# Pose-Group/FAMI-Pose

Hardware: AMD Instinct MI355X
Metric: train clips/sec (5-frame 384x288 HRNet-W48) (higher is better)
Workload: dtype f32

## Files before the change

fami-pose_amd/csrc/elementwise.hip:

```cpp
#include "common.h"

template <typename T>
__global__ void nchw_to_nhwc_kernel(const float* __restrict__ src, T* __restrict__ dst, int N, int C, int H, int W) {
  const long total = (long)N * C * H * W;
  const long HW = (long)H * W;
  for (long i = blockIdx.x * (long)blockDim.x + threadIdx.x; i < total; i += (long)gridDim.x * blockDim.x) {
    const int c = (int)(i % C);
    const long p = i / C;
    const long n = p / HW, hw = p - n * HW;
    st1(dst + i, src[(n * C + c) * HW + hw]);
  }
}
template <typename T>
__global__ void nhwc_to_nchw_kernel(const T* __restrict__ src, float* __restrict__ dst, int N, int C, int H, int W,
                                    int accumulate) {
  const long total = (long)N * C * H * W;
  const long HW = (long)H * W;
  for (long i = blockIdx.x * (long)blockDim.x + threadIdx.x; i < total; i += (long)gridDim.x * blockDim.x) {
    const long hw = i % HW;
    const long nc = i / HW;
    const long n = nc / C;
    const int c = (int)(nc - n * C);
    const float v = ld1(src + (n * HW + hw) * C + c);
    dst[i] = accumulate ? dst[i] + v : v;
  }
}

template <typename T>
__global__ void pack_frames_kernel(const float* __restrict__ kf, const float* __restrict__ sup, T* __restrict__ out,
                                   int B, int S, int H, int W) {
  const long HW = (long)H * W;
  const long total = (long)(1 + S) * B * HW * 3;
  for (long i = blockIdx.x * (long)blockDim.x + threadIdx.x; i < total; i += (long)gridDim.x * blockDim.x) {
    const int c = (int)(i % 3);
    const long p = i / 3;
    const long n = p / HW, hw = p - n * HW;
    const int f = (int)(n / B), b = (int)(n - (long)f * B);
    float v;
    if (f == 0)
      v = kf[((long)b * 3 + c) * HW + hw];
    else
      v = sup[((long)b * 3 * S + 3 * (f - 1) + c) * HW + hw];
    st1(out + i, v);
  }
}

template <typename T, int V>
__global__ void copy_channels_kernel(const T* __restrict__ src, T* __restrict__ dst, long P, int Cs, int src_off,
                                     int Cd, int dst_off, int Cc, int accumulate) {
  const int CcV = Cc / V;
  const long total = P * CcV;
  for (long i = blockIdx.x * (long)blockDim.x + threadIdx.x; i < total; i += (long)gridDim.x * blockDim.x) {
    const int c = (int)(i % CcV) * V;
    const long p = i / CcV;
    const T* sp = src + p * Cs + src_off + c;
    T* d = dst + p * Cd + dst_off + c;
    if (V == 4) {
      f32x4 v = ld4(sp);
      if (accumulate) v += ld4(d);
      st4(d, v);
    } else {
      const float v = ld1(sp);
      st1(d, accumulate ? ld1(d) + v : v);
    }
  }
}

struct Cat4 { const void* src[4]; void* dst[4]; int c[4], acc[4]; int n; };
template <typename T, bool SPLIT>
__global__ void cat4_kernel(Cat4 a, const T* __restrict__ whole_src, T* __restrict__ whole_dst, long P, int Ct) {
  const int CtV = Ct >> 2;
  const long total = P * CtV;
  for (long i = blockIdx.x * (long)blockDim.x + threadIdx.x; i < total; i += (long)gridDim.x * blockDim.x) {
    const int c = (int)(i % CtV) * 4;
    const long p = i / CtV;
    int k = 0, base = 0;
#pragma unroll
    for (int j = 0; j < 3; ++j)
      if (j + 1 < a.n && c >= base + a.c[k]) {
        base += a.c[k];
        ++k;
      }
    if (SPLIT) {
      T* d = reinterpret_cast<T*>(a.dst[k]);
      if (!d) continue;
      d += p * a.c[k] + (c - base);
      f32x4 v = ld4(whole_src + p * Ct + c);
      if (a.acc[k]) v += ld4(d);
      st4(d, v);
    } else {
      st4(whole_dst + p * Ct + c, ld4(reinterpret_cast<const T*>(a.src[k]) + p * a.c[k] + (c - base)));
    }
  }
}
template <typename T>
static int cat4_impl(bool split, const void* const* ptrs, const int* cs, const int* accs, int n, const T* whole_src, T* whole_dst, long P,
                     hipStream_t s, const char* nm) {
  FAMI_REQUIRE(ptrs && cs && n >= 1 && n <= 4 && P > 0 && (split ? (const void*)whole_src : (const void*)whole_dst), nm, "bad argument");
  Cat4 a;
  int Ct = 0;
  for (int k = 0; k < 4; ++k) {
    a.src[k] = nullptr; a.dst[k] = nullptr; a.c[k] = 0; a.acc[k] = 0;
    if (k < n) {
      FAMI_REQUIRE(cs[k] > 0 && (cs[k] & 3) == 0 && (split || ptrs[k]) && (reinterpret_cast<uintptr_t>(ptrs[k]) & 7) == 0, nm,
                   "channel counts must be multiples of 4, pointers 8-byte aligned");
      if (split) { a.dst[k] = const_cast<void*>(ptrs[k]); a.acc[k] = accs ? accs[k] : 0; }
      else a.src[k] = ptrs[k];
      a.c[k] = cs[k];
      Ct += cs[k];
    }
  }
  a.n = n;
  if (split) hipLaunchKernelGGL((cat4_kernel<T, true>), dim3(fami_ew_grid(P * Ct / 4)), dim3(256), 0, s, a, whole_src, (T*)nullptr, P, Ct);
  else hipLaunchKernelGGL((cat4_kernel<T, false>), dim3(fami_ew_grid(P * Ct / 4)), dim3(256), 0, s, a, (const T*)nullptr, whole_dst, P, Ct);
  FAMI_CHECK_LAUNCH(nm);
  return FAMI_OK;
}

__global__ void scale_pairs_kernel(const float* __restrict__ in, float* __restrict__ out, long n, float sx, float sy, int acc) {
  const long i = blockIdx.x * (long)blockDim.x + threadIdx.x;
  if (i >= 2 * n) return;
  const float v = in[i] * ((i & 1) ? sy : sx);
  out[i] = acc ? out[i] + v : v;
}

__global__ __launch_bounds__(256) void unscale_check_kernel(float* __restrict__ g, long n, float f, unsigned* __restrict__ flag) {
  bool bad = false;
  const long n4 = n >> 2;
  for (long i = blockIdx.x * (long)blockDim.x + threadIdx.x; i < n4; i += (long)gridDim.x * blockDim.x) {
    f32x4 v = ld4(g + i * 4) * f;
#pragma unroll
    for (int t = 0; t < 4; ++t) bad |= !(fabsf(v[t]) <= 3.4028235e38f);
    st4(g + i * 4, v);
  }
  for (long i = n4 * 4 + blockIdx.x * (long)blockDim.x + threadIdx.x; i < n; i += (long)gridDim.x * blockDim.x) {
    const float v = g[i] * f;
    bad |= !(fabsf(v) <= 3.4028235e38f);
    g[i] = v;
  }
  if (__any(bad) && (threadIdx.x & 63) == 0) atomicOr(flag, 1u);
}

template <typename T>
__global__ void axpby_kernel(const T* a, const T* b, T* out, long n, float alpha, float beta, int vec) {
  const long n4 = vec ? n >> 2 : 0;
  for (long i = blockIdx.x * (long)blockDim.x + threadIdx.x; i < n4; i += (long)gridDim.x * blockDim.x) {
    f32x4 v = ld4(a + i * 4) * alpha;
    if (b) v += ld4(b + i * 4) * beta;
    st4(out + i * 4, v);
  }
  for (long i = (n4 << 2) + blockIdx.x * (long)blockDim.x + threadIdx.x; i < n; i += (long)gridDim.x * blockDim.x) {
    float v = alpha * ld1(a + i);
    if (b) v += beta * ld1(b + i);
    st1(out + i, v);
  }
}

template <typename T>
__global__ void cast_add_kernel(const float* __restrict__ src, T* dst, long n, int accumulate) {
  for (long i = blockIdx.x * (long)blockDim.x + threadIdx.x; i < n; i += (long)gridDim.x * blockDim.x) {
    const float v = src[i];
    st1(dst + i, accumulate ? ld1(dst + i) + v : v);
  }
}

template <typename T>
__global__ void fill_kernel(T* out, long n, float v) {
  for (long i = blockIdx.x * (long)blockDim.x + threadIdx.x; i < n; i += (long)gridDim.x * blockDim.x) st1(out + i, v);
}

__global__ void incr_i64_kernel(long long* v, long n) {
  for (long i = blockIdx.x * (long)blockDim.x + threadIdx.x; i < n; i += (long)gridDim.x * blockDim.x) v[i] += 1;
}
__global__ void add_i64_kernel(long long* v, const long long* inc, long n) {
  for (long i = blockIdx.x * (long)blockDim.x + threadIdx.x; i < n; i += (long)gridDim.x * blockDim.x) v[i] += inc[i];
}

template <typename T>
struct FuseArgs {
  const T* x[4];
  const float* mean[4];
  const float* invstd[4];
  const float* gamma[4];
  const float* beta[4];
  int shift[4];
  int nterms;
};

template <typename T>
__global__ __launch_bounds__(256) void fuse_sum_kernel(FuseArgs<T> a, T* __restrict__ y, int N, int H, int W, int C,
                                                       int relu) {
  const int CV = C >> 2;
  const long total = (long)N * H * W * CV;
  for (long i = blockIdx.x * (long)blockDim.x + threadIdx.x; i < total; i += (long)gridDim.x * blockDim.x) {
    const int cv = (int)(i % CV);
    long p = i / CV;
    const int w = (int)(p % W);
    p /= W;
    const int h = (int)(p % H);
    const long n = p / H;
    f32x4 acc = {0.f, 0.f, 0.f, 0.f};
    for (int k = 0; k < a.nterms; ++k) {
      const int s = a.shift[k];
      const int Hk = H >> s, Wk = W >> s;
      const long o = ((n * Hk + (h >> s)) * Wk + (w >> s)) * C + cv * 4;
      f32x4 v = ld4(a.x[k] + o);
      if (a.mean[k]) {
#pragma unroll
        for (int t = 0; t < 4; ++t) {
          const int c = cv * 4 + t;
          const float sc = a.invstd[k][c] * a.gamma[k][c];
          v[t] = v[t] * sc + (a.beta[k][c] - a.mean[k][c] * sc);
        }
      }
      acc += v;
    }
    if (relu) {
#pragma unroll
      for (int t = 0; t < 4; ++t) acc[t] = fmaxf(acc[t], 0.f);
    }
    st4(y + i * 4, acc);
  }
}

template <typename T>
__global__ void relu_bwd_kernel(const T* __restrict__ dy, const T* __restrict__ y, T* dx, long n4, int accumulate) {
  for (long i = blockIdx.x * (long)blockDim.x + threadIdx.x; i < n4; i += (long)gridDim.x * blockDim.x) {
    f32x4 g = ld4(dy + i * 4);
    const f32x4 yy = ld4(y + i * 4);
#pragma unroll
    for (int t = 0; t < 4; ++t) g[t] = yy[t] > 0.f ? g[t] : 0.f;
    if (accumulate) g += ld4(dx + i * 4);
    st4(dx + i * 4, g);
  }
}

template <typename T>
__global__ void pool_relu_bwd_kernel(const T* __restrict__ dy, const T* __restrict__ y, T* __restrict__ out, int N,
                                     int Hl, int Wl, int C, int s, int relu) {
  const int CV = C >> 2;
  const int f = 1 << s;
  const int H = Hl << s, W = Wl << s;
  const long total = (long)N * Hl * Wl * CV;
  for (long i = blockIdx.x * (long)blockDim.x + threadIdx.x; i < total; i += (long)gridDim.x * blockDim.x) {
    const int cv = (int)(i % CV);
    long p = i / CV;
    const int wl = (int)(p % Wl);
    p /= Wl;
    const int hl = (int)(p % Hl);
    const long n = p / Hl;
    f32x4 acc = {0.f, 0.f, 0.f, 0.f};
    for (int dh = 0; dh < f; ++dh)
      for (int dw = 0; dw < f; ++dw) {
        const long o = ((n * H + (hl * f + dh)) * W + (wl * f + dw)) * C + cv * 4;
        f32x4 g = ld4(dy + o);
        if (relu) {
          const f32x4 yy = ld4(y + o);
#pragma unroll
          for (int t = 0; t < 4; ++t) g[t] = yy[t] > 0.f ? g[t] : 0.f;
        }
        acc += g;
      }
    st4(out + i * 4, acc);
  }
}

__global__ void adam_prep_kernel(float* state, float beta1, float beta2, unsigned* flag) {
  if (threadIdx.x == 0 && blockIdx.x == 0) {
    if (flag && *flag) {
      *flag = 0u;
      flag[1] += 1u;
      state[2] = 0.f;
      return;
    }
    const float t = state[0] + 1.f;
    state[0] = t;
    state[2] = 1.f - powf(beta1, t);
    state[3] = 1.f - powf(beta2, t);
  }
}
__device__ __forceinline__ void adam_elem(float& p, float gi, float& m, float& v, float beta1, float beta2, float eps,
                                          float wd, float step_size, float bc2s) {
#pragma clang fp contract(off)
  const float pi = p;
  if (wd != 0.f) gi = fmaf(wd, pi, gi);
  const float mi = beta1 * m + (1.f - beta1) * gi;
  const float vi = beta2 * v + (1.f - beta2) * gi * gi;
  m = mi;
  v = vi;
  p = fmaf(-step_size, mi / (sqrtf(vi) / bc2s + eps), pi);
}
template <bool SCALED>
__device__ __forceinline__ void adam_body(float* __restrict__ p, const float* __restrict__ g, float* __restrict__ m,
                                          float* __restrict__ v, long n, const float* __restrict__ state, float beta1,
                                          float beta2, float eps, float wd, const float* __restrict__ gmul) {
  const float lr = state[1], bc1 = state[2], bc2s = sqrtf(state[3]);
  if (bc1 == 0.f) return;
  const float step_size = lr / bc1;
  const float gm = SCALED ? gmul[0] : 1.f;
  for (long i = blockIdx.x * (long)blockDim.x + threadIdx.x; i < n; i += (long)gridDim.x * blockDim.x) {
    const float gi = SCALED ? mul_rn(gm, g[i]) : g[i];
    float pe = p[i], me = m[i], ve = v[i];
    adam_elem(pe, gi, me, ve, beta1, beta2, eps, wd, step_size, bc2s);
    m[i] = me;
    v[i] = ve;
    p[i] = pe;
  }
}
__global__ void adam_kernel(float* __restrict__ p, const float* __restrict__ g, float* __restrict__ m,
                            float* __restrict__ v, long n, const float* __restrict__ state, float beta1,
                            float beta2, float eps, float wd) {
  adam_body<false>(p, g, m, v, n, state, beta1, beta2, eps, wd, nullptr);
}
__global__ void adam_scaled_kernel(float* __restrict__ p, const float* __restrict__ g, float* __restrict__ m,
                                   float* __restrict__ v, long n, const float* __restrict__ state, float beta1,
                                   float beta2, float eps, float wd, const float* __restrict__ gmul) {
  adam_body<true>(p, g, m, v, n, state, beta1, beta2, eps, wd, gmul);
}


template <typename T>
static int nchw_to_nhwc_impl(const float* src, T* dst, int N, int C, int H, int W, hipStream_t s, const char* nm) {
  FAMI_REQUIRE(src && dst && N > 0 && C > 0 && H > 0 && W > 0, nm, "bad argument");
  hipLaunchKernelGGL(nchw_to_nhwc_kernel<T>, dim3(fami_ew_grid((long)N * C * H * W)), dim3(256), 0, s, src, dst, N, C, H, W);
  FAMI_CHECK_LAUNCH(nm);
  return FAMI_OK;
}
template <typename T>
static int nhwc_to_nchw_impl(const T* src, float* dst, int N, int C, int H, int W, int accumulate, hipStream_t s,
                             const char* nm) {
  FAMI_REQUIRE(src && dst && N > 0 && C > 0 && H > 0 && W > 0, nm, "bad argument");
  hipLaunchKernelGGL(nhwc_to_nchw_kernel<T>, dim3(fami_ew_grid((long)N * C * H * W)), dim3(256), 0, s, src, dst, N, C, H, W, accumulate);
  FAMI_CHECK_LAUNCH(nm);
  return FAMI_OK;
}
template <typename T>
static int pack_frames_impl(const float* kf, const float* sup, T* out, int B, int S, int H, int W, hipStream_t s,
                            const char* nm) {
  FAMI_REQUIRE(kf && out && B > 0 && S >= 0 && (S == 0 || sup), nm, "bad argument");
  hipLaunchKernelGGL(pack_frames_kernel<T>, dim3(fami_ew_grid((long)(1 + S) * B * H * W * 3)), dim3(256), 0, s, kf, sup, out, B, S, H, W);
  FAMI_CHECK_LAUNCH(nm);
  return FAMI_OK;
}
template <typename T>
static int copy_channels_impl(const T* src, T* dst, long P, int Cs, int src_off, int Cd, int dst_off, int Cc,
                              int accumulate, hipStream_t s, const char* nm) {
  FAMI_REQUIRE(src && dst && P > 0 && Cc > 0 && src_off >= 0 && dst_off >= 0 && src_off + Cc <= Cs && dst_off + Cc <= Cd, nm, "bad argument");
  const bool v4 = ((Cs | src_off | Cd | dst_off | Cc) & 3) == 0 && ((reinterpret_cast<uintptr_t>(src) | reinterpret_cast<uintptr_t>(dst)) & 15) == 0;
  if (v4)
    hipLaunchKernelGGL((copy_channels_kernel<T, 4>), dim3(fami_ew_grid(P * Cc / 4)), dim3(256), 0, s, src, dst, P, Cs, src_off, Cd, dst_off, Cc, accumulate);
  else
    hipLaunchKernelGGL((copy_channels_kernel<T, 1>), dim3(fami_ew_grid(P * Cc)), dim3(256), 0, s, src, dst, P, Cs, src_off, Cd, dst_off, Cc, accumulate);
  FAMI_CHECK_LAUNCH(nm);
  return FAMI_OK;
}
template <typename T>
static int axpby_impl(const T* a, const T* b, T* out, long n, float alpha, float beta, hipStream_t s, const char* nm) {
  FAMI_REQUIRE(a && out && n > 0, nm, "bad argument");
  const int vec = ((reinterpret_cast<uintptr_t>(a) | reinterpret_cast<uintptr_t>(b) | reinterpret_cast<uintptr_t>(out)) & (4 * sizeof(T) - 1)) == 0;
  hipLaunchKernelGGL(axpby_kernel<T>, dim3(fami_ew_grid(vec ? (n + 3) / 4 : n)), dim3(256), 0, s, a, b, out, n, alpha, beta, vec);
  FAMI_CHECK_LAUNCH(nm);
  return FAMI_OK;
}
template <typename T>
__global__ void widen_kernel(const T* __restrict__ src, float* __restrict__ dst, long n) {
  for (long i = blockIdx.x * (long)blockDim.x + threadIdx.x; i < n; i += (long)gridDim.x * blockDim.x) dst[i] = ld1(src + i);
}
template <typename T>
static int widen_impl(const T* src, float* dst, long n, hipStream_t s, const char* nm) {
  FAMI_REQUIRE(src && dst && n > 0, nm, "bad argument");
  hipLaunchKernelGGL(widen_kernel<T>, dim3(fami_ew_grid(n)), dim3(256), 0, s, src, dst, n);
  FAMI_CHECK_LAUNCH(nm);
  return FAMI_OK;
}

template <typename T>
static int cast_add_impl(const float* src, T* dst, long n, int accumulate, hipStream_t s, const char* nm) {
  FAMI_REQUIRE(src && dst && n > 0, nm, "bad argument");
  hipLaunchKernelGGL(cast_add_kernel<T>, dim3(fami_ew_grid(n)), dim3(256), 0, s, src, dst, n, accumulate);
  FAMI_CHECK_LAUNCH(nm);
  return FAMI_OK;
}
template <typename T>
static int fill_impl(T* out, long n, float v, hipStream_t s, const char* nm) {
  FAMI_REQUIRE(out && n > 0, nm, "bad argument");
  hipLaunchKernelGGL(fill_kernel<T>, dim3(fami_ew_grid(n)), dim3(256), 0, s, out, n, v);
  FAMI_CHECK_LAUNCH(nm);
  return FAMI_OK;
}
template <typename T>
static int fuse_sum_impl(int nterms, const T* const* x, const float* const* mean, const float* const* invstd,
                         const float* const* gamma, const float* const* beta, const int* shift, T* y, int N, int H,
                         int W, int C, int relu, hipStream_t s, const char* nm) {
  FAMI_REQUIRE(nterms >= 1 && nterms <= 4 && x && shift && y && (C % 4) == 0, nm, "bad argument");
  FuseArgs<T> a;
  a.nterms = nterms;
  for (int k = 0; k < 4; ++k) {
    const bool on = k < nterms;
    a.x[k] = on ? x[k] : nullptr;
    a.mean[k] = on && mean ? mean[k] : nullptr;
    a.invstd[k] = on && invstd ? invstd[k] : nullptr;
    a.gamma[k] = on && gamma ? gamma[k] : nullptr;
    a.beta[k] = on && beta ? beta[k] : nullptr;
    a.shift[k] = on ? shift[k] : 0;
    if (on) {
      FAMI_REQUIRE(a.x[k] && a.shift[k] >= 0 && (H % (1 << a.shift[k])) == 0 && (W % (1 << a.shift[k])) == 0, nm, "bad term");
    }
  }
  hipLaunchKernelGGL(fuse_sum_kernel<T>, dim3(fami_ew_grid((long)N * H * W * (C / 4))), dim3(256), 0, s, a, y, N, H, W, C, relu);
  FAMI_CHECK_LAUNCH(nm);
  return FAMI_OK;
}
template <typename T>
static int relu_bwd_impl(const T* dy, const T* y, T* dx, long n, int accumulate, hipStream_t s, const char* nm) {
  FAMI_REQUIRE(dy && y && dx && n > 0 && (n % 4) == 0, nm, "bad argument");
  hipLaunchKernelGGL(relu_bwd_kernel<T>, dim3(fami_ew_grid(n / 4)), dim3(256), 0, s, dy, y, dx, n / 4, accumulate);
  FAMI_CHECK_LAUNCH(nm);
  return FAMI_OK;
}
template <typename T>
static int pool_relu_bwd_impl(const T* dy, const T* y, T* out, int N, int Hl, int Wl, int C, int shift, int relu,
                              hipStream_t s, const char* nm) {
  FAMI_REQUIRE(dy && out && (!relu || y) && (C % 4) == 0 && shift >= 0 && shift <= 4, nm, "bad argument");
  hipLaunchKernelGGL(pool_relu_bwd_kernel<T>, dim3(fami_ew_grid((long)N * Hl * Wl * (C / 4))), dim3(256), 0, s, dy, y, out, N, Hl, Wl, C, shift, relu);
  FAMI_CHECK_LAUNCH(nm);
  return FAMI_OK;
}


#define FAMI_AXPBY_BATCH 32
struct AxpbyBatch { const float* a[FAMI_AXPBY_BATCH]; float* out[FAMI_AXPBY_BATCH]; int n[FAMI_AXPBY_BATCH]; };
__global__ __launch_bounds__(256) void add_batch_kernel(AxpbyBatch b) {
  const float* __restrict__ a = b.a[blockIdx.y];
  float* __restrict__ o = b.out[blockIdx.y];
  const int n = b.n[blockIdx.y];
  for (int i = blockIdx.x * 256 + threadIdx.x; i < n; i += gridDim.x * 256) o[i] += a[i];
}

extern "C" {

#define FAMI_EW_ABI(sfx, T)                                                                                            \
  int fami_nchw_to_nhwc_##sfx(const float* src, T* dst, int N, int C, int H, int W, hipStream_t s) {                   \
    return nchw_to_nhwc_impl<T>(src, dst, N, C, H, W, s, "fami_nchw_to_nhwc_" #sfx);                                   \
  }                                                                                                                    \
  int fami_nhwc_to_nchw_##sfx(const T* src, float* dst, int N, int C, int H, int W, int accumulate, hipStream_t s) {   \
    return nhwc_to_nchw_impl<T>(src, dst, N, C, H, W, accumulate, s, "fami_nhwc_to_nchw_" #sfx);                       \
  }                                                                                                                    \
                        \
  int fami_pack_frames_##sfx(const float* kf, const float* sup, T* out, int B, int S, int H, int W, hipStream_t s) {   \
    return pack_frames_impl<T>(kf, sup, out, B, S, H, W, s, "fami_pack_frames_" #sfx);                                 \
  }                                                                                                                    \
  int fami_copy_channels_##sfx(const T* src, T* dst, long P, int Cs, int src_off, int Cd, int dst_off, int Cc,         \
                               int accumulate, hipStream_t s) {                                                        \
    return copy_channels_impl<T>(src, dst, P, Cs, src_off, Cd, dst_off, Cc, accumulate, s, "fami_copy_channels_" #sfx);\
  }                                                                                                                    \
                                         \
  int fami_concat_channels_##sfx(const T* const* src, const int* c, int n, T* dst, long P, hipStream_t s) {            \
    return cat4_impl<T>(false, reinterpret_cast<const void* const*>(src), c, nullptr, n, (const T*)nullptr, dst, P, s, \
                        "fami_concat_channels_" #sfx);                                                                \
  }                                                                                                                    \
   \
  int fami_split_channels_##sfx(const T* src, T* const* dst, const int* c, const int* accumulate, int n, long P,       \
                                hipStream_t s) {                                                                       \
    return cat4_impl<T>(true, reinterpret_cast<const void* const*>(dst), c, accumulate, n, src, (T*)nullptr, P, s,     \
                        "fami_split_channels_" #sfx);                                                                 \
  }                                                                                                                    \
  int fami_axpby_##sfx(const T* a, const T* b, T* out, long n, float alpha, float beta, hipStream_t s) {               \
    return axpby_impl<T>(a, b, out, n, alpha, beta, s, "fami_axpby_" #sfx);                                            \
  }                                                                                                                    \
  int fami_cast_add_##sfx(const float* src, T* dst, long n, int accumulate, hipStream_t s) {                           \
    return cast_add_impl<T>(src, dst, n, accumulate, s, "fami_cast_add_" #sfx);                                        \
  }                                                                                                                    \
  int fami_widen_##sfx(const T* src, float* dst, long n, hipStream_t s) {                                              \
    return widen_impl<T>(src, dst, n, s, "fami_widen_" #sfx);                                                          \
  }                                                                                                                    \
  int fami_fill_##sfx(T* out, long n, float v, hipStream_t s) { return fill_impl<T>(out, n, v, s, "fami_fill_" #sfx); }\
   \
  int fami_fuse_sum_##sfx(int nterms, const T* const* x, const float* const* mean, const float* const* invstd,         \
                          const float* const* gamma, const float* const* beta, const int* shift, T* y, int N, int H,   \
                          int W, int C, int relu, hipStream_t s) {                                                     \
    return fuse_sum_impl<T>(nterms, x, mean, invstd, gamma, beta, shift, y, N, H, W, C, relu, s, "fami_fuse_sum_" #sfx);\
  }                                                                                                                    \
  int fami_relu_bwd_##sfx(const T* dy, const T* y, T* dx, long n, int accumulate, hipStream_t s) {                     \
    return relu_bwd_impl<T>(dy, y, dx, n, accumulate, s, "fami_relu_bwd_" #sfx);                                       \
  }                                                                                                                    \
                                                                     \
  int fami_pool_relu_bwd_##sfx(const T* dy, const T* y, T* out, int N, int Hl, int Wl, int C, int shift, int relu,     \
                               hipStream_t s) {                                                                        \
    return pool_relu_bwd_impl<T>(dy, y, out, N, Hl, Wl, C, shift, relu, s, "fami_pool_relu_bwd_" #sfx);                \
  }
FAMI_EW_ABI(f32, float)
FAMI_EW_ABI(bf16, bf16_t)
FAMI_EW_ABI(f16, f16_t)
#undef FAMI_EW_ABI

int fami_scale_pairs_f32(const float* in, float* out, long n, float sx, float sy, int accumulate, hipStream_t s) {
  FAMI_REQUIRE(in && out && n > 0, "fami_scale_pairs_f32", "bad argument");
  hipLaunchKernelGGL(scale_pairs_kernel, dim3(fami_cdiv(2 * n, 256)), dim3(256), 0, s, in, out, n, sx, sy, accumulate);
  FAMI_CHECK_LAUNCH("fami_scale_pairs_f32");
  return FAMI_OK;
}

int fami_incr_i64(long long* v, long n, hipStream_t s) {
  FAMI_REQUIRE(v && n > 0, "fami_incr_i64", "bad argument");
  hipLaunchKernelGGL(incr_i64_kernel, dim3(fami_ew_grid(n)), dim3(256), 0, s, v, n);
  FAMI_CHECK_LAUNCH("fami_incr_i64");
  return FAMI_OK;
}

int fami_add_i64(long long* v, const long long* inc, long n, hipStream_t s) {
  FAMI_REQUIRE(v && inc && n > 0, "fami_add_i64", "bad argument");
  hipLaunchKernelGGL(add_i64_kernel, dim3(fami_ew_grid(n)), dim3(256), 0, s, v, inc, n);
  FAMI_CHECK_LAUNCH("fami_add_i64");
  return FAMI_OK;
}

int fami_adam_prep_f32(float* state, float beta1, float beta2, hipStream_t s) {
  FAMI_REQUIRE(state, "fami_adam_prep_f32", "bad argument");
  hipLaunchKernelGGL(adam_prep_kernel, dim3(1), dim3(64), 0, s, state, beta1, beta2, (unsigned*)nullptr);
  FAMI_CHECK_LAUNCH("fami_adam_prep_f32");
  return FAMI_OK;
}
int fami_adam_prep_checked_f32(float* state, float beta1, float beta2, unsigned* flag, hipStream_t s) {
  FAMI_REQUIRE(state && flag, "fami_adam_prep_checked_f32", "bad argument");
  hipLaunchKernelGGL(adam_prep_kernel, dim3(1), dim3(64), 0, s, state, beta1, beta2, flag);
  FAMI_CHECK_LAUNCH("fami_adam_prep_checked_f32");
  return FAMI_OK;
}
int fami_unscale_check_f32(float* g, long n, float f, unsigned* flag, hipStream_t s) {
  FAMI_REQUIRE(g && flag && n > 0, "fami_unscale_check_f32", "bad argument");
  hipLaunchKernelGGL(unscale_check_kernel, dim3(fami_ew_grid((n + 3) / 4)), dim3(256), 0, s, g, n, f, flag);
  FAMI_CHECK_LAUNCH("fami_unscale_check_f32");
  return FAMI_OK;
}
int fami_adam_f32(float* p, const float* g, float* m, float* v, long n, const float* state, float beta1, float beta2,
                  float eps, float weight_decay, hipStream_t s) {
  FAMI_REQUIRE(p && g && m && v && state && n > 0, "fami_adam_f32", "bad argument");
  hipLaunchKernelGGL(adam_kernel, dim3(fami_ew_grid(n)), dim3(256), 0, s, p, g, m, v, n, state, beta1, beta2, eps, weight_decay);
  FAMI_CHECK_LAUNCH("fami_adam_f32");
  return FAMI_OK;
}
int fami_adam_scaled_f32(float* p, const float* g, float* m, float* v, long n, const float* state, float beta1, float beta2,
                         float eps, float weight_decay, const float* gmul, hipStream_t s) {
  FAMI_REQUIRE(p && g && m && v && state && gmul && n > 0, "fami_adam_scaled_f32", "bad argument");
  hipLaunchKernelGGL(adam_scaled_kernel, dim3(fami_ew_grid(n)), dim3(256), 0, s, p, g, m, v, n, state, beta1, beta2, eps,
                     weight_decay, gmul);
  FAMI_CHECK_LAUNCH("fami_adam_scaled_f32");
  return FAMI_OK;
}


int fami_add_batch_f32(const long* ptrs, const int* counts, int n, hipStream_t s) {
  FAMI_REQUIRE(ptrs && counts && n > 0, "fami_add_batch_f32", "bad argument");
  int i0 = 0;
  while (i0 < n) {
    AxpbyBatch b;
    int m = 0, maxn = 1;
    for (; m < FAMI_AXPBY_BATCH && i0 + m < n; ++m) {
      float* o = reinterpret_cast<float*>(ptrs[2 * (i0 + m) + 1]);
      bool repeated = false;
      for (int k = 0; k < m; ++k) repeated |= (b.out[k] == o);
      if (repeated) break;
      b.a[m] = reinterpret_cast<const float*>(ptrs[2 * (i0 + m)]);
      b.out[m] = o;
      b.n[m] = counts[i0 + m];
      if (b.n[m] > maxn) maxn = b.n[m];
    }
    for (int i = m; i < FAMI_AXPBY_BATCH; ++i) { b.a[i] = b.a[0]; b.out[i] = b.out[0]; b.n[i] = 0; }
    int gx = (maxn + 255) / 256;
    if (gx > 64) gx = 64;
    hipLaunchKernelGGL(add_batch_kernel, dim3(gx, m), dim3(256), 0, s, b);
    FAMI_CHECK_LAUNCH("fami_add_batch_f32");
    i0 += m;
  }
  return FAMI_OK;
}

}
```

fami-pose_amd/csrc/norm.hip:

```cpp
#include "common.h"

#define BN_MAXG 512
#ifndef BN_U
#define BN_U 4
#endif

struct ColMap {
  int cv, prow, rows, CV;
  bool active;
};
__device__ __forceinline__ ColMap col_map(int C) {
  ColMap m;
  m.CV = C >> 2;
  m.rows = 256 / m.CV;
  m.cv = threadIdx.x % m.CV;
  m.prow = threadIdx.x / m.CV;
  m.active = m.prow < m.rows;
  return m;
}

__device__ __forceinline__ double block_sum_d(double v, double* sm4) {
  v = wave_sum_d(v);
  const int lane = threadIdx.x & 63, wave = threadIdx.x >> 6;
  __syncthreads();
  if (lane == 0) sm4[wave] = v;
  __syncthreads();
  return (sm4[0] + sm4[1]) + (sm4[2] + sm4[3]);
}

template <typename T>
__global__ __launch_bounds__(256) void bn_partial_kernel(const T* __restrict__ x, float* __restrict__ partial,
                                                         long P, int C) {
  extern __shared__ float sm[];
  const ColMap m = col_map(C);
  f32x4 s = {0.f, 0.f, 0.f, 0.f}, q = {0.f, 0.f, 0.f, 0.f};
  if (m.active) {
    const f32x4 piv = ld4(x + m.cv * 4);
    const long step = (long)gridDim.x * m.rows;
    long p = (long)blockIdx.x * m.rows + m.prow;
    for (; p + (BN_U - 1) * step < P; p += BN_U * step) {
      f32x4 v[BN_U];
#pragma unroll
      for (int u = 0; u < BN_U; ++u) v[u] = ld4(x + (p + u * step) * C + m.cv * 4);
#pragma unroll
      for (int u = 0; u < BN_U; ++u) {
        const f32x4 d = v[u] - piv;
        s += d;
        q += d * d;
      }
    }
    for (; p < P; p += step) {
      const f32x4 v = ld4(x + p * C + m.cv * 4) - piv;
      s += v;
      q += v * v;
    }
    float* d = sm + (long)m.prow * 2 * C;
#pragma unroll
    for (int t = 0; t < 4; ++t) {
      d[m.cv * 4 + t] = s[t];
      d[C + m.cv * 4 + t] = q[t];
    }
  }
  __syncthreads();
  for (int e = threadIdx.x; e < 2 * C; e += 256) {
    float tot = 0.f;
    for (int r = 0; r < m.rows; ++r) tot += sm[(long)r * 2 * C + e];
    partial[(long)blockIdx.x * 2 * C + e] = tot;
  }
}

template <typename T>
__global__ void bn_finalize_kernel(const float* __restrict__ partial, const T* __restrict__ x, int G, long P,
                                   int C, float* mean, float* invstd, float* running_mean, float* running_var,
                                   float momentum, float eps) {
  __shared__ double sm4[4];
  const int c = blockIdx.x;
  double s = 0.0, q = 0.0;
  for (int g = threadIdx.x; g < G; g += 256) {
    s += (double)partial[(long)g * 2 * C + c];
    q += (double)partial[(long)g * 2 * C + C + c];
  }
  s = block_sum_d(s, sm4);
  q = block_sum_d(q, sm4);
  if (threadIdx.x != 0) return;
  const double dm = s / (double)P;
  double var = q / (double)P - dm * dm;
  if (var < 0.0) var = 0.0;
  const double mu = (double)ld1(x + c) + dm;
  mean[c] = (float)mu;
  invstd[c] = (float)(1.0 / sqrt(var + (double)eps));
  if (running_mean) {
    const double unb = P > 1 ? var * (double)P / (double)(P - 1) : var;
    running_mean[c] = (float)((1.0 - momentum) * running_mean[c] + momentum * mu);
    running_var[c] = (float)((1.0 - momentum) * running_var[c] + momentum * unb);
  }
}

__global__ void bn_finalize_slots_kernel(const double* __restrict__ slots, int NS, const float* __restrict__ pivot, long P,
                                         int C, float* mean, float* invstd, float* running_mean, float* running_var,
                                         float momentum, float eps) {
  const int c = blockIdx.x * blockDim.x + threadIdx.x;
  if (c >= C) return;
  double s = 0.0, q = 0.0;
  for (int k = 0; k < NS; ++k) {
    s += slots[(long)k * 2 * C + c];
    q += slots[(long)k * 2 * C + C + c];
  }
  const double invP = 1.0 / (double)P;
  const double dm = s * invP;
  double var = q * invP - dm * dm;
  if (var < 0.0) var = 0.0;
  const double mu = (double)pivot[c] + dm;
  mean[c] = (float)mu;
  invstd[c] = (float)(1.0 / sqrt(var + (double)eps));
  if (running_mean) {
    const double unb = P > 1 ? var * (double)P / (double)(P - 1) : var;
    running_mean[c] = (float)((1.0 - momentum) * running_mean[c] + momentum * mu);
    running_var[c] = (float)((1.0 - momentum) * running_var[c] + momentum * unb);
  }
}

__global__ void bn_running_update_kernel(float* running_mean, float* running_var, const float* __restrict__ mean,
                                         const float* __restrict__ invstd, int C, long P, float momentum, float eps) {
  const int c = blockIdx.x * blockDim.x + threadIdx.x;
  if (c >= C) return;
  const double mu = (double)mean[c], is = (double)invstd[c];
  double var = 1.0 / (is * is) - (double)eps;
  if (var < 0.0) var = 0.0;
  const double unb = P > 1 ? var * (double)P / (double)(P - 1) : var;
  running_mean[c] = (float)((1.0 - momentum) * running_mean[c] + momentum * mu);
  running_var[c] = (float)((1.0 - momentum) * running_var[c] + momentum * unb);
}


#define FAMI_BNRU_BATCH 32
struct BnRunBatch { float* rm[FAMI_BNRU_BATCH]; float* rv[FAMI_BNRU_BATCH]; const float* mean[FAMI_BNRU_BATCH]; const float* invstd[FAMI_BNRU_BATCH];
                    int C[FAMI_BNRU_BATCH]; float P[FAMI_BNRU_BATCH], mom[FAMI_BNRU_BATCH], eps[FAMI_BNRU_BATCH]; int n; };
__global__ __launch_bounds__(256) void bn_running_update_batch_kernel(BnRunBatch b) {
  const int c = blockIdx.x * blockDim.x + threadIdx.x;
  for (int k = 0; k < b.n; ++k) {
    if (c >= b.C[k]) continue;
    const double mu = (double)b.mean[k][c], is = (double)b.invstd[k][c];
    double var = 1.0 / (is * is) - (double)b.eps[k];
    if (var < 0.0) var = 0.0;
    const double P = (double)b.P[k];
    const double unb = P > 1.0 ? var * P / (P - 1.0) : var;
    const float momentum = b.mom[k];
    b.rm[k][c] = (float)((1.0 - momentum) * b.rm[k][c] + momentum * mu);
    b.rv[k][c] = (float)((1.0 - momentum) * b.rv[k][c] + momentum * unb);
  }
}

__global__ void bn_eval_stats_kernel(const float* running_mean, const float* running_var, float* mean, float* invstd,
                                     int C, float eps) {
  const int c = blockIdx.x * blockDim.x + threadIdx.x;
  if (c >= C) return;
  mean[c] = running_mean[c];
  invstd[c] = 1.0f / sqrtf(running_var[c] + eps);
}

template <typename T>
__global__ __launch_bounds__(256) void bn_apply_kernel(const T* __restrict__ x, const float* __restrict__ mean,
                                                       const float* __restrict__ invstd,
                                                       const float* __restrict__ gamma,
                                                       const float* __restrict__ beta,
                                                       const T* __restrict__ residual, T* __restrict__ y,
                                                       long P, int C, int relu) {
  const ColMap m = col_map(C);
  if (!m.active) return;
  f32x4 sc, sf;
#pragma unroll
  for (int t = 0; t < 4; ++t) {
    const int c = m.cv * 4 + t;
    sc[t] = invstd[c] * gamma[c];
    sf[t] = beta[c] - mean[c] * sc[t];
  }
  for (long p = (long)blockIdx.x * m.rows + m.prow; p < P; p += (long)gridDim.x * m.rows) {
    const long o = p * C + m.cv * 4;
    f32x4 v = ld4(x + o) * sc + sf;
    if (residual) v += ld4(residual + o);
    if (relu) {
#pragma unroll
      for (int t = 0; t < 4; ++t) v[t] = fmaxf(v[t], 0.f);
    }
    st4(y + o, v);
  }
}

template <typename T>
__global__ __launch_bounds__(256) void bn_bwd_partial_kernel(const T* __restrict__ dy,
                                                             const T* __restrict__ x,
                                                             const T* __restrict__ y,
                                                             const float* __restrict__ mean,
                                                             const float* __restrict__ invstd,
                                                             float* __restrict__ partial, long P, int C, int relu) {
  extern __shared__ float sm[];
  const ColMap m = col_map(C);
  f32x4 s = {0.f, 0.f, 0.f, 0.f}, q = {0.f, 0.f, 0.f, 0.f};
  if (m.active) {
    f32x4 mu, is;
#pragma unroll
    for (int t = 0; t < 4; ++t) {
      mu[t] = mean[m.cv * 4 + t];
      is[t] = invstd[m.cv * 4 + t];
    }
    const long step = (long)gridDim.x * m.rows;
    for (long p = (long)blockIdx.x * m.rows + m.prow; p < P; p += BN_U * step) {
      f32x4 g[BN_U], yy[BN_U], xx[BN_U];
      long o[BN_U];
#pragma unroll
      for (int u = 0; u < BN_U; ++u) {
        const long pu = p + u * step;
        o[u] = (pu < P ? pu : p) * C + m.cv * 4;
        g[u] = ld4(dy + o[u]);
      }
      if (relu) {
#pragma unroll
        for (int u = 0; u < BN_U; ++u) yy[u] = ld4(y + o[u]);
      }
#pragma unroll
      for (int u = 0; u < BN_U; ++u) xx[u] = ld4(x + o[u]);
#pragma unroll
      for (int u = 0; u < BN_U; ++u) {
        if (relu) {
#pragma unroll
          for (int t = 0; t < 4; ++t) g[u][t] = yy[u][t] > 0.f ? g[u][t] : 0.f;
        }
        if (p + u * step >= P) g[u] = f32x4{0.f, 0.f, 0.f, 0.f};
        const f32x4 xh = (xx[u] - mu) * is;
        s += g[u];
        q += g[u] * xh;
      }
    }
    float* d = sm + (long)m.prow * 2 * C;
#pragma unroll
    for (int t = 0; t < 4; ++t) {
      d[m.cv * 4 + t] = s[t];
      d[C + m.cv * 4 + t] = q[t];
    }
  }
  __syncthreads();
  for (int e = threadIdx.x; e < 2 * C; e += 256) {
    float tot = 0.f;
    for (int r = 0; r < m.rows; ++r) tot += sm[(long)r * 2 * C + e];
    partial[(long)blockIdx.x * 2 * C + e] = tot;
  }
}

__global__ void bn_bwd_finalize_kernel(const float* __restrict__ partial, int G, long P, int C, float* coef,
                                       float* dgamma, float* dbeta, int accumulate) {
  __shared__ double sm4[4];
  const int c = blockIdx.x;
  double s = 0.0, q = 0.0;
  for (int g = threadIdx.x; g < G; g += 256) {
    s += (double)partial[(long)g * 2 * C + c];
    q += (double)partial[(long)g * 2 * C + C + c];
  }
  s = block_sum_d(s, sm4);
  q = block_sum_d(q, sm4);
  if (threadIdx.x != 0) return;
  if (coef) {
    coef[c] = (float)(s / (double)P);
    coef[C + c] = (float)(q / (double)P);
  }
  if (dgamma) dgamma[c] = accumulate ? dgamma[c] + (float)q : (float)q;
  if (dbeta) dbeta[c] = accumulate ? dbeta[c] + (float)s : (float)s;
}

template <typename T>
__global__ __launch_bounds__(256) void bn_bwd_apply_kernel(const T* __restrict__ dy, const T* __restrict__ x,
                                                           const T* __restrict__ y,
                                                           const float* __restrict__ mean,
                                                           const float* __restrict__ invstd,
                                                           const float* __restrict__ gamma,
                                                           const float* __restrict__ coef, T* __restrict__ dx,
                                                           T* __restrict__ dres, long P, int C, int relu,
                                                           int acc_dx, int acc_dres) {
  const ColMap m = col_map(C);
  if (!m.active) return;
  f32x4 mu, is, gi, c1, c2;
#pragma unroll
  for (int t = 0; t < 4; ++t) {
    const int c = m.cv * 4 + t;
    mu[t] = mean[c];
    is[t] = invstd[c];
    gi[t] = gamma[c] * invstd[c];
    c1[t] = coef[c];
    c2[t] = coef[C + c];
  }
  for (long p = (long)blockIdx.x * m.rows + m.prow; p < P; p += (long)gridDim.x * m.rows) {
    const long o = p * C + m.cv * 4;
    f32x4 g = ld4(dy + o);
    if (relu) {
      const f32x4 yy = ld4(y + o);
#pragma unroll
      for (int t = 0; t < 4; ++t) g[t] = yy[t] > 0.f ? g[t] : 0.f;
    }
    const f32x4 xh = (ld4(x + o) - mu) * is;
    f32x4 d = gi * (g - c1 - xh * c2);
    if (acc_dx) d += ld4(dx + o);
    st4(dx + o, d);
    if (dres) {
      f32x4 r = g;
      if (acc_dres) r += ld4(dres + o);
      st4(dres + o, r);
    }
  }
}

template <typename T, bool SUMS>
__global__ __launch_bounds__(256) void bn_eval_bwd_kernel(const T* __restrict__ dy, const T* __restrict__ x,
                                                          const T* __restrict__ y, const float* __restrict__ mean,
                                                          const float* __restrict__ invstd,
                                                          const float* __restrict__ gamma, float* __restrict__ partial,
                                                          T* dx, T* dres, long P, int C, int relu, int acc_dx,
                                                          int acc_dres) {
  extern __shared__ float sm[];
  const ColMap m = col_map(C);
  f32x4 s = {0.f, 0.f, 0.f, 0.f}, q = {0.f, 0.f, 0.f, 0.f};
  if (m.active) {
    f32x4 mu = {0.f, 0.f, 0.f, 0.f}, is, gi;
#pragma unroll
    for (int t = 0; t < 4; ++t) {
      const int c = m.cv * 4 + t;
      is[t] = invstd[c];
      gi[t] = gamma[c] * is[t];
      if (SUMS) mu[t] = mean[c];
    }
    const long step = (long)gridDim.x * m.rows;
    for (long p = (long)blockIdx.x * m.rows + m.prow; p < P; p += BN_U * step) {
      f32x4 g[BN_U], yy[BN_U], xx[BN_U], dd[BN_U], rr[BN_U];
      long o[BN_U];
#pragma unroll
      for (int u = 0; u < BN_U; ++u) {
        const long pu = p + u * step;
        o[u] = (pu < P ? pu : p) * C + m.cv * 4;
        g[u] = ld4(dy + o[u]);
      }
      if (relu) {
#pragma unroll
        for (int u = 0; u < BN_U; ++u) yy[u] = ld4(y + o[u]);
      }
      if (SUMS) {
#pragma unroll
        for (int u = 0; u < BN_U; ++u) xx[u] = ld4(x + o[u]);
      }
      if (acc_dx) {
#pragma unroll
        for (int u = 0; u < BN_U; ++u) dd[u] = ld4(dx + o[u]);
      }
      if (dres && acc_dres) {
#pragma unroll
        for (int u = 0; u < BN_U; ++u) rr[u] = ld4(dres + o[u]);
      }
#pragma unroll
      for (int u = 0; u < BN_U; ++u) {
        if (relu) {
#pragma unroll
          for (int t = 0; t < 4; ++t) g[u][t] = yy[u][t] > 0.f ? g[u][t] : 0.f;
        }
        const bool in = p + u * step < P;
        if (SUMS) {
          const f32x4 gz = in ? g[u] : f32x4{0.f, 0.f, 0.f, 0.f};
          s += gz;
          q += gz * ((xx[u] - mu) * is);
        }
        if (in) {
          f32x4 d = g[u] * gi;
          if (acc_dx) d += dd[u];
          st4(dx + o[u], d);
          if (dres) {
            f32x4 r = g[u];
            if (acc_dres) r += rr[u];
            st4(dres + o[u], r);
          }
        }
      }
    }
    if (SUMS) {
      float* d = sm + (long)m.prow * 2 * C;
#pragma unroll
      for (int t = 0; t < 4; ++t) {
        d[m.cv * 4 + t] = s[t];
        d[C + m.cv * 4 + t] = q[t];
      }
    }
  }
  if (!SUMS) return;
  __syncthreads();
  for (int e = threadIdx.x; e < 2 * C; e += 256) {
    float tot = 0.f;
    for (int r = 0; r < m.rows; ++r) tot += sm[(long)r * 2 * C + e];
    partial[(long)blockIdx.x * 2 * C + e] = tot;
  }
}


template <typename T>
__global__ __launch_bounds__(256) void bn_partial2_kernel(const T* __restrict__ x, double* __restrict__ slots, int NS,
                                                          long P, int C) {
  extern __shared__ float sm[];
  const ColMap m = col_map(C);
  f32x4 s = {0.f, 0.f, 0.f, 0.f}, q = {0.f, 0.f, 0.f, 0.f};
  if (m.active) {
    const f32x4 piv = ld4(x + m.cv * 4);
    const long step = (long)gridDim.x * m.rows;
    long p = (long)blockIdx.x * m.rows + m.prow;
    for (; p + (BN_U - 1) * step < P; p += BN_U * step) {
      f32x4 v[BN_U];
#pragma unroll
      for (int u = 0; u < BN_U; ++u) v[u] = ld4(x + (p + u * step) * C + m.cv * 4);
#pragma unroll
      for (int u = 0; u < BN_U; ++u) {
        const f32x4 d = v[u] - piv;
        s += d;
        q += d * d;
      }
    }
    for (; p < P; p += step) {
      const f32x4 v = ld4(x + p * C + m.cv * 4) - piv;
      s += v;
      q += v * v;
    }
    float* d = sm + (long)m.prow * 2 * C;
#pragma unroll
    for (int t = 0; t < 4; ++t) {
      d[m.cv * 4 + t] = s[t];
      d[C + m.cv * 4 + t] = q[t];
    }
  }
  __syncthreads();
  double* row = slots + (long)(blockIdx.x % NS) * 2 * C;
  for (int e = threadIdx.x; e < 2 * C; e += 256) {
    float tot = 0.f;
    for (int r = 0; r < m.rows; ++r) tot += sm[(long)r * 2 * C + e];
    unsafeAtomicAdd(row + e, (double)tot);
  }
}

__device__ __forceinline__ void bn_scale_shift(float mean, float invstd, float gamma, float beta, float& sc, float& sf) {
  sc = invstd * gamma;
  sf = __builtin_fmaf(-mean, sc, beta);
}

template <typename T>
__global__ __launch_bounds__(256) void bn_apply2_kernel(const T* __restrict__ x, const double* __restrict__ slots, int NS,
                                                        const float* __restrict__ gamma, const float* __restrict__ beta,
                                                        const T* __restrict__ residual, T* __restrict__ y,
                                                        float* __restrict__ mean, float* __restrict__ invstd,
                                                        float* running_mean, float* running_var, long P, int C,
                                                        int relu, float momentum, float eps, const float* pivot) {
  extern __shared__ float sm[];
  for (int c = threadIdx.x; c < C; c += 256) {
    double s = 0.0, q = 0.0;
    for (int k = 0; k < NS; ++k) {
      s += slots[(long)k * 2 * C + c];
      q += slots[(long)k * 2 * C + C + c];
    }
    const double invP = 1.0 / (double)P;
    const double dm = s * invP;
    double var = q * invP - dm * dm;
    if (var < 0.0) var = 0.0;
    const double mu = (double)(pivot ? pivot[c] : ld1(x + c)) + dm;
    const float muf = (float)mu;
    const float isf = (float)(1.0 / sqrt(var + (double)eps));
    if (blockIdx.x == 0) {
      mean[c] = muf;
      invstd[c] = isf;
      if (running_mean) {
        const double unb = P > 1 ? var * (double)P / (double)(P - 1) : var;
        running_mean[c] = (float)((1.0 - momentum) * running_mean[c] + momentum * mu);
        running_var[c] = (float)((1.0 - momentum) * running_var[c] + momentum * unb);
      }
    }
    float sc, sf;
    bn_scale_shift(muf, isf, gamma[c], beta[c], sc, sf);
    sm[c] = sc;
    sm[C + c] = sf;
  }
  __syncthreads();
  const ColMap m = col_map(C);
  if (!m.active) return;
  const f32x4 sc = *reinterpret_cast<const f32x4*>(sm + m.cv * 4), sf = *reinterpret_cast<const f32x4*>(sm + C + m.cv * 4);
  for (long p = (long)blockIdx.x * m.rows + m.prow; p < P; p += (long)gridDim.x * m.rows) {
    const long o = p * C + m.cv * 4;
    const f32x4 xv = ld4(x + o);
    f32x4 v;
#pragma unroll
    for (int t = 0; t < 4; ++t) v[t] = __builtin_fmaf(xv[t], sc[t], sf[t]);
    if (residual) v += ld4(residual + o);
    if (relu) {
#pragma unroll
      for (int t = 0; t < 4; ++t) v[t] = fmaxf(v[t], 0.f);
    }
    st4(y + o, v);
  }
}

__device__ __forceinline__ f32x4 bn_relu_mask(f32x4 g, int relu, f32x4 yy, f32x4 xv, f32x4 sc, f32x4 sf) {
  if (relu == 1) {
#pragma unroll
    for (int t = 0; t < 4; ++t) g[t] = yy[t] > 0.f ? g[t] : 0.f;
  } else if (relu == 2) {
#pragma unroll
    for (int t = 0; t < 4; ++t) g[t] = __builtin_fmaf(xv[t], sc[t], sf[t]) > 0.f ? g[t] : 0.f;
  }
  return g;
}

template <typename T>
__global__ __launch_bounds__(256) void bn_bwd_partial2_kernel(const T* __restrict__ dy, const T* __restrict__ x,
                                                              const T* __restrict__ y, const float* __restrict__ mean,
                                                              const float* __restrict__ invstd,
                                                              const float* __restrict__ gamma,
                                                              const float* __restrict__ beta,
                                                              double* __restrict__ slots, int NS, long P, int C, int relu) {
  extern __shared__ float sm[];
  const ColMap m = col_map(C);
  f32x4 s = {0.f, 0.f, 0.f, 0.f}, q = {0.f, 0.f, 0.f, 0.f};
  if (m.active) {
    f32x4 mu, is, sc, sf;
#pragma unroll
    for (int t = 0; t < 4; ++t) {
      const int c = m.cv * 4 + t;
      mu[t] = mean[c];
      is[t] = invstd[c];
      float a, b;
      bn_scale_shift(mu[t], is[t], gamma[c], beta[c], a, b);
      sc[t] = a;
      sf[t] = b;
    }
    const long step = (long)gridDim.x * m.rows;
    for (long p = (long)blockIdx.x * m.rows + m.prow; p < P; p += BN_U * step) {
      f32x4 g[BN_U], yy[BN_U], xx[BN_U];
      long o[BN_U];
#pragma unroll
      for (int u = 0; u < BN_U; ++u) {
        const long pu = p + u * step;
        o[u] = (pu < P ? pu : p) * C + m.cv * 4;
        g[u] = ld4(dy + o[u]);
      }
      if (relu == 1) {
#pragma unroll
        for (int u = 0; u < BN_U; ++u) yy[u] = ld4(y + o[u]);
      }
#pragma unroll
      for (int u = 0; u < BN_U; ++u) xx[u] = ld4(x + o[u]);
#pragma unroll
      for (int u = 0; u < BN_U; ++u) {
        g[u] = bn_relu_mask(g[u], relu, yy[u], xx[u], sc, sf);
        if (p + u * step >= P) g[u] = f32x4{0.f, 0.f, 0.f, 0.f};
        const f32x4 xh = (xx[u] - mu) * is;
        s += g[u];
        q += g[u] * xh;
      }
    }
    float* d = sm + (long)m.prow * 2 * C;
#pragma unroll
    for (int t = 0; t < 4; ++t) {
      d[m.cv * 4 + t] = s[t];
      d[C + m.cv * 4 + t] = q[t];
    }
  }
  __syncthreads();
  double* row = slots + (long)(blockIdx.x % NS) * 2 * C;
  for (int e = threadIdx.x; e < 2 * C; e += 256) {
    float tot = 0.f;
    for (int r = 0; r < m.rows; ++r) tot += sm[(long)r * 2 * C + e];
    unsafeAtomicAdd(row + e, (double)tot);
  }
}

template <typename T>
__global__ __launch_bounds__(256) void bn_bwd_apply2_kernel(const T* __restrict__ dy, const T* __restrict__ x,
                                                            const T* __restrict__ y, const float* __restrict__ mean,
                                                            const float* __restrict__ invstd,
                                                            const float* __restrict__ gamma,
                                                            const float* __restrict__ beta,
                                                            const double* __restrict__ slots, int NS, T* __restrict__ dx,
                                                            float* dgamma, float* dbeta, T* __restrict__ dres, long P,
                                                            int C, int relu, int acc_dx, int acc_param, int acc_dres) {
  extern __shared__ float sm[];
  for (int c = threadIdx.x; c < C; c += 256) {
    double s = 0.0, q = 0.0;
    for (int k = 0; k < NS; ++k) {
      s += slots[(long)k * 2 * C + c];
      q += slots[(long)k * 2 * C + C + c];
    }
    sm[c] = (float)(s / (double)P);
    sm[C + c] = (float)(q / (double)P);
    if (blockIdx.x == 0) {
      if (dgamma) dgamma[c] = acc_param ? dgamma[c] + (float)q : (float)q;
      if (dbeta) dbeta[c] = acc_param ? dbeta[c] + (float)s : (float)s;
    }
  }
  __syncthreads();
  const ColMap m = col_map(C);
  if (!m.active) return;
  f32x4 mu, is, gi, sc, sf;
  const f32x4 c1 = *reinterpret_cast<const f32x4*>(sm + m.cv * 4), c2 = *reinterpret_cast<const f32x4*>(sm + C + m.cv * 4);
#pragma unroll
  for (int t = 0; t < 4; ++t) {
    const int c = m.cv * 4 + t;
    mu[t] = mean[c];
    is[t] = invstd[c];
    gi[t] = gamma[c] * invstd[c];
    float a, b;
    bn_scale_shift(mu[t], is[t], gamma[c], beta[c], a, b);
    sc[t] = a;
    sf[t] = b;
  }
  for (long p = (long)blockIdx.x * m.rows + m.prow; p < P; p += (long)gridDim.x * m.rows) {
    const long o = p * C + m.cv * 4;
    f32x4 g = ld4(dy + o);
    const f32x4 xv = ld4(x + o);
    f32x4 yy = {0.f, 0.f, 0.f, 0.f};
    if (relu == 1) yy = ld4(y + o);
    g = bn_relu_mask(g, relu, yy, xv, sc, sf);
    const f32x4 xh = (xv - mu) * is;
    f32x4 d = gi * (g - c1 - xh * c2);
    if (acc_dx) d += ld4(dx + o);
    st4(dx + o, d);
    if (dres) {
      f32x4 r = g;
      if (acc_dres) r += ld4(dres + o);
      st4(dres + o, r);
    }
  }
}

#define BN_SMALL_P 16384
static inline bool bn_small_ok(long P, int C) { return P * C <= g_bn_small_elems; }

__device__ __forceinline__ f32x4 block_sum4(f32x4 v, float* sm) {
  const int lane = threadIdx.x & 63, wave = threadIdx.x >> 6;
#pragma unroll
  for (int t = 0; t < 4; ++t) v[t] = wave_sum(v[t]);
  __syncthreads();
  if (lane == 0) {
#pragma unroll
    for (int t = 0; t < 4; ++t) sm[wave * 4 + t] = v[t];
  }
  __syncthreads();
  f32x4 r;
#pragma unroll
  for (int t = 0; t < 4; ++t) r[t] = (sm[t] + sm[4 + t]) + (sm[8 + t] + sm[12 + t]);
  return r;
}

template <typename T>
__global__ __launch_bounds__(256) void bn_small_fwd_kernel(const T* __restrict__ x, const T* __restrict__ residual,
                                                           T* __restrict__ y, const float* __restrict__ gamma,
                                                           const float* __restrict__ beta, float* __restrict__ mean,
                                                           float* __restrict__ invstd, float* running_mean,
                                                           float* running_var, long P, int C, int relu,
                                                           float momentum, float eps) {
  __shared__ float sm[16];
  const int c0 = blockIdx.x * 4;
  const f32x4 piv = ld4(x + c0);
  f32x4 s = {0.f, 0.f, 0.f, 0.f}, q = {0.f, 0.f, 0.f, 0.f};
  for (long p = threadIdx.x; p < P; p += 256) {
    const f32x4 v = ld4(x + p * C + c0) - piv;
    s += v;
    q += v * v;
  }
  s = block_sum4(s, sm);
  q = block_sum4(q, sm);
  f32x4 mu, is, sc, sf;
#pragma unroll
  for (int t = 0; t < 4; ++t) {
    const double dm = (double)s[t] / (double)P;
    double var = (double)q[t] / (double)P - dm * dm;
    if (var < 0.0) var = 0.0;
    const double m = (double)piv[t] + dm;
    mu[t] = (float)m;
    is[t] = (float)(1.0 / sqrt(var + (double)eps));
    if (threadIdx.x == 0) {
      mean[c0 + t] = mu[t];
      invstd[c0 + t] = is[t];
      if (running_mean) {
        const double unb = P > 1 ? var * (double)P / (double)(P - 1) : var;
        running_mean[c0 + t] = (float)((1.0 - momentum) * running_mean[c0 + t] + momentum * m);
        running_var[c0 + t] = (float)((1.0 - momentum) * running_var[c0 + t] + momentum * unb);
      }
    }
    sc[t] = is[t] * gamma[c0 + t];
    sf[t] = beta[c0 + t] - mu[t] * sc[t];
  }
  for (long p = threadIdx.x; p < P; p += 256) {
    const long o = p * C + c0;
    f32x4 v = ld4(x + o) * sc + sf;
    if (residual) v += ld4(residual + o);
    if (relu) {
#pragma unroll
      for (int t = 0; t < 4; ++t) v[t] = fmaxf(v[t], 0.f);
    }
    st4(y + o, v);
  }
}

template <typename T>
__global__ __launch_bounds__(256) void bn_small_bwd_kernel(const T* __restrict__ dy, const T* __restrict__ x,
                                                           const T* __restrict__ y, const float* __restrict__ mean,
                                                           const float* __restrict__ invstd,
                                                           const float* __restrict__ gamma, T* __restrict__ dx,
                                                           float* dgamma, float* dbeta, T* __restrict__ dres, long P,
                                                           int C, int relu, int acc_dx, int acc_param, int acc_dres) {
  __shared__ float sm[16];
  const int c0 = blockIdx.x * 4;
  f32x4 mu, is, gi;
#pragma unroll
  for (int t = 0; t < 4; ++t) {
    mu[t] = mean[c0 + t];
    is[t] = invstd[c0 + t];
    gi[t] = gamma[c0 + t] * is[t];
  }
  f32x4 s = {0.f, 0.f, 0.f, 0.f}, q = {0.f, 0.f, 0.f, 0.f};
  for (long p = threadIdx.x; p < P; p += 256) {
    const long o = p * C + c0;
    f32x4 g = ld4(dy + o);
    if (relu) {
      const f32x4 yy = ld4(y + o);
#pragma unroll
      for (int t = 0; t < 4; ++t) g[t] = yy[t] > 0.f ? g[t] : 0.f;
    }
    s += g;
    q += g * ((ld4(x + o) - mu) * is);
  }
  s = block_sum4(s, sm);
  q = block_sum4(q, sm);
  f32x4 c1, c2;
#pragma unroll
  for (int t = 0; t < 4; ++t) {
    c1[t] = (float)((double)s[t] / (double)P);
    c2[t] = (float)((double)q[t] / (double)P);
    if (threadIdx.x == 0) {
      if (dgamma) dgamma[c0 + t] = acc_param ? dgamma[c0 + t] + q[t] : q[t];
      if (dbeta) dbeta[c0 + t] = acc_param ? dbeta[c0 + t] + s[t] : s[t];
    }
  }
  for (long p = threadIdx.x; p < P; p += 256) {
    const long o = p * C + c0;
    f32x4 g = ld4(dy + o);
    if (relu) {
      const f32x4 yy = ld4(y + o);
#pragma unroll
      for (int t = 0; t < 4; ++t) g[t] = yy[t] > 0.f ? g[t] : 0.f;
    }
    const f32x4 xh = (ld4(x + o) - mu) * is;
    f32x4 d = gi * (g - c1 - xh * c2);
    if (acc_dx) d += ld4(dx + o);
    st4(dx + o, d);
    if (dres) {
      f32x4 r = g;
      if (acc_dres) r += ld4(dres + o);
      st4(dres + o, r);
    }
  }
}

template <typename T>
__global__ __launch_bounds__(256) void chan_sum_partial_kernel(const T* __restrict__ x,
                                                               float* __restrict__ partial, long P, int C) {
  extern __shared__ float sm[];
  if (C > 256) {
    for (int c = threadIdx.x; c < C; c += 256) {
      float s = 0.f;
      for (long p = blockIdx.x; p < P; p += gridDim.x) s += ld1(x + p * C + c);
      partial[(long)blockIdx.x * C + c] = s;
    }
    return;
  }
  const int rows = max(1, 256 / C);
  const int c = threadIdx.x % C, prow = threadIdx.x / C;
  const bool active = prow < rows;
  float s = 0.f;
  if (active) {
    for (long p = (long)blockIdx.x * rows + prow; p < P; p += (long)gridDim.x * rows) s += ld1(x + p * C + c);
    sm[prow * C + c] = s;
  }
  __syncthreads();
  for (int e = threadIdx.x; e < C; e += 256) {
    float tot = 0.f;
    for (int r = 0; r < rows; ++r) tot += sm[r * C + e];
    partial[(long)blockIdx.x * C + e] = tot;
  }
}
template <typename T>
__global__ __launch_bounds__(256) void chan_sum_partial4_kernel(const T* __restrict__ x, float* __restrict__ partial, long P,
                                                                int C) {
  extern __shared__ float sm[];
  const ColMap m = col_map(C);
  f32x4 s = {0.f, 0.f, 0.f, 0.f};
  if (m.active) {
    const long step = (long)gridDim.x * m.rows;
    long p = (long)blockIdx.x * m.rows + m.prow;
    for (; p + (BN_U - 1) * step < P; p += BN_U * step) {
      f32x4 v[BN_U];
#pragma unroll
      for (int u = 0; u < BN_U; ++u) v[u] = ld4(x + (p + u * step) * C + m.cv * 4);
#pragma unroll
      for (int u = 0; u < BN_U; ++u) s += v[u];
    }
    for (; p < P; p += step) s += ld4(x + p * C + m.cv * 4);
    *reinterpret_cast<f32x4*>(sm + (long)m.prow * C + m.cv * 4) = s;
  }
  __syncthreads();
  for (int e = threadIdx.x; e < C; e += 256) {
    float tot = 0.f;
    for (int r = 0; r < m.rows; ++r) tot += sm[r * C + e];
    partial[(long)blockIdx.x * C + e] = tot;
  }
}
__global__ void chan_sum_finalize_kernel(const float* __restrict__ partial, int G, int C, float* out,
                                         int accumulate) {
  __shared__ double sm4[4];
  const int c = blockIdx.x;
  double s = 0.0;
  for (int g = threadIdx.x; g < G; g += 256) s += (double)partial[(long)g * C + c];
  s = block_sum_d(s, sm4);
  if (threadIdx.x != 0) return;
  out[c] = accumulate ? out[c] + (float)s : (float)s;
}

static inline int bn_grid(long P, int C) {
  const int rows = 256 / (C >> 2);
  long g = (P + (long)rows * 2 * BN_U - 1) / ((long)rows * 2 * BN_U);
  if (g > BN_MAXG) g = BN_MAXG;
  if (g < 1) g = 1;
  return (int)g;
}
static inline int bn_grid2(long P, int C, int esz) {
  const int rows = 256 / (C >> 2);
  long g = (P + (long)rows * 2 * BN_U - 1) / ((long)rows * 2 * BN_U);
  const long cap = (long)g_bn2_maxg * (esz == 4 ? 4 : 1);
  if (g > cap) g = cap;
  if (g < 1) g = 1;
  return (int)g;
}
static inline bool bn_shape_ok(long P, int C) { return P > 0 && C >= 4 && (C % 4) == 0 && C <= 1024; }

template <typename T>
static int bn_stats_impl(const T* x, long P, int C, float* mean, float* invstd, float* running_mean,
                         float* running_var, float momentum, float eps, float* ws, hipStream_t s, const char* nm) {
  FAMI_REQUIRE(x && mean && invstd && ws, nm, "null pointer");
  if (!bn_shape_ok(P, C)) {
    fami_set_error(nm, "C must be a multiple of 4, <= 1024");
    return FAMI_ESHAPE;
  }
  const int G = bn_grid(P, C);
  const int rows = 256 / (C >> 2);
  hipLaunchKernelGGL(bn_partial_kernel<T>, dim3(G), dim3(256), (size_t)rows * 2 * C * sizeof(float), s, x, ws, P, C);
  FAMI_CHECK_LAUNCH(nm);
  hipLaunchKernelGGL(bn_finalize_kernel<T>, dim3(C), dim3(256), 0, s, ws, x, G, P, C, mean, invstd, running_mean,
                     running_var, momentum, eps);
  FAMI_CHECK_LAUNCH(nm);
  return FAMI_OK;
}

template <typename T>
static int bn_apply_impl(const T* x, const float* mean, const float* invstd, const float* gamma, const float* beta,
                         const T* residual, T* y, long P, int C, int relu, hipStream_t s, const char* nm) {
  FAMI_REQUIRE(x && mean && invstd && gamma && beta && y, nm, "null pointer");
  if (!bn_shape_ok(P, C)) {
    fami_set_error(nm, "C must be a multiple of 4, <= 1024");
    return FAMI_ESHAPE;
  }
  const int rows = 256 / (C >> 2);
  long g = (P + rows - 1) / rows;
  if (g > 2048) g = 2048;
  hipLaunchKernelGGL(bn_apply_kernel<T>, dim3((int)g), dim3(256), 0, s, x, mean, invstd, gamma, beta, residual, y, P,
                     C, relu);
  FAMI_CHECK_LAUNCH(nm);
  return FAMI_OK;
}

template <typename T>
static int bn_bwd_impl(const T* dy, const T* x, const T* y, const float* mean, const float* invstd,
                       const float* gamma, T* dx, float* dgamma, float* dbeta, T* dres, long P, int C, int relu,
                       int acc_dx, int acc_param, int acc_dres, float* ws, hipStream_t s, const char* nm) {
  FAMI_REQUIRE(dy && x && mean && invstd && gamma && dx && ws, nm, "null pointer");
  FAMI_REQUIRE(!relu || y, nm, "relu needs y");
  if (!bn_shape_ok(P, C)) {
    fami_set_error(nm, "C must be a multiple of 4, <= 1024");
    return FAMI_ESHAPE;
  }
  if (bn_small_ok(P, C)) {
    hipLaunchKernelGGL(bn_small_bwd_kernel<T>, dim3(C / 4), dim3(256), 0, s, dy, x, y, mean, invstd, gamma, dx, dgamma,
                       dbeta, dres, P, C, relu, acc_dx, acc_param, acc_dres);
    FAMI_CHECK_LAUNCH(nm);
    return FAMI_OK;
  }
  const int G = bn_grid(P, C);
  const int rows = 256 / (C >> 2);
  float* coef = ws + (long)BN_MAXG * 2 * C - 2 * C;
  const int Gp = G < BN_MAXG ? G : BN_MAXG - 1;
  hipLaunchKernelGGL(bn_bwd_partial_kernel<T>, dim3(Gp), dim3(256), (size_t)rows * 2 * C * sizeof(float), s, dy, x, y,
                     mean, invstd, ws, P, C, relu);
  FAMI_CHECK_LAUNCH(nm);
  hipLaunchKernelGGL(bn_bwd_finalize_kernel, dim3(C), dim3(256), 0, s, ws, Gp, P, C, coef, dgamma, dbeta, acc_param);
  FAMI_CHECK_LAUNCH(nm);
  long g = (P + rows - 1) / rows;
  if (g > 2048) g = 2048;
  hipLaunchKernelGGL(bn_bwd_apply_kernel<T>, dim3((int)g), dim3(256), 0, s, dy, x, y, mean, invstd, gamma, coef, dx,
                     dres, P, C, relu, acc_dx, acc_dres);
  FAMI_CHECK_LAUNCH(nm);
  return FAMI_OK;
}

template <typename T>
static int bn_eval_bwd_impl(const T* dy, const T* x, const T* y, const float* mean, const float* invstd,
                            const float* gamma, T* dx, float* dgamma, float* dbeta, T* dres, long P, int C, int relu,
                            int acc_dx, int acc_param, int acc_dres, float* ws, hipStream_t s, const char* nm) {
  FAMI_REQUIRE(dy && invstd && gamma && dx, nm, "null pointer");
  FAMI_REQUIRE(!relu || y, nm, "relu needs y");
  if (!bn_shape_ok(P, C)) {
    fami_set_error(nm, "C must be a multiple of 4, <= 1024");
    return FAMI_ESHAPE;
  }
  const int rows = 256 / (C >> 2);
  if (!dgamma && !dbeta) {
    long g = (P + (long)rows * BN_U - 1) / ((long)rows * BN_U);
    if (g > 2048) g = 2048;
    hipLaunchKernelGGL((bn_eval_bwd_kernel<T, false>), dim3((int)g), dim3(256), 0, s, dy, x, y, mean, invstd, gamma,
                       (float*)nullptr, dx, dres, P, C, relu, acc_dx, acc_dres);
    FAMI_CHECK_LAUNCH(nm);
    return FAMI_OK;
  }
  FAMI_REQUIRE(x && mean && ws, nm, "parameter sums need x, mean and ws");
  const int G = bn_grid(P, C);
  hipLaunchKernelGGL((bn_eval_bwd_kernel<T, true>), dim3(G), dim3(256), (size_t)rows * 2 * C * sizeof(float), s, dy, x, y,
                     mean, invstd, gamma, ws, dx, dres, P, C, relu, acc_dx, acc_dres);
  FAMI_CHECK_LAUNCH(nm);
  hipLaunchKernelGGL(bn_bwd_finalize_kernel, dim3(C), dim3(256), 0, s, ws, G, P, C, (float*)nullptr, dgamma, dbeta,
                     acc_param);
  FAMI_CHECK_LAUNCH(nm);
  return FAMI_OK;
}

template <typename T>
static int bn_train_fwd_impl(const T* x, const T* residual, T* y, const float* gamma, const float* beta, float* mean,
                             float* invstd, float* running_mean, float* running_var, long P, int C, int relu,
                             float momentum, float eps, float* ws, hipStream_t s, const char* nm) {
  FAMI_REQUIRE(x && y && gamma && beta && mean && invstd && ws, nm, "null pointer");
  if (!bn_shape_ok(P, C)) {
    fami_set_error(nm, "C must be a multiple of 4, <= 1024");
    return FAMI_ESHAPE;
  }
  if (bn_small_ok(P, C)) {
    hipLaunchKernelGGL(bn_small_fwd_kernel<T>, dim3(C / 4), dim3(256), 0, s, x, residual, y, gamma, beta, mean, invstd,
                       running_mean, running_var, P, C, relu, momentum, eps);
    FAMI_CHECK_LAUNCH(nm);
    return FAMI_OK;
  }
  int rc = bn_stats_impl<T>(x, P, C, mean, invstd, running_mean, running_var, momentum, eps, ws, s, nm);
  if (rc != FAMI_OK) return rc;
  return bn_apply_impl<T>(x, mean, invstd, gamma, beta, residual, y, P, C, relu, s, nm);
}

static inline int bn_apply_grid(long P, int C) {
  const int rows = 256 / (C >> 2);
  long g = (P + rows - 1) / rows;
  if (g > 1024) g = 1024;
  return (int)g;
}

template <typename T>
static int bn_train_fwd2_impl(const T* x, const T* residual, T* y, const float* gamma, const float* beta, float* mean,
                              float* invstd, float* running_mean, float* running_var, long P, int C, int relu,
                              float momentum, float eps, void* slots, int pre, hipStream_t s, const char* nm) {
  FAMI_REQUIRE(x && y && gamma && beta && mean && invstd && slots, nm, "null pointer");
  if (!bn_shape_ok(P, C)) {
    fami_set_error(nm, "C must be a multiple of 4, <= 1024");
    return FAMI_ESHAPE;
  }
  if (bn_small_ok(P, C) && !pre) {
    hipLaunchKernelGGL(bn_small_fwd_kernel<T>, dim3(C / 4), dim3(256), 0, s, x, residual, y, gamma, beta, mean, invstd,
                       running_mean, running_var, P, C, relu, momentum, eps);
    FAMI_CHECK_LAUNCH(nm);
    return FAMI_OK;
  }
  const int G = bn_grid2(P, C, (int)sizeof(T)), NS = bn_slots(C);
  const int rows = 256 / (C >> 2);
  if (!pre) {
    hipLaunchKernelGGL(bn_partial2_kernel<T>, dim3(G), dim3(256), (size_t)rows * 2 * C * sizeof(float), s, x,
                       reinterpret_cast<double*>(slots), NS, P, C);
    FAMI_CHECK_LAUNCH(nm);
  }
  hipLaunchKernelGGL(bn_apply2_kernel<T>, dim3(bn_apply_grid(P, C)), dim3(256), (size_t)2 * C * sizeof(float), s, x,
                     reinterpret_cast<const double*>(slots), NS, gamma, beta, residual, y, mean, invstd, running_mean,
                     running_var, P, C, relu, momentum, eps, pre ? bn_slots_pivot(slots, C) : (const float*)nullptr);
  FAMI_CHECK_LAUNCH(nm);
  return FAMI_OK;
}

template <typename T>
static int bn_bwd2_impl(const T* dy, const T* x, const T* y, const float* mean, const float* invstd, const float* gamma,
                        const float* beta, T* dx, float* dgamma, float* dbeta, T* dres, long P, int C, int relu,
                        int acc_dx, int acc_param, int acc_dres, void* slots, int pre, hipStream_t s, const char* nm) {
  FAMI_REQUIRE(dy && x && mean && invstd && gamma && beta && dx && slots, nm, "null pointer");
  FAMI_REQUIRE(relu != 1 || y, nm, "relu = 1 needs y");
  FAMI_REQUIRE(relu >= 0 && relu <= 2, nm, "relu must be 0, 1 (mask from y) or 2 (mask recomputed from x)");
  if (!bn_shape_ok(P, C)) {
    fami_set_error(nm, "C must be a multiple of 4, <= 1024");
    return FAMI_ESHAPE;
  }
  if (bn_small_ok(P, C) && !pre) {
    FAMI_REQUIRE(relu != 2 || y, nm, "small tensors take the ReLU mask from y");
    hipLaunchKernelGGL(bn_small_bwd_kernel<T>, dim3(C / 4), dim3(256), 0, s, dy, x, y, mean, invstd, gamma, dx, dgamma,
                       dbeta, dres, P, C, relu ? 1 : 0, acc_dx, acc_param, acc_dres);
    FAMI_CHECK_LAUNCH(nm);
    return FAMI_OK;
  }
  const int G = bn_grid2(P, C, (int)sizeof(T)), NS = bn_slots(C);
  const int rows = 256 / (C >> 2);
  if (!pre) {
    hipLaunchKernelGGL(bn_bwd_partial2_kernel<T>, dim3(G), dim3(256), (size_t)rows * 2 * C * sizeof(float), s, dy, x, y, mean,
                       invstd, gamma, beta, reinterpret_cast<double*>(slots), NS, P, C, relu);
    FAMI_CHECK_LAUNCH(nm);
  }
  hipLaunchKernelGGL(bn_bwd_apply2_kernel<T>, dim3(bn_apply_grid(P, C)), dim3(256), (size_t)2 * C * sizeof(float), s, dy, x,
                     y, mean, invstd, gamma, beta, reinterpret_cast<const double*>(slots), NS, dx, dgamma, dbeta, dres, P,
                     C, relu, acc_dx, acc_param, acc_dres);
  FAMI_CHECK_LAUNCH(nm);
  return FAMI_OK;
}

template <typename T>
static int channel_sum_impl(const T* x, long P, int C, float* out, int accumulate, float* ws, hipStream_t s,
                            const char* nm) {
  FAMI_REQUIRE(x && out && ws && P > 0 && C > 0, nm, "bad argument");
  FAMI_REQUIRE(C <= 4096, nm, "C > 4096 unsupported");
  int rows = C > 256 ? 1 : 256 / C;
  const bool vec4 = C % 4 == 0 && C <= 1024 && P >= 4096;
  if (vec4) rows = 256 / (C >> 2);
  long g = (P + rows - 1) / rows;
  if (vec4) g = (g + 2 * BN_U - 1) / (2 * BN_U);
  if (g > BN_MAXG) g = BN_MAXG;
  if (g < 1) g = 1;
  if (vec4) hipLaunchKernelGGL(chan_sum_partial4_kernel<T>, dim3((int)g), dim3(256), (size_t)rows * C * sizeof(float), s, x, ws, P, C);
  else hipLaunchKernelGGL(chan_sum_partial_kernel<T>, dim3((int)g), dim3(256), C > 256 ? 0 : (size_t)rows * C * sizeof(float), s, x, ws, P, C);
  FAMI_CHECK_LAUNCH(nm);
  hipLaunchKernelGGL(chan_sum_finalize_kernel, dim3(C), dim3(256), 0, s, ws, (int)g, C, out, accumulate);
  FAMI_CHECK_LAUNCH(nm);
  return FAMI_OK;
}

extern "C" {

long fami_bn_workspace(int C) { return (long)BN_MAXG * 2 * C * (long)sizeof(float); }
long fami_bn_slots_bytes(int C) { return bn_slots_bytes(C); }
int fami_bn_tune_small(long elems) {
  if (elems <= -1000) { g_bn2_maxg = (int)(-elems - 1000); return FAMI_OK; }
  if (elems < 0) { g_bn_small_elems = 32768; g_bn2_maxg = 512; return FAMI_OK; }
  g_bn_small_elems = elems;
  return FAMI_OK;
}
int fami_bn_is_small(long P, int C) { return bn_small_ok(P, C) ? 1 : 0; }
long fami_channel_sum_workspace(int C) { return (long)BN_MAXG * C * (long)sizeof(float); }

int fami_bn_eval_stats_f32(const float* running_mean, const float* running_var, float* mean, float* invstd, int C,
                           float eps, hipStream_t s) {
  FAMI_REQUIRE(running_mean && running_var && mean && invstd && C > 0, "fami_bn_eval_stats_f32", "bad argument");
  hipLaunchKernelGGL(bn_eval_stats_kernel, dim3(fami_cdiv(C, 64)), dim3(64), 0, s, running_mean, running_var, mean,
                     invstd, C, eps);
  FAMI_CHECK_LAUNCH("fami_bn_eval_stats_f32");
  return FAMI_OK;
}

int fami_bn_finalize_slots_f32(void* slots, long P, int C, float* mean, float* invstd, float* running_mean,
                               float* running_var, float momentum, float eps, hipStream_t s) {
  FAMI_REQUIRE(slots && mean && invstd && C > 0 && P > 0, "fami_bn_finalize_slots_f32", "bad argument");
  hipLaunchKernelGGL(bn_finalize_slots_kernel, dim3(fami_cdiv(C, 64)), dim3(64), 0, s, reinterpret_cast<const double*>(slots),
                     bn_slots(C), bn_slots_pivot(slots, C), P, C, mean, invstd, running_mean, running_var, momentum, eps);
  FAMI_CHECK_LAUNCH("fami_bn_finalize_slots_f32");
  return FAMI_OK;
}

int fami_bn_running_update_f32(float* running_mean, float* running_var, const float* mean, const float* invstd, int C,
                               long P, float momentum, float eps, hipStream_t s) {
  FAMI_REQUIRE(running_mean && running_var && mean && invstd && C > 0 && P > 0, "fami_bn_running_update_f32", "bad argument");
  hipLaunchKernelGGL(bn_running_update_kernel, dim3(fami_cdiv(C, 64)), dim3(64), 0, s, running_mean, running_var, mean,
                     invstd, C, P, momentum, eps);
  FAMI_CHECK_LAUNCH("fami_bn_running_update_f32");
  return FAMI_OK;
}


int fami_bn_running_update_batch_f32(const long* ptrs, const float* meta, int n, hipStream_t s) {
  FAMI_REQUIRE(ptrs && meta && n > 0, "fami_bn_running_update_batch_f32", "bad argument");
  for (int i0 = 0; i0 < n; i0 += FAMI_BNRU_BATCH) {
    BnRunBatch b;
    b.n = n - i0 < FAMI_BNRU_BATCH ? n - i0 : FAMI_BNRU_BATCH;
    int maxc = 1;
    for (int i = 0; i < FAMI_BNRU_BATCH; ++i) {
      const int j = i < b.n ? i0 + i : i0;
      b.rm[i] = reinterpret_cast<float*>(ptrs[4 * j]);
      b.rv[i] = reinterpret_cast<float*>(ptrs[4 * j + 1]);
      b.mean[i] = reinterpret_cast<const float*>(ptrs[4 * j + 2]);
      b.invstd[i] = reinterpret_cast<const float*>(ptrs[4 * j + 3]);
      b.C[i] = (int)meta[4 * j];
      b.P[i] = meta[4 * j + 1];
      b.mom[i] = meta[4 * j + 2];
      b.eps[i] = meta[4 * j + 3];
      if (i < b.n && b.C[i] > maxc) maxc = b.C[i];
    }
    hipLaunchKernelGGL(bn_running_update_batch_kernel, dim3(fami_cdiv(maxc, 256)), dim3(256), 0, s, b);
    FAMI_CHECK_LAUNCH("fami_bn_running_update_batch_f32");
  }
  return FAMI_OK;
}

#define FAMI_BN_ABI(sfx, T)                                                                                            \
                            \
  int fami_bn_stats_##sfx(const T* x, long P, int C, float* mean, float* invstd, float* running_mean,                  \
                          float* running_var, float momentum, float eps, float* ws, hipStream_t s) {                   \
    return bn_stats_impl<T>(x, P, C, mean, invstd, running_mean, running_var, momentum, eps, ws, s, "fami_bn_stats_" #sfx); \
  }                                                                                                                    \
  int fami_bn_apply_##sfx(const T* x, const float* mean, const float* invstd, const float* gamma, const float* beta,   \
                          const T* residual, T* y, long P, int C, int relu, hipStream_t s) {                           \
    return bn_apply_impl<T>(x, mean, invstd, gamma, beta, residual, y, P, C, relu, s, "fami_bn_apply_" #sfx);          \
  }                                                                                                                    \
                     \
  int fami_bn_bwd_##sfx(const T* dy, const T* x, const T* y, const float* mean, const float* invstd,                   \
                        const float* gamma, T* dx, float* dgamma, float* dbeta, T* dres, long P, int C, int relu,      \
                        int acc_dx, int acc_param, int acc_dres, float* ws, hipStream_t s) {                           \
    return bn_bwd_impl<T>(dy, x, y, mean, invstd, gamma, dx, dgamma, dbeta, dres, P, C, relu, acc_dx, acc_param,       \
                          acc_dres, ws, s, "fami_bn_bwd_" #sfx);                                                       \
  }                                                                                                                    \
   \
   \
  int fami_bn_eval_bwd_##sfx(const T* dy, const T* x, const T* y, const float* mean, const float* invstd,              \
                             const float* gamma, T* dx, float* dgamma, float* dbeta, T* dres, long P, int C, int relu, \
                             int acc_dx, int acc_param, int acc_dres, float* ws, hipStream_t s) {                      \
    return bn_eval_bwd_impl<T>(dy, x, y, mean, invstd, gamma, dx, dgamma, dbeta, dres, P, C, relu, acc_dx, acc_param,  \
                               acc_dres, ws, s, "fami_bn_eval_bwd_" #sfx);                                             \
  }                                                                                                                    \
                           \
  int fami_bn_train_fwd_##sfx(const T* x, const T* residual, T* y, const float* gamma, const float* beta,              \
                              float* mean, float* invstd, float* running_mean, float* running_var, long P, int C,      \
                              int relu, float momentum, float eps, float* ws, hipStream_t s) {                         \
    return bn_train_fwd_impl<T>(x, residual, y, gamma, beta, mean, invstd, running_mean, running_var, P, C, relu,      \
                                momentum, eps, ws, s, "fami_bn_train_fwd_" #sfx);                                      \
  }                                                                                                                    \
   \
   \
   \
  int fami_bn_train_fwd2_##sfx(const T* x, const T* residual, T* y, const float* gamma, const float* beta,             \
                               float* mean, float* invstd, float* running_mean, float* running_var, long P, int C,     \
                               int relu, float momentum, float eps, void* slots, hipStream_t s) {                      \
    return bn_train_fwd2_impl<T>(x, residual, y, gamma, beta, mean, invstd, running_mean, running_var, P, C, relu,     \
                                 momentum, eps, slots, 0, s, "fami_bn_train_fwd2_" #sfx);                              \
  }                                                                                                                    \
    \
  int fami_bn_apply_slots_##sfx(const T* x, const T* residual, T* y, const float* gamma, const float* beta,            \
                                float* mean, float* invstd, float* running_mean, float* running_var, long P, int C,    \
                                int relu, float momentum, float eps, void* slots, hipStream_t s) {                     \
    return bn_train_fwd2_impl<T>(x, residual, y, gamma, beta, mean, invstd, running_mean, running_var, P, C, relu,     \
                                 momentum, eps, slots, 1, s, "fami_bn_apply_slots_" #sfx);                             \
  }                                                                                                                    \
  \
  \
  int fami_bn_bwd_apply_slots_##sfx(const T* dz, const T* x, const float* mean, const float* invstd,                   \
                                    const float* gamma, const float* beta, T* dx, float* dgamma, float* dbeta,         \
                                    T* dres, long P, int C, int acc_dx, int acc_param, int acc_dres, void* slots,      \
                                    hipStream_t s) {                                                                   \
    return bn_bwd2_impl<T>(dz, x, (const T*)nullptr, mean, invstd, gamma, beta, dx, dgamma, dbeta, dres, P, C, 0,      \
                           acc_dx, acc_param, acc_dres, slots, 1, s, "fami_bn_bwd_apply_slots_" #sfx);                 \
  }                                                                                                                    \
  int fami_bn_bwd2_##sfx(const T* dy, const T* x, const T* y, const float* mean, const float* invstd,                  \
                         const float* gamma, const float* beta, T* dx, float* dgamma, float* dbeta, T* dres, long P,   \
                         int C, int relu, int acc_dx, int acc_param, int acc_dres, void* slots, hipStream_t s) {       \
    return bn_bwd2_impl<T>(dy, x, y, mean, invstd, gamma, beta, dx, dgamma, dbeta, dres, P, C, relu, acc_dx,           \
                           acc_param, acc_dres, slots, 0, s, "fami_bn_bwd2_" #sfx);                                    \
  }                                                                                                                    \
                                                                        \
  int fami_channel_sum_##sfx(const T* x, long P, int C, float* out, int accumulate, float* ws, hipStream_t s) {        \
    return channel_sum_impl<T>(x, P, C, out, accumulate, ws, s, "fami_channel_sum_" #sfx);                             \
  }
FAMI_BN_ABI(f32, float)
FAMI_BN_ABI(bf16, bf16_t)
FAMI_BN_ABI(f16, f16_t)
#undef FAMI_BN_ABI

}
```

fami-pose_amd/engine.py:

```python
import ctypes
import weakref

import torch

from . import options
from ._lib import lib

BN_EPS = 1e-5


def _p(t):
    return None if t is None else t.data_ptr()


_ABL_WGRAD = options.flag('FAMI_ABL_WGRAD', '0')
_SFX = {torch.float32: '_f32', torch.bfloat16: '_bf16', torch.float16: '_f16'}


def _sfx(t):
    return _SFX[t.dtype]


class T:
    __slots__ = ('data', 'grad', 'requires_grad', 'parent', 'n0', 'n1', 'f32grad', 'uses', 'lanes', 'bnrec', 'nofuse', 'xbn', 'pending')

    def __init__(self, data, requires_grad=False, parent=None, n0=0, n1=0, f32grad=False):
        self.data = data
        self.grad = None
        self.requires_grad = requires_grad
        self.parent, self.n0, self.n1 = parent, n0, n1
        self.f32grad = f32grad
        self.uses = 0
        self.lanes = None
        self.bnrec = None
        self.nofuse = parent is not None
        self.xbn = None
        self.pending = None

    @property
    def shape(self):
        return tuple(self.data.shape)


class CatParam:

    def __init__(self, parts):
        self.parts = list(parts)
        self.shape = (sum(p.shape[0] for p in self.parts),) + tuple(self.parts[0].shape[1:])

    @property
    def requires_grad(self):
        return all(p.requires_grad for p in self.parts)

    def adjacent(self):
        ps = self.parts
        if any(not p.data.is_contiguous() or p.dtype != torch.float32 or p.shape[1:] != ps[0].shape[1:] for p in ps):
            return False
        if len({p.requires_grad for p in ps}) != 1:
            return False
        return all(b.data_ptr() == a.data_ptr() + a.numel() * 4 for a, b in zip(ps, ps[1:]))

    @property
    def data(self):
        a = self.parts[0].data
        return torch.as_strided(a, self.shape, a.stride())

    def numel(self):
        return sum(p.numel() for p in self.parts)


def _real_params(ps):
    out = []
    for p in ps:
        if isinstance(p, CatParam):
            out.extend(p.parts)
        else:
            out.append(p)
    return out


class _RoutedQueries:

    def __init__(self, L, eng):
        self._L, self._eng = L, weakref.ref(eng)

    def __getattr__(self, name):
        fn, L, eng = getattr(self._L.cdll, name), self._L, self._eng()

        def query(*args):
            L.bind(eng.route)
            return fn(*args)
        return query


class Engine:
    def __init__(self, device, grad_views=None, record=True, dtype=torch.float32, deterministic=None, route=None):
        assert dtype in _SFX
        self.route = route
        self.dt = dtype
        self.sfx = _SFX[dtype]
        self.half = dtype != torch.float32
        self.deterministic = (options.flag('FAMI_DETERMINISTIC', '0')) if deterministic is None else bool(deterministic)
        self.L = lib()
        self.Q = _RoutedQueries(self.L, self)
        self.record = record
        self.dev = device
        self.tape = []
        self.param_grads = {}
        self.grad_views = grad_views
        self.stream = None
        self.aux = {}
        self.bn_trained = []
        self.prepacked = None
        self.use_lanes = options.flag('FAMI_LANES', '1')
        self.lane = 0
        self._main = None
        self._side = []
        self._forked = 0
        self._epoch = 0
        self._lane_owner = {}
        self._lane_priv = {}
        self._merge = []
        self.defer_bn = None
        self._side_events = []
        self.persist_lanes = True
        self.head_wlane = self.use_lanes
        self.wlane_scope = False
        self.wlane_pair = False
        self.stem_wlanes = 4
        self.head_wlanes = 4
        self._wstreams = []
        self._wowner = {}
        self._wflip = 0
        self._wdirty = False
        self._sliced = []
        self._keep = []
        self.bn2 = not self.deterministic
        fz = options.get('FAMI_FUSE_BN', 'auto')
        self.fuse_bn_fwd = self.bn2 and fz in ('1', 'fwd', 'auto', 'autoall', 'fwd3')
        self.fuse_bn_fwd3 = fz == 'fwd3' or (fz == 'auto' and self.half)
        self.fuse_bn_bwd = self.bn2 and fz in ('1', 'bwd')
        self.fuse_bn_bwd_auto = self.bn2 and self.half and fz in ('auto', 'autoall', 'bwdauto')
        self.fuse_bn_c64 = 2
        self.merge_predictors = options.flag('FAMI_MERGE_PREDICTORS', '1')
        self.use_xbn = options.flag('FAMI_XBN', '0' if self.half else '1')
        self.serial_scope = False
        self.serial_fuse = False
        self.nfused = {'fwd': 0, 'bwd': 0, 'xbn': 0}
        self.conv_flops = 0
        self.defer_reduce = True
        self.npair = 0
        self._red = {}
        self._red_dw = {}
        self._red_longs = self.Q.fami_wgrad_reduce_desc_longs()
        self.abl_lanes = options.number('FAMI_ABL_LANES', '0')
        self.nbnin = 0
        self._pending = []
        self.bn_in = self.half and options.flag('FAMI_BN_IN', '1')
        self.abl_bn1 = options.number('FAMI_ABL_BN1', '0')
        self.sync_stream()
        self._zero_begin()

    def rq(self, p):
        return self.record and p is not None and p.requires_grad

    def sync_stream(self):
        self._main = torch.cuda.current_stream(self.dev)
        self.stream = self._main.cuda_stream
        self.lane = 0

    _side_pool = {}

    def _lanes(self, n):
        pool = Engine._side_pool.setdefault(self.dev, [])
        main = self._main.cuda_stream
        side = [s for s in pool if s.cuda_stream != main]
        tries = 0
        while len(side) < n - 1 and tries < 64:
            tries += 1
            s = torch.cuda.Stream(self.dev)
            if s.cuda_stream != main and all(s.cuda_stream != t.cuda_stream for t in pool):
                pool.append(s)
                side.append(s)
        if len(side) < n - 1:
            raise RuntimeError('could not obtain %d distinct side streams' % (n - 1))
        self._side = side
        if options.flag('FAMI_DEBUG_STREAMS'):
            print('[fami] lanes: main %#x side %s capturing %s' % (main, [hex(t.cuda_stream) for t in side[:n - 1]],
                                                                  torch.cuda.is_current_stream_capturing()), flush=True)
        return side

    def set_lane(self, i):
        self.lane = i
        self.stream = self._main.cuda_stream if i == 0 else self._side[i - 1].cuda_stream

    _wgrad_pool = {}

    def _lane_stream(self):
        return self._main if self.lane == 0 else self._side[self.lane - 1]

    def _new_wstream(self, extra=()):
        taken = {self._main.cuda_stream} | {t.cuda_stream for t in Engine._side_pool.get(self.dev, [])} | set(extra)
        ws, tries = None, 0
        while (ws is None or ws.cuda_stream in taken) and tries < 64:
            ws = torch.cuda.Stream(self.dev)
            tries += 1
        if ws.cuda_stream in taken:
            raise RuntimeError('could not obtain a distinct weight-gradient stream')
        return ws

    def _enter_wlane(self, pair=False, key=None):
        n = max(1, self.stem_wlanes if pair else self.head_wlanes)
        while len(self._wstreams) < n:
            k = len(self._wstreams)
            taken = {self._main.cuda_stream} | {t.cuda_stream for t in Engine._side_pool.get(self.dev, [])} | {t.cuda_stream for t in self._wstreams}
            ws = Engine._wgrad_pool.get((self.dev, k))
            if ws is None or ws.cuda_stream in taken:
                ws = self._new_wstream(tuple(t.cuda_stream for t in self._wstreams))
            Engine._wgrad_pool[(self.dev, k)] = ws
            self._wstreams.append(ws)
        own = self._wowner.get(key) if key is not None else None
        if own is not None and own < n:
            target = self._wstreams[own]
        else:
            self._wflip = (self._wflip + 1) % n
            target = self._wstreams[self._wflip]
            if key is not None:
                self._wowner[key] = self._wflip
        ev = torch.cuda.Event()
        ev.record(self._lane_stream())
        target.wait_event(ev)
        saved = self.stream
        self.stream = target.cuda_stream
        self._wdirty = True
        return saved

    def sync_wgrad_lane(self):
        if self._wdirty:
            for ws in self._wstreams:
                self.flush_reduces(ws.cuda_stream)
                ev = torch.cuda.Event()
                ev.record(ws)
                self._main.wait_event(ev)
            self._wdirty = False

    def side_launch(self, fn):
        side = self._lanes(2)[0]
        ev = torch.cuda.Event()
        ev.record(self._main)
        side.wait_event(ev)
        fn(side.cuda_stream)
        done = torch.cuda.Event()
        done.record(side)
        return done

    late_weights_ready = None

    def join_late_weights(self):
        if self.late_weights_ready is not None:
            self._main.wait_event(self.late_weights_ready)
            self.late_weights_ready = None

    def join_side(self):
        for ev in self._side_events:
            self._main.wait_event(ev)
        self._side_events = []

    def wait_main(self, ev):
        self._main.wait_event(ev)

    def _do_fork(self, n):
        side = self._lanes(n)
        self.flush_reduces()
        ev = torch.cuda.Event()
        ev.record(self._main)
        for i in range(n - 1):
            side[i].wait_event(ev)
        self._forked = n
        self._epoch += 1

    def _do_join(self, n):
        side = self._lanes(n)
        self.flush_reduces()
        for i in range(n - 1):
            ev = torch.cuda.Event()
            ev.record(side[i])
            self._main.wait_event(ev)
        self.set_lane(0)
        self._forked = 0
        if self._merge:
# ... 420 lines not shown
                if xfirst:
                    do_x()
                saved = self._enter_wlane(wpair, id(weight)) if on_wl else None
                if self.rq(weight):
                    g, acc = self.pgrad(weight)
                    self.wgrad(x.data, dy, g, geo, acc,
                               None if xb is None else (xb['mean'], xb['invstd'], xb['bn'].weight.data, xb['bn'].bias.data))
                    self.conv_flops += flops
                if self.rq(bias):
                    do_bias()
                if saved is not None:
                    self.stream = saved
                if not xfirst:
                    do_x()

            def do_bias():
                g, acc = self.pgrad(bias)
                ws = self.ws(self.Q.fami_channel_sum_workspace(Co))
                self.acall('fami_channel_sum', _p(out.grad), N * Ho * Wo, Co, _p(g), acc, _p(ws))

            def do_x(pair=False):
                dy = out.grad
                if x.requires_grad:
                    self.conv_flops += flops
                    gx, acc = self.gbuf(x)
                    wpd = self.packed(weight, 1)
                    rec = x.bnrec
                    pays = False
                    if self.fuse_bn_bwd_auto and rec is not None and (kh, stride, pad, dil) == (3, 1, 1, 1):
                        kind = self.Q.fami_conv_t6_eligible(N, Ho, Wo, Co, Ci)
                        pays = kind in (1, 2) or (kind == 3 and bool(self.fuse_bn_c64 & 2))
                    stats = None
                    if (rec is not None and (self.fuse_bn_bwd or fuse_here or pays) and x.uses == 0 and not x.nofuse and x.lanes is not None
                            and len(x.lanes) == 1 and not x.f32grad):
                        slots = self.zeros_bytes(self.Q.fami_bn_slots_bytes(Ci))
                        stats = (_p(rec['z']), _p(rec['y'] if rec['rmode'] == 1 else None), _p(rec['mean']), _p(rec['invstd']),
                                 _p(rec['gamma']), _p(rec['beta']), rec['rmode'], _p(slots))
                        rec['pre_bwd'] = slots
                        self.nfused['bwd'] += 1
                    xbn_args = None if xb is None else (xb['mean'], xb['invstd'], xb['bn'].weight.data, xb['bn'].bias.data)
                    if pair and (self.half or stats is None):
                        gw, accw = self.pgrad(weight)
                        self.conv_flops += flops
                        self.wgrad_pair(x.data, dy, wpd, gx, acc, gw, accw, geo, stats, xbn_args)
                        return
                    if pair:
                        gw, accw = self.pgrad(weight)
                        self.wgrad(x.data, dy, gw, geo, accw, xbn_args)
                        self.conv_flops += flops
                    if stats is not None:
                        self.acall('fami_conv2d_dgrad_bnstats', _p(dy), _p(wpd), _p(gx), *geo, acc, *stats)
                    elif self.half:
                        self.acall('fami_conv2d_dgrad', _p(dy), _p(wpd), _p(gx), *geo, acc)
                    else:
                        self.call('fami_conv2d_dgrad_f32', _p(dy), _p(wpd), None, _p(gx), *geo, acc)
            self.record_bwd(bwd, [weight, bias], (x,))
        return out

    @staticmethod
    def bn_batch_stats(bn):
        return bn.training and not getattr(bn, 'frozen_stats', False)

    def bn_fusable(self, P, C):
        return C % 4 == 0 and 4 <= C <= 1024 and not self.Q.fami_bn_is_small(P, C)

    def conv_fuses_stats(self, N, Ho, Wo, Ci, Co, kh, st, pd, dl):
        if self.fuse_bn_fwd3:
            kinds = (1, 2, 3) if (self.fuse_bn_c64 & 1) else (1, 2)
            return self.half and (kh, st, pd, dl) == (3, 1, 1, 1) and self.Q.fami_conv_t6_eligible(N, Ho, Wo, Ci, Co) in kinds
        if self.half and not (self.fuse_bn_c64 & 1) and (kh, st, pd, dl) == (3, 1, 1, 1):
            return self.Q.fami_conv_t6_eligible(N, Ho, Wo, Ci, Co) != 3
        return True

    def conv_bn(self, x, conv, bn, relu=False, residual=None):
        N, H, W, _ = x.shape
        Co, _, kh, kw = conv.weight.shape
        st, pd, dl = conv.stride[0], conv.padding[0], conv.dilation[0]
        Ho = (H + 2 * pd - dl * (kh - 1) - 1) // st + 1
        Wo = (W + 2 * pd - dl * (kw - 1) - 1) // st + 1
        if (self.bn_batch_stats(bn) and self.fuse_bn_fwd and self.bn_fusable(N * Ho * Wo, Co)
                and self.conv_fuses_stats(N, Ho, Wo, conv.weight.shape[1], Co, kh, st, pd, dl)):
            slots = self.zeros_bytes(self.Q.fami_bn_slots_bytes(Co))
            z = self.conv(x, conv.weight, conv.bias, st, pd, dl, stats=(slots, bn.running_mean))
            return self.bn(z, bn, relu=relu, residual=residual, pre=slots)
        return self.bn(self.conv(x, conv.weight, conv.bias, st, pd, dl), bn, relu=relu, residual=residual)

    def conv_bn_relu_into(self, x, conv, bn, nxt):
        N, H, W, _ = x.shape
        Co, _, kh, kw = conv.weight.shape
        st, pd, dl = conv.stride[0], conv.padding[0], conv.dilation[0]
        Ho = (H + 2 * pd - dl * (kh - 1) - 1) // st + 1
        Wo = (W + 2 * pd - dl * (kw - 1) - 1) // st + 1
        P = N * Ho * Wo
        okq = self.Q.fami_conv2d_xbn_ok if self.half else self.Q.fami_conv2d_xbn_ok_f32
        ok = (self.use_xbn and self.bn2 and self.defer_reduce and self.bn_batch_stats(bn) and self.fuse_bn_fwd
              and self.defer_bn is None and bn.running_mean is not None and self.bn_fusable(P, Co)
              and tuple(nxt.weight.shape[1:]) == (Co, 3, 3) and nxt.stride[0] == 1 and nxt.padding[0] == 1
              and nxt.dilation[0] == 1 and okq(N, Ho, Wo, Co, nxt.weight.shape[0]))
        if not ok:
            if self.abl_bn1 and self.bn_batch_stats(bn) and self.fuse_bn_fwd and self.bn_fusable(P, Co):
                return self._abl_bn1(x, conv, bn, st, pd, dl, Co)
            if (self.bn_in and self.bn_batch_stats(bn) and self.fuse_bn_fwd and self.bn_fusable(P, Co)
                    and self.conv_fuses_stats(N, Ho, Wo, conv.weight.shape[1], Co, kh, st, pd, dl)
                    and tuple(nxt.weight.shape[1:]) == (Co, 3, 3) and nxt.stride[0] == 1 and nxt.padding[0] == 1
                    and nxt.dilation[0] == 1 and self.Q.fami_conv2d_fwd_bnin_ok(N, Ho, Wo, Co, nxt.weight.shape[0])):
                slots = self.zeros_bytes(self.Q.fami_bn_slots_bytes(Co))
                z = self.conv(x, conv.weight, conv.bias, st, pd, dl, stats=(slots, bn.running_mean))
                return self.bn(z, bn, relu=True, pre=slots, defer=True)
            return self.conv_bn(x, conv, bn, relu=True)
        slots = self.zeros_bytes(self.Q.fami_bn_slots_bytes(Co))
        z = self.conv(x, conv.weight, conv.bias, st, pd, dl, stats=(slots, bn.running_mean))
        self._lane_guard(('running statistics', id(bn)))
        mean, invstd = self.empty(Co), self.empty(Co)
        self.bn_trained.append(bn)
        need_p = self.rq(bn.weight)
        out = T(z.data, z.requires_grad or need_p)
        out.xbn = {'bn': bn, 'slots': slots, 'mean': mean, 'invstd': invstd, 'P': P,
                   'mom': 0.1 if bn.momentum is None else bn.momentum, 'used': False}
        if out.requires_grad:
            def bwd():
                if out.grad is None:
                    return
                gx, accx = self.gbuf(z) if z.requires_grad else (self.act(N, Ho, Wo, Co), 0)
                gg = gb = None
                accp = 0
                if need_p:
                    gg, accp = self.pgrad(bn.weight)
                    gb, _ = self.pgrad(bn.bias)
                self.acall('fami_bn_bwd2', _p(out.grad), _p(z.data), None, _p(mean), _p(invstd), _p(bn.weight.data),
                           _p(bn.bias.data), _p(gx), _p(gg), _p(gb), None, P, Co, 2, accx, accp, 0,
                           _p(self.zeros_bytes(self.Q.fami_bn_slots_bytes(Co))))
            self.record_bwd(bwd, [bn.weight, bn.bias], (z,))
        return out

    _abl_skip = 0

    def _abl_bn1(self, x, conv, bn, st, pd, dl, Co):
        slots = self.zeros_bytes(self.Q.fami_bn_slots_bytes(Co))
        z = self.conv(x, conv.weight, conv.bias, st, pd, dl, stats=(slots, bn.running_mean))
        self._abl_skip = self.abl_bn1
        try:
            y = self.bn(z, bn, relu=True, pre=slots)
        finally:
            self._abl_skip = 0
        return y

    def bn(self, x, bn, relu=False, residual=None, pre=None, defer=False):
        shp = x.shape
        C = shp[-1]
        P = x.data.numel() // C
        mean, invstd = self.empty(C), self.empty(C)
        y = self.like(x.data)
        pending = None
        training = self.bn_batch_stats(bn)
        if training:
            deferred = self.defer_bn is not None and bn.running_mean is not None
            if not deferred:
                self._lane_guard(('running statistics', id(bn)))
            mom = 0.1 if bn.momentum is None else bn.momentum
            bn2 = self.bn2
            if pre is not None and (self._abl_skip & 1):
                y = x.data
                self.call('fami_bn_finalize_slots_f32', _p(pre), P, C, _p(mean), _p(invstd), _p(None if deferred else bn.running_mean),
                          _p(None if deferred else bn.running_var), float(mom), float(bn.eps))
            elif pre is not None and defer and residual is None and relu:
                pending = {'z': x.data, 'y': y, 'slots': pre, 'P': P, 'C': C, 'bn': bn, 'mean': mean, 'invstd': invstd,
                           'rm': None if deferred else bn.running_mean, 'rv': None if deferred else bn.running_var,
                           'mom': float(mom), 'eps': float(bn.eps), 'done': False}
                self._pending.append(pending)
            elif pre is not None:
                self.acall('fami_bn_apply_slots', _p(x.data), _p(None if residual is None else residual.data), _p(y),
                           _p(bn.weight.data), _p(bn.bias.data), _p(mean), _p(invstd),
                           _p(None if deferred else bn.running_mean), _p(None if deferred else bn.running_var), P, C,
                           int(relu), float(mom), float(bn.eps), _p(pre))
            else:
                ws = self.zeros_bytes(self.Q.fami_bn_slots_bytes(C)) if bn2 else self.ws(self.Q.fami_bn_workspace(C))
                self.acall('fami_bn_train_fwd2' if bn2 else 'fami_bn_train_fwd', _p(x.data),
                           _p(None if residual is None else residual.data), _p(y),
                           _p(bn.weight.data), _p(bn.bias.data), _p(mean), _p(invstd),
                           _p(None if deferred else bn.running_mean), _p(None if deferred else bn.running_var), P, C,
                           int(relu), float(mom), float(bn.eps), _p(ws))
            if deferred:
                self.defer_bn.append((bn, mean, invstd, P, float(mom)))
            self.bn_trained.append(bn)
        else:
            assert pre is None
            self.call('fami_bn_eval_stats_f32', _p(bn.running_mean), _p(bn.running_var), _p(mean), _p(invstd), C,
                      float(bn.eps))
            self.acall('fami_bn_apply', _p(x.data), _p(mean), _p(invstd), _p(bn.weight.data), _p(bn.bias.data),
                       _p(None if residual is None else residual.data), _p(y), P, C, int(relu))
        need_p = self.rq(bn.weight)
        rg = x.requires_grad or need_p or (residual is not None and residual.requires_grad)
        out = T(y, rg)
        out.pending = pending
        if rg:
            rmode = (1 if residual is not None else 2) if relu else 0
            rec = None
            if training and self.bn2 and self.bn_fusable(P, C):
                rec = out.bnrec = {'z': x.data, 'y': y, 'mean': mean, 'invstd': invstd, 'gamma': bn.weight.data,
                                   'beta': bn.bias.data, 'rmode': rmode, 'pre_bwd': None}

            abl_bwd = bool(self._abl_skip & 2)
            if abl_bwd:
                rec = out.bnrec = None

            def bwd():
                if out.grad is None:
                    return
                if abl_bwd:
                    if x.requires_grad:
                        x.grad = out.grad
                    return
                gx, accx = self.gbuf(x) if x.requires_grad else (self.act(*shp), 0)
                gg = gb = None
                accp = 0
                if need_p:
                    gg, accp = self.pgrad(bn.weight)
                    gb, _ = self.pgrad(bn.bias)
                gr, accr = (None, 0)
                if residual is not None and residual.requires_grad:
                    gr, accr = self.gbuf(residual)
                if not training:
                    self.acall('fami_bn_eval_bwd', _p(out.grad), _p(x.data), _p(y), _p(mean), _p(invstd),
                               _p(bn.weight.data), _p(gx), _p(gg), _p(gb), _p(gr), P, C, int(relu), accx, accp, accr,
                               _p(self.ws(self.Q.fami_bn_workspace(C)) if need_p else None))
                elif rec is not None and rec['pre_bwd'] is not None:
                    self.acall('fami_bn_bwd_apply_slots', _p(out.grad), _p(x.data), _p(mean), _p(invstd),
                               _p(bn.weight.data), _p(bn.bias.data), _p(gx), _p(gg), _p(gb), _p(gr), P, C, accx, accp,
                               accr, _p(rec['pre_bwd']))
                elif self.bn2:
                    self.acall('fami_bn_bwd2', _p(out.grad), _p(x.data), _p(y), _p(mean), _p(invstd),
                               _p(bn.weight.data), _p(bn.bias.data), _p(gx), _p(gg), _p(gb), _p(gr), P, C, rmode, accx,
                               accp, accr, _p(self.zeros_bytes(self.Q.fami_bn_slots_bytes(C))))
                else:
                    ws = self.ws(self.Q.fami_bn_workspace(C))
                    self.acall('fami_bn_bwd', _p(out.grad), _p(x.data), _p(y), _p(mean), _p(invstd),
                               _p(bn.weight.data), _p(gx), _p(gg), _p(gb), _p(gr), P, C, int(relu), accx, accp, accr,
                               _p(ws))
            self.record_bwd(bwd, [bn.weight, bn.bias], (x, residual))
        return out

    def conv_fuse_term(self, x, conv, bn, shift):
        N, H, W, _ = x.shape
        Co, _, kh, kw = conv.weight.shape
        st, pd, dl = conv.stride[0], conv.padding[0], conv.dilation[0]
        Ho = (H + 2 * pd - dl * (kh - 1) - 1) // st + 1
        Wo = (W + 2 * pd - dl * (kw - 1) - 1) // st + 1
        if (self.bn_batch_stats(bn) and self.fuse_bn_fwd and self.bn_fusable(N * Ho * Wo, Co)
                and self.conv_fuses_stats(N, Ho, Wo, conv.weight.shape[1], Co, kh, st, pd, dl)):
            slots = self.zeros_bytes(self.Q.fami_bn_slots_bytes(Co))
            z = self.conv(x, conv.weight, conv.bias, st, pd, dl, stats=(slots, bn.running_mean))
            return self.fuse_term(z, bn, shift, pre=slots)
        return self.fuse_term(self.conv(x, conv.weight, conv.bias, st, pd, dl), bn, shift)

    def fuse_term(self, x, bn, shift, pre=None):
        C = x.shape[-1]
        h = {'x': x, 'bn': bn, 'shift': shift, 'stats': None, 'out': None}
        if bn is not None:
            Pk = x.data.numel() // C
            mean, invstd = self.empty(C), self.empty(C)
            if self.bn_batch_stats(bn):
                self._lane_guard(('running statistics', id(bn)))
                mom = 0.1 if bn.momentum is None else bn.momentum
                if pre is not None:
                    self.call('fami_bn_finalize_slots_f32', _p(pre), Pk, C, _p(mean), _p(invstd), _p(bn.running_mean),
                              _p(bn.running_var), float(mom), float(bn.eps))
                else:
                    ws = self.ws(self.Q.fami_bn_workspace(C))
                    self.acall('fami_bn_stats', _p(x.data), Pk, C, _p(mean), _p(invstd), _p(bn.running_mean),
                               _p(bn.running_var), float(mom), float(bn.eps), _p(ws))
                self.bn_trained.append(bn)
            else:
                assert pre is None
                self.call('fami_bn_eval_stats_f32', _p(bn.running_mean), _p(bn.running_var), _p(mean), _p(invstd),
                          C, float(bn.eps))
            h['stats'] = (mean, invstd)
        need_p = bn is not None and self.rq(bn.weight)
        training = bn is not None and self.bn_batch_stats(bn)
        if self.record and (x.requires_grad or need_p):
            def bwd():
                out = h['out']
                if out is None or out.grad is None:
                    return
                dy, y = out.grad, out.data
                N, H, W, _ = out.shape
                if bn is None:
                    if x.requires_grad:
                        g, acc = self.gbuf(x)
                        self.acall('fami_relu_bwd', _p(dy), _p(y), _p(g), y.numel(), acc)
                    return
                Pk = x.data.numel() // C
                gx, accx = self.gbuf(x) if x.requires_grad else (self.like(x.data), 0)
                gg = gb = None
                accp = 0
                if need_p:
                    gg, accp = self.pgrad(bn.weight)
                    gb, _ = self.pgrad(bn.bias)
                st = h['stats']
                if not training:
                    ws = self.ws(self.Q.fami_bn_workspace(C)) if need_p else None
                    if shift == 0:
                        self.acall('fami_bn_eval_bwd', _p(dy), _p(x.data), _p(y), _p(st[0]), _p(st[1]),
                                   _p(bn.weight.data), _p(gx), _p(gg), _p(gb), None, Pk, C, 1, accx, accp, 0, _p(ws))
                    else:
                        low = self.like(x.data)
                        self.acall('fami_pool_relu_bwd', _p(dy), _p(y), _p(low), N, H >> shift, W >> shift, C, shift, 1)
                        self.acall('fami_bn_eval_bwd', _p(low), _p(x.data), None, _p(st[0]), _p(st[1]),
                                   _p(bn.weight.data), _p(gx), _p(gg), _p(gb), None, Pk, C, 0, accx, accp, 0, _p(ws))
                    return
                two = self.bn2 and self.bn_fusable(Pk, C)
                ws = self.zeros_bytes(self.Q.fami_bn_slots_bytes(C)) if two else self.ws(self.Q.fami_bn_workspace(C))
                if shift == 0:
                    if two:
                        self.acall('fami_bn_bwd2', _p(dy), _p(x.data), _p(y), _p(st[0]), _p(st[1]), _p(bn.weight.data),
                                   _p(bn.bias.data), _p(gx), _p(gg), _p(gb), None, Pk, C, 1, accx, accp, 0, _p(ws))
                    else:
                        self.acall('fami_bn_bwd', _p(dy), _p(x.data), _p(y), _p(st[0]), _p(st[1]),
                                   _p(bn.weight.data), _p(gx), _p(gg), _p(gb), None, Pk, C, 1, accx, accp, 0, _p(ws))
                else:
                    low = self.like(x.data)
                    self.acall('fami_pool_relu_bwd', _p(dy), _p(y), _p(low), N, H >> shift, W >> shift, C, shift, 1)
                    if two:
                        self.acall('fami_bn_bwd2', _p(low), _p(x.data), None, _p(st[0]), _p(st[1]), _p(bn.weight.data),
                                   _p(bn.bias.data), _p(gx), _p(gg), _p(gb), None, Pk, C, 0, accx, accp, 0, _p(ws))
                    else:
                        self.acall('fami_bn_bwd', _p(low), _p(x.data), None, _p(st[0]), _p(st[1]),
                                   _p(bn.weight.data), _p(gx), _p(gg), _p(gb), None, Pk, C, 0, accx, accp, 0, _p(ws))
            self.record_bwd(bwd, [bn.weight, bn.bias] if bn is not None else [], (x,))
        return h

    def fuse(self, handles):
        k = len(handles)
        assert 1 <= k <= 4
        big = [h for h in handles if h['shift'] == 0][0]['x']
        N, H, W, C = big.shape
        PA = ctypes.c_void_p * k
        xs = PA(*[_p(h['x'].data) for h in handles])
        mean_a = PA(*[None if h['stats'] is None else _p(h['stats'][0]) for h in handles])
        inv_a = PA(*[None if h['stats'] is None else _p(h['stats'][1]) for h in handles])
        gam_a = PA(*[None if h['bn'] is None else _p(h['bn'].weight.data) for h in handles])
        bet_a = PA(*[None if h['bn'] is None else _p(h['bn'].bias.data) for h in handles])
        sh_a = (ctypes.c_int * k)(*[h['shift'] for h in handles])
        y = self.act(N, H, W, C)
        self.acall('fami_fuse_sum', k, xs, mean_a, inv_a, gam_a, bet_a, sh_a, _p(y), N, H, W, C, 1)
        rg = self.record and any(h['x'].requires_grad or (h['bn'] is not None and self.rq(h['bn'].weight)) for h in handles)
        out = T(y, rg)
        for h in handles:
            h['out'] = out
        return out

    def batch_slice(self, x, n0, n1, terminal=False):
        x.nofuse = True
        if x.requires_grad and not terminal and all(x is not p for p in self._sliced):
            self._sliced.append(x)
        return T(x.data[n0:n1], x.requires_grad, parent=x, n0=n0, n1=n1)

    def sub(self, a, b):
        y = self.like(a.data)
        self.acall('fami_axpby', _p(a.data), _p(b.data), _p(y), y.numel(), 1.0, -1.0)
        out = T(y, a.requires_grad or b.requires_grad)
        if out.requires_grad:
            def bwd():
                if out.grad is None:
                    return
                for t, sgn in ((a, 1.0), (b, -1.0)):
                    if t.requires_grad:
                        g, acc = self.gbuf(t)
                        self.acall('fami_axpby', _p(out.grad), _p(g) if acc else None, _p(g), g.numel(), sgn, 1.0)
            self.record_bwd(bwd, (), (a, b))
        return out

    def concat(self, xs):
        N, H, W, _ = xs[0].shape
        Ct = sum(x.shape[3] for x in xs)
        P = N * H * W
        y = self.act(N, H, W, Ct)
        n = len(xs)
        one = 2 <= n <= 4 and all(x.shape[3] % 4 == 0 for x in xs) and len({id(x) for x in xs}) == n
        cs = (ctypes.c_int * 4)(*[x.shape[3] for x in xs]) if one else None
        if one:
            self.acall('fami_concat_channels', (ctypes.c_void_p * 4)(*[x.data.data_ptr() for x in xs]), cs, n, _p(y), P)
        else:
            off = 0
            for x in xs:
                c = x.shape[3]
                self.acall('fami_copy_channels', _p(x.data), _p(y), P, c, 0, Ct, off, c, 0)
                off += c
        out = T(y, any(x.requires_grad for x in xs))
        if out.requires_grad:
            def bwd():
                if out.grad is None:
                    return
                if one:
                    dst, accs = (ctypes.c_void_p * 4)(), (ctypes.c_int * 4)()
                    for k, x in enumerate(xs):
                        if x.requires_grad:
                            g, acc = self.gbuf(x)
                            dst[k], accs[k] = g.data_ptr(), acc
                    self.acall('fami_split_channels', _p(out.grad), dst, cs, accs, n, P)
                    return
                o = 0
                for x in xs:
                    c = x.shape[3]
                    if x.requires_grad:
                        g, acc = self.gbuf(x)
                        self.acall('fami_copy_channels', _p(out.grad), _p(g), P, Ct, o, c, 0, c, acc)
                    o += c
            self.record_bwd(bwd, (), tuple(xs))
        return out

    def flatten_chw(self, x):
        N, H, W, C = x.shape
        y = self.empty(N, C * H * W)
        self.acall('fami_nhwc_to_nchw', _p(x.data), _p(y), N, C, H, W, 0)
        out = T(y, x.requires_grad, f32grad=True)
        if out.requires_grad:
            def bwd():
                if out.grad is None:
                    return
                g, acc = self.gbuf(x)
                if acc:
                    tmp = self.like(g)
                    self.acall('fami_nchw_to_nhwc', _p(out.grad), _p(tmp), N, C, H, W)
                    self.acall('fami_axpby', _p(tmp), _p(g), _p(g), g.numel(), 1.0, 1.0)
                else:
                    self.acall('fami_nchw_to_nhwc', _p(out.grad), _p(g), N, C, H, W)
            self.record_bwd(bwd, (), (x,))
        return out

    def linear(self, x, lin):
        M, K = x.shape
        Nn = lin.out_features
        y = self.empty(M, Nn)
        self.call('fami_linear_fwd_f32', _p(x.data), _p(lin.weight.data), _p(None if lin.bias is None else lin.bias.data),
                  _p(y), M, K, Nn)
        need_p = self.rq(lin.weight)
        out = T(y, x.requires_grad or need_p, f32grad=True)
        if out.requires_grad:
            def bwd():
                if out.grad is None:
                    return
                gx = gw = gb = None
                accx = accp = 0
                if x.requires_grad:
                    gx, accx = self.gbuf(x)
                if need_p:
                    gw, accp = self.pgrad(lin.weight)
                    if lin.bias is not None:
                        gb, _ = self.pgrad(lin.bias)
                self.call('fami_linear_bwd_f32', _p(out.grad), _p(x.data), _p(lin.weight.data), _p(gx), _p(gw),
                          _p(gb), M, K, Nn, accx, accp)
            self.record_bwd(bwd, [lin.weight, lin.bias], (x,))
        return out

    def scale_pairs(self, t, sx, sy):
        B = t.shape[0]
        y = self.empty(B, 2)
        self.call('fami_scale_pairs_f32', _p(t.data), _p(y), B, float(sx), float(sy), 0)
        out = T(y, t.requires_grad, f32grad=True)
        if out.requires_grad:
            def bwd():
                if out.grad is None:
                    return
                g, acc = self.gbuf(t)
                self.call('fami_scale_pairs_f32', _p(out.grad), _p(g), B, float(sx), float(sy), acc)
            self.record_bwd(bwd, (), (t,))
        return out

    def shift(self, x, t, align_corners=True):
        B, H, W, C = x.shape
        if not align_corners:
            t = self.scale_pairs(t, W / max(W - 1, 1), H / max(H - 1, 1))
        y = self.like(x.data)
        self.acall('fami_shift_bilinear_fwd', _p(x.data), _p(t.data), _p(y), B, H, W, C)
        out = T(y, x.requires_grad or t.requires_grad)
        if out.requires_grad:
            def bwd():
                if out.grad is None:
                    return
                gs = gt = None
                accs = acct = 0
                if x.requires_grad:
                    gs, accs = self.gbuf(x)
                if t.requires_grad:
                    gt, acct = self.gbuf(t)
                ws = self.ws(self.Q.fami_shift_workspace(B))
                self.acall('fami_shift_bilinear_bwd', _p(out.grad), _p(x.data), _p(t.data), _p(gs), _p(gt), B, H,
                           W, C, accs, acct, _p(ws))
            self.record_bwd(bwd, (), (x, t))
        return out

    def dcn(self, x, off, msk, weight, bias, G, pad=3, dil=3):
        om = msk is None
        B, H, W, C = x.shape
        Co, _, kh, kw = weight.shape
        K = kh * kw
        wp = (getattr(self, 'prepacked_dcn_fwd', None) or {}).get(id(weight))
        if wp is not None:
            ev = getattr(self, 'dcn_fwd_ready', None)
            if ev is not None:
                self.wait_main(ev)
# ... 141 lines not shown
```

fami-pose_amd/options.py:

```python
import os

SWITCHES = {
    'FAMI_LANES': ('1', 'independent sub-graphs (the parallel HRNet branches) on side streams between fork / join; 0: everything on one stream (debug)'),
    'FAMI_DEBUG_STREAMS': ('', 'print the stream handles of every lane set-up'),
    'FAMI_FUSE_BN': ('auto', "BatchNorm statistics in the neighbouring convolutions' epilogues: auto (f32: forward everywhere; 16-bit: forward in the DMA-staged 3x3 kernels only + backward where the input gradient runs on one) | autoall (16-bit: forward everywhere) | 0 | fwd | fwd3 | bwd | bwdauto | 1"),
    'FAMI_BN_IN': ('1', 'conv1 -> bn1 -> ReLU -> conv2 (16-bit storage): bn1\'s apply pass inside conv2\'s launch where the weight-resident 48-channel kernel takes conv2 (fami_conv2d_fwd_bnin_*)'),
    'FAMI_XBN': (None, 'BatchNorm + ReLU applied by the consumer convolution; default on in f32 storage, off in the 16-bit modes'),
    'FAMI_MERGE_PREDICTORS': ('1', 'offset + mask predictor of a DCN layer as one 48 -> 324 convolution (needs the Trainer arena)'),
    'FAMI_DETERMINISTIC': ('0', 'run-to-run reproducible kernels (fixed-point DCN input gradient, three-launch BatchNorm)'),
    'FAMI_DDP_PLAN': ('overlap', 'data-parallel launch plan: overlap (graph segments + all-reduce between them) | serial'),
    'FAMI_DDP_GRAPH': ('1', '0: eager launches with the all-reduce fired from the backward hooks'),
    'FAMI_DDP_ALGO': ('ring', 'ring (one all_reduce per slice) | mesh (reduce_scatter_tensor -> all_gather_into_tensor)'),
    'FAMI_DDP_PAYLOAD': ('f32', 'gradient bytes on the wire: f32 | bf16 | f16 (the arena, the 1/world scale and Adam stay fp32)'),
    'FAMI_F32_SPLIT': ('1', 'f32 3x3 convolutions as exact three-term bf16 splits on the matrix pipe; 0 = exact-f32 MFMA'),
    'FAMI_T5': ('1', 'A/B: 0 = the band kernel instead of the persistent split-product kernel'),
    'FAMI_T5_WG': ('', 'A/B: workgroups of the persistent grid / 8'),
    'FAMI_WG16_TARGET': ('', 'A/B: workgroup target of the pipelined 16-bit weight-gradient kernel'),
    'FAMI_WGS3_TARGET': ('', 'A/B: workgroup target of the split-product weight-gradient kernel'),
    'FAMI_ALLOW_WRONG': ('', '1: allow the ablation switches below'),
    'FAMI_T5_ABL': ('', 'upper bound: n channel chunks per split-product convolution'),
    'FAMI_ABL_WGRAD': ('0', 'upper bound: no weight-gradient kernels at all'),
    'FAMI_ABL_LANES': ('0', 'critical-path probe: bit i = every launch enqueued on stream lane i is skipped (what the step costs without that branch)'),
    'FAMI_ABL_BN1': ('0', 'upper bound: bit 1 no apply pass / bit 2 no backward of every conv1 -> bn1 -> ReLU -> conv2 BatchNorm'),
}
WRONG = ('FAMI_T5_ABL', 'FAMI_ABL_WGRAD', 'FAMI_ABL_LANES', 'FAMI_ABL_BN1')


def get(name, default=None):
    if name not in SWITCHES:
        raise KeyError('%s is not a registered switch (fami_pose_amd/options.py)' % name)
    v = os.environ.get(name)
    if v is None or v == '':
        reg = SWITCHES[name][0]
        return default if (default is not None or reg is None) else reg
    if name in WRONG and v != '0' and os.environ.get('FAMI_ALLOW_WRONG') != '1':
        raise RuntimeError('%s set: this switch skips work and produces WRONG results (measurement ablation only); '
                           'set FAMI_ALLOW_WRONG=1 to run it on purpose' % name)
    return v


def flag(name, default=None):
    v = get(name, default)
    return v not in (None, '', '0')


def number(name, default=None):
    v = get(name, default)
    return int(v) if v not in (None, '') else None


def describe():
    return '\n'.join('%-24s %-8s %s' % (k, 'mode' if d is None else (d or '-'), m) for k, (d, m) in SWITCHES.items())
```

include/fami.h:

```cpp
#ifndef FAMI_H
#define FAMI_H
#ifdef __cplusplus
extern "C" {
#endif

typedef void* fami_stream_t;

#include "fami_route.h"
long fami_route_size(void);
int fami_route_init(fami_route_t* route);
int fami_route_bind(fami_route_t* route);

const char* fami_version(void);
const char* fami_last_error(void);
int fami_device_info(int device, int* info, char* name, int name_len);

int fami_conv_tune(int mt, int nt, int ks);
int fami_conv_tune_lds(int on);
int fami_conv_tune_wgrad_lds(int on);
int fami_conv_tune_xcd(int mode);
int fami_conv_tune_stages(int stages);
int fami_tune_reset(void);
int fami_tune_defaults(int f32_split);
int fami_conv_t5_eligible(int N, int H, int W, int Ci, int Co);
// ... 332 lines not shown
int fami_relu_bwd_bf16(const fami_bf16_t* dy, const fami_bf16_t* y, fami_bf16_t* dx, long n, int accumulate,
                       fami_stream_t stream);
int fami_pool_relu_bwd_bf16(const fami_bf16_t* dy, const fami_bf16_t* y, fami_bf16_t* out, int N, int Hl, int Wl,
                            int C, int shift, int relu, fami_stream_t stream);

int fami_shift_bilinear_fwd_bf16(const fami_bf16_t* src, const float* t, fami_bf16_t* out, int B, int H, int W, int C,
                                 fami_stream_t stream);
int fami_shift_bilinear_bwd_bf16(const fami_bf16_t* gout, const fami_bf16_t* src, const float* t, fami_bf16_t* gsrc,
                                 float* gt, int B, int H, int W, int C, int acc_src, int acc_t, float* ws,
                                 fami_stream_t stream);
int fami_dcn_fwd_bf16(const fami_bf16_t* x, const fami_bf16_t* off, const fami_bf16_t* msk, const float* wp,
                      const float* bias, fami_bf16_t* y, int B, int H, int W, int C, int Co, int G, int kh, int kw,
                      int stride, int pad, int dil, fami_stream_t stream);
int fami_dcn_bwd_bf16(const fami_bf16_t* x, const fami_bf16_t* off, const fami_bf16_t* msk, const fami_bf16_t* dy,
                      const float* wpb, fami_bf16_t* col, float* gx, fami_bf16_t* goff, fami_bf16_t* gmsk, int B,
                      int H, int W, int C, int Co, int G, int kh, int kw, int stride, int pad, int dil, int acc_off,
                      fami_stream_t stream);
int fami_dcn_bwd_det_bf16(const fami_bf16_t* x, const fami_bf16_t* off, const fami_bf16_t* msk, const fami_bf16_t* dy, const float* wpb, fami_bf16_t* col,
                         fami_bf16_t* gx, fami_bf16_t* goff, fami_bf16_t* gmsk, int B, int H, int W, int C, int Co, int G, int kh, int kw,
                         int stride, int pad, int dil, int acc_off, int acc_x, void* ws, fami_stream_t stream);
int fami_dcn_fwd_om_bf16(const fami_bf16_t* x, const fami_bf16_t* om, const float* wp, const float* bias, fami_bf16_t* y, int B, int H, int W,
                       int C, int Co, int G, int kh, int kw, int stride, int pad, int dil, fami_stream_t stream);
int fami_dcn_bwd_om_bf16(const fami_bf16_t* x, const fami_bf16_t* om, const fami_bf16_t* dy, const float* wpb, fami_bf16_t* col, float* gx, fami_bf16_t* gom,
                       int B, int H, int W, int C, int Co, int G, int kh, int kw, int stride, int pad, int dil, int acc_om,
                       fami_stream_t stream);
int fami_dcn_bwd_det_om_bf16(const fami_bf16_t* x, const fami_bf16_t* om, const fami_bf16_t* dy, const float* wpb, fami_bf16_t* col, fami_bf16_t* gx,
                           fami_bf16_t* gom, int B, int H, int W, int C, int Co, int G, int kh, int kw, int stride, int pad,
                           int dil, int acc_om, int acc_x, void* ws, fami_stream_t stream);


typedef unsigned short fami_f16_t;

long fami_packed_weight_elems_f16(int Co, int Ci, int kh, int kw, int mode);
int fami_pack_conv_weight_f16(const float* w_oihw, fami_f16_t* wp, int Co, int Ci, int kh, int kw, int mode,
                               fami_stream_t stream);
int fami_pack_conv_weights_batch_f16(const float* params, fami_f16_t* packed, const void* desc, int n,
                                      fami_stream_t stream);
int fami_conv2d_fwd_f16(const fami_f16_t* x, const fami_f16_t* wp, const float* bias, void* y, int N, int H, int W,
                         int Ci, int Co, int kh, int kw, int stride, int pad, int dil, int relu, int accumulate,
                         int out_f32, fami_stream_t stream);
int fami_conv2d_dgrad_f16(const fami_f16_t* dy, const fami_f16_t* wp, fami_f16_t* dx, int N, int H, int W, int Ci,
                           int Co, int kh, int kw, int stride, int pad, int dil, int accumulate,
                           fami_stream_t stream);
int fami_conv2d_fwd_xbn_f16(const fami_f16_t* z, const fami_f16_t* wp, const float* bias, fami_f16_t* y, int N, int H, int W,
                             int Ci, int Co, void* slots, const float* pivot_src, const void* xslots, long xP,
                             const float* xgamma, const float* xbeta, float* xmean, float* xinvstd,
                             float* xrunning_mean, float* xrunning_var, float xmomentum, float xeps, fami_stream_t stream);
int fami_conv2d_fwd_bnin_f16(const fami_f16_t* z, const fami_f16_t* wp, const float* bias, fami_f16_t* y, fami_f16_t* a_out, int N, int H, int W,
                              int Ci, int Co, void* slots, const float* pivot_src, const void* xslots, long xP,
                              const float* xgamma, const float* xbeta, float* xmean, float* xinvstd,
                              float* xrunning_mean, float* xrunning_var, float xmomentum, float xeps, fami_stream_t stream);
int fami_conv2d_wgrad_defer_xbn_f16(const fami_f16_t* z, const fami_f16_t* dy, float* dw, float* workspace, long ws_bytes,
                                     int N, int H, int W, int Ci, int Co, int accumulate, long* desc_out,
                                     const float* xmean, const float* xinvstd, const float* xgamma, const float* xbeta,
                                     fami_stream_t stream);
int fami_conv2d_fwd_stats_f16(const fami_f16_t* x, const fami_f16_t* wp, const float* bias, fami_f16_t* y, int N, int H, int W,
                               int Ci, int Co, int kh, int kw, int stride, int pad, int dil, void* slots,
                               const float* pivot_src, fami_stream_t stream);
int fami_conv2d_dgrad_bnstats_f16(const fami_f16_t* dy, const fami_f16_t* wp, fami_f16_t* dx, int N, int H, int W, int Ci,
                                   int Co, int kh, int kw, int stride, int pad, int dil, int accumulate,
                                   const fami_f16_t* z, const fami_f16_t* yrelu, const float* mean, const float* invstd,
                                   const float* gamma, const float* beta, int relu, void* slots, fami_stream_t stream);
int fami_conv2d_bwd_pair_f16(const fami_f16_t* x, const fami_f16_t* dy, const fami_f16_t* wpd, fami_f16_t* dx, float* dw, float* workspace,
                              long ws_bytes, int N, int H, int W, int Ci, int Co, int kh, int kw, int stride, int pad,
                              int dil, int acc_dx, int acc_dw, long* desc_out, const fami_f16_t* z, const fami_f16_t* yrelu,
                              const float* mean, const float* invstd, const float* gamma, const float* beta, int relu,
                              void* slots, fami_stream_t stream);
int fami_bn_apply_slots_f16(const fami_f16_t* x, const fami_f16_t* residual, fami_f16_t* y, const float* gamma,
                             const float* beta, float* mean, float* invstd, float* running_mean, float* running_var,
                             long P, int C, int relu, float momentum, float eps, void* slots, fami_stream_t stream);
int fami_bn_bwd_apply_slots_f16(const fami_f16_t* dz, const fami_f16_t* x, const float* mean, const float* invstd,
                                 const float* gamma, const float* beta, fami_f16_t* dx, float* dgamma, float* dbeta,
                                 fami_f16_t* dres, long P, int C, int acc_dx, int acc_param, int acc_dres, void* slots,
                                 fami_stream_t stream);
int fami_conv2d_wgrad_defer_f16(const fami_f16_t* x, const fami_f16_t* dy, float* dw, float* workspace, long ws_bytes,
                                 int N, int H, int W, int Ci, int Co, int kh, int kw, int stride, int pad, int dil,
                                 int accumulate, long* desc_out, fami_stream_t stream);
int fami_conv2d_wgrad_f16(const fami_f16_t* x, const fami_f16_t* dy, float* dw, float* workspace, long ws_bytes,
                           int N, int H, int W, int Ci, int Co, int kh, int kw, int stride, int pad, int dil,
                           int accumulate, fami_stream_t stream);

int fami_bn_stats_f16(const fami_f16_t* x, long P, int C, float* mean, float* invstd, float* running_mean,
                       float* running_var, float momentum, float eps, float* ws, fami_stream_t stream);
int fami_bn_train_fwd_f16(const fami_f16_t* x, const fami_f16_t* residual, fami_f16_t* y, const float* gamma,
                           const float* beta, float* mean, float* invstd, float* running_mean, float* running_var,
                           long P, int C, int relu, float momentum, float eps, float* ws, fami_stream_t stream);
int fami_bn_apply_f16(const fami_f16_t* x, const float* mean, const float* invstd, const float* gamma,
                       const float* beta, const fami_f16_t* residual, fami_f16_t* y, long P, int C, int relu,
                       fami_stream_t stream);
int fami_bn_train_fwd2_f16(const fami_f16_t* x, const fami_f16_t* residual, fami_f16_t* y, const float* gamma, const float* beta,
                           float* mean, float* invstd, float* running_mean, float* running_var, long P, int C,
                           int relu, float momentum, float eps, void* slots, fami_stream_t stream);
int fami_bn_bwd2_f16(const fami_f16_t* dy, const fami_f16_t* x, const fami_f16_t* y, const float* mean, const float* invstd,
                     const float* gamma, const float* beta, fami_f16_t* dx, float* dgamma, float* dbeta, fami_f16_t* dres, long P,
                     int C, int relu, int acc_dx, int acc_param, int acc_dres, void* slots, fami_stream_t stream);
int fami_bn_bwd_f16(const fami_f16_t* dy, const fami_f16_t* x, const fami_f16_t* y, const float* mean,
                     const float* invstd, const float* gamma, fami_f16_t* dx, float* dgamma, float* dbeta,
                     fami_f16_t* dres, long P, int C, int relu, int acc_dx, int acc_param, int acc_dres, float* ws,
                     fami_stream_t stream);
int fami_bn_eval_bwd_f16(const fami_f16_t* dy, const fami_f16_t* x, const fami_f16_t* y, const float* mean,
                     const float* invstd, const float* gamma, fami_f16_t* dx, float* dgamma, float* dbeta,
                     fami_f16_t* dres, long P, int C, int relu, int acc_dx, int acc_param, int acc_dres, float* ws,
                     fami_stream_t stream);
int fami_channel_sum_f16(const fami_f16_t* x, long P, int C, float* out, int accumulate, float* ws,
                          fami_stream_t stream);

int fami_nchw_to_nhwc_f16(const float* src, fami_f16_t* dst, int N, int C, int H, int W, fami_stream_t stream);
int fami_nhwc_to_nchw_f16(const fami_f16_t* src, float* dst, int N, int C, int H, int W, int accumulate,
                           fami_stream_t stream);
int fami_pack_frames_f16(const float* kf_nchw, const float* sup_nchw, fami_f16_t* frames_nhwc, int B, int S, int H,
                          int W, fami_stream_t stream);
int fami_copy_channels_f16(const fami_f16_t* src, fami_f16_t* dst, long P, int Cs, int src_off, int Cd,
                            int dst_off, int Cc, int accumulate, fami_stream_t stream);
int fami_concat_channels_f16(const fami_f16_t* const* src, const int* c, int n, fami_f16_t* dst, long P, fami_stream_t stream);
int fami_split_channels_f16(const fami_f16_t* src, fami_f16_t* const* dst, const int* c, const int* accumulate, int n, long P,
                             fami_stream_t stream);
int fami_axpby_f16(const fami_f16_t* a, const fami_f16_t* b, fami_f16_t* out, long n, float alpha, float beta,
                    fami_stream_t stream);
int fami_widen_f16(const fami_f16_t* src, float* dst, long n, fami_stream_t stream);
int fami_cast_add_f16(const float* src, fami_f16_t* dst, long n, int accumulate, fami_stream_t stream);
int fami_fill_f16(fami_f16_t* out, long n, float v, fami_stream_t stream);
int fami_fuse_sum_f16(int nterms, const fami_f16_t* const* x, const float* const* mean, const float* const* invstd,
                       const float* const* gamma, const float* const* beta, const int* shift, fami_f16_t* y, int N,
                       int H, int W, int C, int relu, fami_stream_t stream);
int fami_relu_bwd_f16(const fami_f16_t* dy, const fami_f16_t* y, fami_f16_t* dx, long n, int accumulate,
                       fami_stream_t stream);
int fami_pool_relu_bwd_f16(const fami_f16_t* dy, const fami_f16_t* y, fami_f16_t* out, int N, int Hl, int Wl,
                            int C, int shift, int relu, fami_stream_t stream);

int fami_shift_bilinear_fwd_f16(const fami_f16_t* src, const float* t, fami_f16_t* out, int B, int H, int W, int C,
                                 fami_stream_t stream);
int fami_shift_bilinear_bwd_f16(const fami_f16_t* gout, const fami_f16_t* src, const float* t, fami_f16_t* gsrc,
                                 float* gt, int B, int H, int W, int C, int acc_src, int acc_t, float* ws,
                                 fami_stream_t stream);
int fami_dcn_fwd_f16(const fami_f16_t* x, const fami_f16_t* off, const fami_f16_t* msk, const float* wp,
                      const float* bias, fami_f16_t* y, int B, int H, int W, int C, int Co, int G, int kh, int kw,
                      int stride, int pad, int dil, fami_stream_t stream);
int fami_dcn_bwd_f16(const fami_f16_t* x, const fami_f16_t* off, const fami_f16_t* msk, const fami_f16_t* dy,
                      const float* wpb, fami_f16_t* col, float* gx, fami_f16_t* goff, fami_f16_t* gmsk, int B,
                      int H, int W, int C, int Co, int G, int kh, int kw, int stride, int pad, int dil, int acc_off,
                      fami_stream_t stream);
int fami_dcn_bwd_det_f16(const fami_f16_t* x, const fami_f16_t* off, const fami_f16_t* msk, const fami_f16_t* dy, const float* wpb, fami_f16_t* col,
                         fami_f16_t* gx, fami_f16_t* goff, fami_f16_t* gmsk, int B, int H, int W, int C, int Co, int G, int kh, int kw,
                         int stride, int pad, int dil, int acc_off, int acc_x, void* ws, fami_stream_t stream);
int fami_dcn_fwd_om_f16(const fami_f16_t* x, const fami_f16_t* om, const float* wp, const float* bias, fami_f16_t* y, int B, int H, int W,
                       int C, int Co, int G, int kh, int kw, int stride, int pad, int dil, fami_stream_t stream);
int fami_dcn_bwd_om_f16(const fami_f16_t* x, const fami_f16_t* om, const fami_f16_t* dy, const float* wpb, fami_f16_t* col, float* gx, fami_f16_t* gom,
                       int B, int H, int W, int C, int Co, int G, int kh, int kw, int stride, int pad, int dil, int acc_om,
                       fami_stream_t stream);
int fami_dcn_bwd_det_om_f16(const fami_f16_t* x, const fami_f16_t* om, const fami_f16_t* dy, const float* wpb, fami_f16_t* col, fami_f16_t* gx,
                           fami_f16_t* gom, int B, int H, int W, int C, int Co, int G, int kh, int kw, int stride, int pad,
                           int dil, int acc_om, int acc_x, void* ws, fami_stream_t stream);

#ifdef __cplusplus
}
#endif
#endif
```

Baseline: 91.40.

## Store ReLU masks as bytes and read them in backward instead of y

BatchNorm+residual+ReLU and the fuse-sum kernels now write a one-byte ReLU mask per 4-channel vector. The backward kernels (relu_bwd, pool_relu_bwd, BN bwd partial/apply) read that byte instead of reloading the 16-byte f32 y vector. This cuts backward memory traffic and may let y be freed or not kept. The cost is an extra mask write in the forward pass, added buffers, and more API surface. It is on by default for f32 storage.

```diff
diff --git a/fami-pose_amd/csrc/elementwise.hip b/fami-pose_amd/csrc/elementwise.hip
--- a/fami-pose_amd/csrc/elementwise.hip
+++ b/fami-pose_amd/csrc/elementwise.hip
@@ -1,4 +1,5 @@
 #include "common.h"
+#include "relu_mask.h"
 
 template <typename T>
 __global__ void nchw_to_nhwc_kernel(const float* __restrict__ src, T* __restrict__ dst, int N, int C, int H, int W) {
@@ -188,8 +189,8 @@
 };
 
 template <typename T>
-__global__ __launch_bounds__(256) void fuse_sum_kernel(FuseArgs<T> a, T* __restrict__ y, int N, int H, int W, int C,
-                                                       int relu) {
+__global__ __launch_bounds__(256) void fuse_sum_kernel(FuseArgs<T> a, T* __restrict__ y, unsigned char* __restrict__ mask,
+                                                       int N, int H, int W, int C, int relu) {
   const int CV = C >> 2;
   const long total = (long)N * H * W * CV;
   for (long i = blockIdx.x * (long)blockDim.x + threadIdx.x; i < total; i += (long)gridDim.x * blockDim.x) {
@@ -218,26 +219,33 @@
     if (relu) {
 #pragma unroll
       for (int t = 0; t < 4; ++t) acc[t] = fmaxf(acc[t], 0.f);
+      if (mask) mask[i] = relu_mask_byte<T>(acc);
     }
     st4(y + i * 4, acc);
   }
 }
 
 template <typename T>
-__global__ void relu_bwd_kernel(const T* __restrict__ dy, const T* __restrict__ y, T* dx, long n4, int accumulate) {
+__global__ void relu_bwd_kernel(const T* __restrict__ dy, const T* __restrict__ y, const unsigned char* __restrict__ mask,
+                                T* dx, long n4, int accumulate) {
   for (long i = blockIdx.x * (long)blockDim.x + threadIdx.x; i < n4; i += (long)gridDim.x * blockDim.x) {
     f32x4 g = ld4(dy + i * 4);
-    const f32x4 yy = ld4(y + i * 4);
+    if (mask) {
+      g = relu_mask_apply(g, mask[i]);
+    } else {
+      const f32x4 yy = ld4(y + i * 4);
 #pragma unroll
-    for (int t = 0; t < 4; ++t) g[t] = yy[t] > 0.f ? g[t] : 0.f;
+      for (int t = 0; t < 4; ++t) g[t] = yy[t] > 0.f ? g[t] : 0.f;
+    }
     if (accumulate) g += ld4(dx + i * 4);
     st4(dx + i * 4, g);
   }
 }
 
 template <typename T>
-__global__ void pool_relu_bwd_kernel(const T* __restrict__ dy, const T* __restrict__ y, T* __restrict__ out, int N,
-                                     int Hl, int Wl, int C, int s, int relu) {
+__global__ void pool_relu_bwd_kernel(const T* __restrict__ dy, const T* __restrict__ y,
+                                     const unsigned char* __restrict__ mask, T* __restrict__ out, int N, int Hl, int Wl,
+                                     int C, int s, int relu) {
   const int CV = C >> 2;
   const int f = 1 << s;
   const int H = Hl << s, W = Wl << s;
@@ -254,7 +262,9 @@
       for (int dw = 0; dw < f; ++dw) {
         const long o = ((n * H + (hl * f + dh)) * W + (wl * f + dw)) * C + cv * 4;
         f32x4 g = ld4(dy + o);
-        if (relu) {
+        if (relu && mask) {
+          g = relu_mask_apply(g, mask[o >> 2]);
+        } else if (relu) {
           const f32x4 yy = ld4(y + o);
 #pragma unroll
           for (int t = 0; t < 4; ++t) g[t] = yy[t] > 0.f ? g[t] : 0.f;
@@ -390,8 +400,8 @@
 }
 template <typename T>
 static int fuse_sum_impl(int nterms, const T* const* x, const float* const* mean, const float* const* invstd,
-                         const float* const* gamma, const float* const* beta, const int* shift, T* y, int N, int H,
-                         int W, int C, int relu, hipStream_t s, const char* nm) {
+                         const float* const* gamma, const float* const* beta, const int* shift, T* y, unsigned char* mask,
+                         int N, int H, int W, int C, int relu, hipStream_t s, const char* nm) {
   FAMI_REQUIRE(nterms >= 1 && nterms <= 4 && x && shift && y && (C % 4) == 0, nm, "bad argument");
   FuseArgs<T> a;
   a.nterms = nterms;
@@ -407,22 +417,23 @@
       FAMI_REQUIRE(a.x[k] && a.shift[k] >= 0 && (H % (1 << a.shift[k])) == 0 && (W % (1 << a.shift[k])) == 0, nm, "bad term");
     }
   }
-  hipLaunchKernelGGL(fuse_sum_kernel<T>, dim3(fami_ew_grid((long)N * H * W * (C / 4))), dim3(256), 0, s, a, y, N, H, W, C, relu);
-  FAMI_CHECK_LAUNCH(nm);
-  return FAMI_OK;
-}
-template <typename T>
-static int relu_bwd_impl(const T* dy, const T* y, T* dx, long n, int accumulate, hipStream_t s, const char* nm) {
-  FAMI_REQUIRE(dy && y && dx && n > 0 && (n % 4) == 0, nm, "bad argument");
-  hipLaunchKernelGGL(relu_bwd_kernel<T>, dim3(fami_ew_grid(n / 4)), dim3(256), 0, s, dy, y, dx, n / 4, accumulate);
-  FAMI_CHECK_LAUNCH(nm);
-  return FAMI_OK;
-}
-template <typename T>
-static int pool_relu_bwd_impl(const T* dy, const T* y, T* out, int N, int Hl, int Wl, int C, int shift, int relu,
-                              hipStream_t s, const char* nm) {
-  FAMI_REQUIRE(dy && out && (!relu || y) && (C % 4) == 0 && shift >= 0 && shift <= 4, nm, "bad argument");
-  hipLaunchKernelGGL(pool_relu_bwd_kernel<T>, dim3(fami_ew_grid((long)N * Hl * Wl * (C / 4))), dim3(256), 0, s, dy, y, out, N, Hl, Wl, C, shift, relu);
+  hipLaunchKernelGGL(fuse_sum_kernel<T>, dim3(fami_ew_grid((long)N * H * W * (C / 4))), dim3(256), 0, s, a, y, mask, N, H, W, C, relu);
+  FAMI_CHECK_LAUNCH(nm);
+  return FAMI_OK;
+}
+template <typename T>
+static int relu_bwd_impl(const T* dy, const T* y, const unsigned char* mask, T* dx, long n, int accumulate, hipStream_t s,
+                         const char* nm) {
+  FAMI_REQUIRE(dy && (y || mask) && dx && n > 0 && (n % 4) == 0, nm, "bad argument");
+  hipLaunchKernelGGL(relu_bwd_kernel<T>, dim3(fami_ew_grid(n / 4)), dim3(256), 0, s, dy, y, mask, dx, n / 4, accumulate);
+  FAMI_CHECK_LAUNCH(nm);
+  return FAMI_OK;
+}
+template <typename T>
+static int pool_relu_bwd_impl(const T* dy, const T* y, const unsigned char* mask, T* out, int N, int Hl, int Wl, int C,
+                              int shift, int relu, hipStream_t s, const char* nm) {
+  FAMI_REQUIRE(dy && out && (!relu || y || mask) && (C % 4) == 0 && shift >= 0 && shift <= 4, nm, "bad argument");
+  hipLaunchKernelGGL(pool_relu_bwd_kernel<T>, dim3(fami_ew_grid((long)N * Hl * Wl * (C / 4))), dim3(256), 0, s, dy, y, mask, out, N, Hl, Wl, C, shift, relu);
   FAMI_CHECK_LAUNCH(nm);
   return FAMI_OK;
 }
@@ -479,15 +490,38 @@
   int fami_fuse_sum_##sfx(int nterms, const T* const* x, const float* const* mean, const float* const* invstd,         \
                           const float* const* gamma, const float* const* beta, const int* shift, T* y, int N, int H,   \
                           int W, int C, int relu, hipStream_t s) {                                                     \
-    return fuse_sum_impl<T>(nterms, x, mean, invstd, gamma, beta, shift, y, N, H, W, C, relu, s, "fami_fuse_sum_" #sfx);\
+    return fuse_sum_impl<T>(nterms, x, mean, invstd, gamma, beta, shift, y, nullptr, N, H, W, C, relu, s,              \
+                            "fami_fuse_sum_" #sfx);                                                                    \
+  }                                                                                                                    \
+   \
+  int fami_fuse_sum_mask_##sfx(int nterms, const T* const* x, const float* const* mean, const float* const* invstd,    \
+                               const float* const* gamma, const float* const* beta, const int* shift, T* y,            \
+                               unsigned char* mask, int N, int H, int W, int C, int relu, hipStream_t s) {             \
+    FAMI_REQUIRE(!relu || mask, "fami_fuse_sum_mask_" #sfx, "relu needs the mask bytes");                              \
+    return fuse_sum_impl<T>(nterms, x, mean, invstd, gamma, beta, shift, y, mask, N, H, W, C, relu, s,                 \
+                            "fami_fuse_sum_mask_" #sfx);                                                               \
   }                                                                                                                    \
   int fami_relu_bwd_##sfx(const T* dy, const T* y, T* dx, long n, int accumulate, hipStream_t s) {                     \
-    return relu_bwd_impl<T>(dy, y, dx, n, accumulate, s, "fami_relu_bwd_" #sfx);                                       \
+    FAMI_REQUIRE(y, "fami_relu_bwd_" #sfx, "bad argument");                                                            \
+    return relu_bwd_impl<T>(dy, y, nullptr, dx, n, accumulate, s, "fami_relu_bwd_" #sfx);                              \
+  }                                                                                                                    \
+                        \
+  int fami_relu_bwd_mask_##sfx(const T* dy, const unsigned char* mask, T* dx, long n, int accumulate, hipStream_t s) { \
+    FAMI_REQUIRE(mask, "fami_relu_bwd_mask_" #sfx, "null mask");                                                       \
+    return relu_bwd_impl<T>(dy, (const T*)nullptr, mask, dx, n, accumulate, s, "fami_relu_bwd_mask_" #sfx);            \
   }                                                                                                                    \
                                                                      \
   int fami_pool_relu_bwd_##sfx(const T* dy, const T* y, T* out, int N, int Hl, int Wl, int C, int shift, int relu,     \
                                hipStream_t s) {                                                                        \
-    return pool_relu_bwd_impl<T>(dy, y, out, N, Hl, Wl, C, shift, relu, s, "fami_pool_relu_bwd_" #sfx);                \
+    FAMI_REQUIRE(!relu || y, "fami_pool_relu_bwd_" #sfx, "bad argument");                                              \
+    return pool_relu_bwd_impl<T>(dy, y, nullptr, out, N, Hl, Wl, C, shift, relu, s, "fami_pool_relu_bwd_" #sfx);       \
+  }                                                                                                                    \
+                       \
+  int fami_pool_relu_bwd_mask_##sfx(const T* dy, const unsigned char* mask, T* out, int N, int Hl, int Wl, int C,      \
+                                    int shift, int relu, hipStream_t s) {                                              \
+    FAMI_REQUIRE(!relu || mask, "fami_pool_relu_bwd_mask_" #sfx, "relu needs the mask bytes");                         \
+    return pool_relu_bwd_impl<T>(dy, (const T*)nullptr, mask, out, N, Hl, Wl, C, shift, relu, s,                       \
+                                 "fami_pool_relu_bwd_mask_" #sfx);                                                     \
   }
 FAMI_EW_ABI(f32, float)
 FAMI_EW_ABI(bf16, bf16_t)
diff --git a/fami-pose_amd/csrc/norm.hip b/fami-pose_amd/csrc/norm.hip
--- a/fami-pose_amd/csrc/norm.hip
+++ b/fami-pose_amd/csrc/norm.hip
@@ -1,4 +1,5 @@
 #include "common.h"
+#include "relu_mask.h"
 
 #define BN_MAXG 512
 #ifndef BN_U
@@ -165,7 +166,7 @@
                                                        const float* __restrict__ gamma,
                                                        const float* __restrict__ beta,
                                                        const T* __restrict__ residual, T* __restrict__ y,
-                                                       long P, int C, int relu) {
+                                                       unsigned char* __restrict__ mask, long P, int C, int relu) {
   const ColMap m = col_map(C);
   if (!m.active) return;
   f32x4 sc, sf;
@@ -182,6 +183,7 @@
     if (relu) {
 #pragma unroll
       for (int t = 0; t < 4; ++t) v[t] = fmaxf(v[t], 0.f);
+      if (mask) mask[o >> 2] = relu_mask_byte<T>(v);
     }
     st4(y + o, v);
   }
@@ -191,6 +193,7 @@
 __global__ __launch_bounds__(256) void bn_bwd_partial_kernel(const T* __restrict__ dy,
                                                              const T* __restrict__ x,
                                                              const T* __restrict__ y,
+                                                             const unsigned char* __restrict__ mask,
                                                              const float* __restrict__ mean,
                                                              const float* __restrict__ invstd,
                                                              float* __restrict__ partial, long P, int C, int relu) {
@@ -214,7 +217,11 @@
         o[u] = (pu < P ? pu : p) * C + m.cv * 4;
         g[u] = ld4(dy + o[u]);
       }
-      if (relu) {
+      unsigned mb[BN_U] = {};
+      if (relu == 3) {
+#pragma unroll
+        for (int u = 0; u < BN_U; ++u) mb[u] = mask[o[u] >> 2];
+      } else if (relu) {
 #pragma unroll
         for (int u = 0; u < BN_U; ++u) yy[u] = ld4(y + o[u]);
       }
@@ -222,7 +229,9 @@
       for (int u = 0; u < BN_U; ++u) xx[u] = ld4(x + o[u]);
 #pragma unroll
       for (int u = 0; u < BN_U; ++u) {
-        if (relu) {
+        if (relu == 3) {
+          g[u] = relu_mask_apply(g[u], mb[u]);
+        } else if (relu) {
 #pragma unroll
           for (int t = 0; t < 4; ++t) g[u][t] = yy[u][t] > 0.f ? g[u][t] : 0.f;
         }
@@ -270,6 +279,7 @@
 template <typename T>
 __global__ __launch_bounds__(256) void bn_bwd_apply_kernel(const T* __restrict__ dy, const T* __restrict__ x,
                                                            const T* __restrict__ y,
+                                                           const unsigned char* __restrict__ mask,
                                                            const float* __restrict__ mean,
                                                            const float* __restrict__ invstd,
                                                            const float* __restrict__ gamma,
@@ -291,7 +301,9 @@
   for (long p = (long)blockIdx.x * m.rows + m.prow; p < P; p += (long)gridDim.x * m.rows) {
     const long o = p * C + m.cv * 4;
     f32x4 g = ld4(dy + o);
-    if (relu) {
+    if (relu == 3) {
+      g = relu_mask_apply(g, mask[o >> 2]);
+    } else if (relu) {
       const f32x4 yy = ld4(y + o);
 #pragma unroll
       for (int t = 0; t < 4; ++t) g[t] = yy[t] > 0.f ? g[t] : 0.f;
@@ -447,6 +459,7 @@
 __global__ __launch_bounds__(256) void bn_apply2_kernel(const T* __restrict__ x, const double* __restrict__ slots, int NS,
                                                         const float* __restrict__ gamma, const float* __restrict__ beta,
                                                         const T* __restrict__ residual, T* __restrict__ y,
+                                                        unsigned char* __restrict__ mask,
                                                         float* __restrict__ mean, float* __restrict__ invstd,
                                                         float* running_mean, float* running_var, long P, int C,
                                                         int relu, float momentum, float eps, const float* pivot) {
@@ -492,12 +505,14 @@
     if (relu) {
 #pragma unroll
       for (int t = 0; t < 4; ++t) v[t] = fmaxf(v[t], 0.f);
+      if (mask) mask[o >> 2] = relu_mask_byte<T>(v);
     }
     st4(y + o, v);
   }
 }
 
-__device__ __forceinline__ f32x4 bn_relu_mask(f32x4 g, int relu, f32x4 yy, f32x4 xv, f32x4 sc, f32x4 sf) {
+__device__ __forceinline__ f32x4 bn_relu_mask(f32x4 g, int relu, f32x4 yy, f32x4 xv, f32x4 sc, f32x4 sf, unsigned mb) {
+  if (relu == 3) return relu_mask_apply(g, mb);
   if (relu == 1) {
 #pragma unroll
     for (int t = 0; t < 4; ++t) g[t] = yy[t] > 0.f ? g[t] : 0.f;
@@ -510,7 +525,9 @@
 
 template <typename T>
 __global__ __launch_bounds__(256) void bn_bwd_partial2_kernel(const T* __restrict__ dy, const T* __restrict__ x,
-                                                              const T* __restrict__ y, const float* __restrict__ mean,
+                                                              const T* __restrict__ y,
+                                                              const unsigned char* __restrict__ mask,
+                                                              const float* __restrict__ mean,
                                                               const float* __restrict__ invstd,
                                                               const float* __restrict__ gamma,
                                                               const float* __restrict__ beta,
@@ -540,15 +557,19 @@
         o[u] = (pu < P ? pu : p) * C + m.cv * 4;
         g[u] = ld4(dy + o[u]);
       }
+      unsigned mb[BN_U] = {};
       if (relu == 1) {
 #pragma unroll
         for (int u = 0; u < BN_U; ++u) yy[u] = ld4(y + o[u]);
+      } else if (relu == 3) {
+#pragma unroll
+        for (int u = 0; u < BN_U; ++u) mb[u] = mask[o[u] >> 2];
       }
 #pragma unroll
       for (int u = 0; u < BN_U; ++u) xx[u] = ld4(x + o[u]);
 #pragma unroll
       for (int u = 0; u < BN_U; ++u) {
-        g[u] = bn_relu_mask(g[u], relu, yy[u], xx[u], sc, sf);
+        g[u] = bn_relu_mask(g[u], relu, yy[u], xx[u], sc, sf, mb[u]);
         if (p + u * step >= P) g[u] = f32x4{0.f, 0.f, 0.f, 0.f};
         const f32x4 xh = (xx[u] - mu) * is;
         s += g[u];
@@ -573,7 +594,9 @@
 
 template <typename T>
 __global__ __launch_bounds__(256) void bn_bwd_apply2_kernel(const T* __restrict__ dy, const T* __restrict__ x,
-                                                            const T* __restrict__ y, const float* __restrict__ mean,
+                                                            const T* __restrict__ y,
+                                                            const unsigned char* __restrict__ mask,
+                                                            const float* __restrict__ mean,
                                                             const float* __restrict__ invstd,
                                                             const float* __restrict__ gamma,
                                                             const float* __restrict__ beta,
@@ -615,8 +638,10 @@
     f32x4 g = ld4(dy + o);
     const f32x4 xv = ld4(x + o);
     f32x4 yy = {0.f, 0.f, 0.f, 0.f};
+    unsigned mb = 0u;
     if (relu == 1) yy = ld4(y + o);
-    g = bn_relu_mask(g, relu, yy, xv, sc, sf);
+    else if (relu == 3) mb = mask[o >> 2];
+    g = bn_relu_mask(g, relu, yy, xv, sc, sf, mb);
     const f32x4 xh = (xv - mu) * is;
     f32x4 d = gi * (g - c1 - xh * c2);
     if (acc_dx) d += ld4(dx + o);
@@ -860,7 +885,8 @@
 
 template <typename T>
 static int bn_apply_impl(const T* x, const float* mean, const float* invstd, const float* gamma, const float* beta,
-                         const T* residual, T* y, long P, int C, int relu, hipStream_t s, const char* nm) {
+                         const T* residual, T* y, unsigned char* mask, long P, int C, int relu, hipStream_t s,
+                         const char* nm) {
   FAMI_REQUIRE(x && mean && invstd && gamma && beta && y, nm, "null pointer");
   if (!bn_shape_ok(P, C)) {
     fami_set_error(nm, "C must be a multiple of 4, <= 1024");
@@ -869,25 +895,28 @@
   const int rows = 256 / (C >> 2);
   long g = (P + rows - 1) / rows;
   if (g > 2048) g = 2048;
-  hipLaunchKernelGGL(bn_apply_kernel<T>, dim3((int)g), dim3(256), 0, s, x, mean, invstd, gamma, beta, residual, y, P,
-                     C, relu);
+  hipLaunchKernelGGL(bn_apply_kernel<T>, dim3((int)g), dim3(256), 0, s, x, mean, invstd, gamma, beta, residual, y,
+                     mask, P, C, relu);
   FAMI_CHECK_LAUNCH(nm);
   return FAMI_OK;
 }
 
 template <typename T>
-static int bn_bwd_impl(const T* dy, const T* x, const T* y, const float* mean, const float* invstd,
-                       const float* gamma, T* dx, float* dgamma, float* dbeta, T* dres, long P, int C, int relu,
-                       int acc_dx, int acc_param, int acc_dres, float* ws, hipStream_t s, const char* nm) {
+static int bn_bwd_impl(const T* dy, const T* x, const T* y, const unsigned char* mask, const float* mean,
+                       const float* invstd, const float* gamma, T* dx, float* dgamma, float* dbeta, T* dres, long P, int C,
+                       int relu, int acc_dx, int acc_param, int acc_dres, float* ws, hipStream_t s, const char* nm) {
   FAMI_REQUIRE(dy && x && mean && invstd && gamma && dx && ws, nm, "null pointer");
-  FAMI_REQUIRE(!relu || y, nm, "relu needs y");
+  FAMI_REQUIRE(relu != 3 || mask, nm, "relu = 3 needs the mask bytes");
+  if (relu != 0 && relu != 3) relu = 1;
+  const bool small = bn_small_ok(P, C);
+  FAMI_REQUIRE(!relu || y || (relu == 3 && !small), nm, "relu needs y");
   if (!bn_shape_ok(P, C)) {
     fami_set_error(nm, "C must be a multiple of 4, <= 1024");
     return FAMI_ESHAPE;
   }
-  if (bn_small_ok(P, C)) {
+  if (small) {
     hipLaunchKernelGGL(bn_small_bwd_kernel<T>, dim3(C / 4), dim3(256), 0, s, dy, x, y, mean, invstd, gamma, dx, dgamma,
-                       dbeta, dres, P, C, relu, acc_dx, acc_param, acc_dres);
+                       dbeta, dres, P, C, relu ? 1 : 0, acc_dx, acc_param, acc_dres);
     FAMI_CHECK_LAUNCH(nm);
     return FAMI_OK;
   }
@@ -896,14 +925,14 @@
   float* coef = ws + (long)BN_MAXG * 2 * C - 2 * C;
   const int Gp = G < BN_MAXG ? G : BN_MAXG - 1;
   hipLaunchKernelGGL(bn_bwd_partial_kernel<T>, dim3(Gp), dim3(256), (size_t)rows * 2 * C * sizeof(float), s, dy, x, y,
-                     mean, invstd, ws, P, C, relu);
+                     mask, mean, invstd, ws, P, C, relu);
   FAMI_CHECK_LAUNCH(nm);
   hipLaunchKernelGGL(bn_bwd_finalize_kernel, dim3(C), dim3(256), 0, s, ws, Gp, P, C, coef, dgamma, dbeta, acc_param);
   FAMI_CHECK_LAUNCH(nm);
   long g = (P + rows - 1) / rows;
   if (g > 2048) g = 2048;
-  hipLaunchKernelGGL(bn_bwd_apply_kernel<T>, dim3((int)g), dim3(256), 0, s, dy, x, y, mean, invstd, gamma, coef, dx,
-                     dres, P, C, relu, acc_dx, acc_dres);
+  hipLaunchKernelGGL(bn_bwd_apply_kernel<T>, dim3((int)g), dim3(256), 0, s, dy, x, y, mask, mean, invstd, gamma, coef,
+                     dx, dres, P, C, relu, acc_dx, acc_dres);
   FAMI_CHECK_LAUNCH(nm);
   return FAMI_OK;
 }
@@ -939,8 +968,8 @@
 }
 
 template <typename T>
-static int bn_train_fwd_impl(const T* x, const T* residual, T* y, const float* gamma, const float* beta, float* mean,
-                             float* invstd, float* running_mean, float* running_var, long P, int C, int relu,
+static int bn_train_fwd_impl(const T* x, const T* residual, T* y, unsigned char* mask, const float* gamma, const float* beta,
+                             float* mean, float* invstd, float* running_mean, float* running_var, long P, int C, int relu,
                              float momentum, float eps, float* ws, hipStream_t s, const char* nm) {
   FAMI_REQUIRE(x && y && gamma && beta && mean && invstd && ws, nm, "null pointer");
   if (!bn_shape_ok(P, C)) {
@@ -955,7 +984,7 @@
   }
   int rc = bn_stats_impl<T>(x, P, C, mean, invstd, running_mean, running_var, momentum, eps, ws, s, nm);
   if (rc != FAMI_OK) return rc;
-  return bn_apply_impl<T>(x, mean, invstd, gamma, beta, residual, y, P, C, relu, s, nm);
+  return bn_apply_impl<T>(x, mean, invstd, gamma, beta, residual, y, mask, P, C, relu, s, nm);
 }
 
 static inline int bn_apply_grid(long P, int C) {
@@ -966,9 +995,10 @@
 }
 
 template <typename T>
-static int bn_train_fwd2_impl(const T* x, const T* residual, T* y, const float* gamma, const float* beta, float* mean,
-                              float* invstd, float* running_mean, float* running_var, long P, int C, int relu,
-                              float momentum, float eps, void* slots, int pre, hipStream_t s, const char* nm) {
+static int bn_train_fwd2_impl(const T* x, const T* residual, T* y, unsigned char* mask, const float* gamma,
+                              const float* beta, float* mean, float* invstd, float* running_mean, float* running_var, long P,
+                              int C, int relu, float momentum, float eps, void* slots, int pre, hipStream_t s,
+                              const char* nm) {
   FAMI_REQUIRE(x && y && gamma && beta && mean && invstd && slots, nm, "null pointer");
   if (!bn_shape_ok(P, C)) {
     fami_set_error(nm, "C must be a multiple of 4, <= 1024");
@@ -988,25 +1018,31 @@
     FAMI_CHECK_LAUNCH(nm);
   }
   hipLaunchKernelGGL(bn_apply2_kernel<T>, dim3(bn_apply_grid(P, C)), dim3(256), (size_t)2 * C * sizeof(float), s, x,
-                     reinterpret_cast<const double*>(slots), NS, gamma, beta, residual, y, mean, invstd, running_mean,
-                     running_var, P, C, relu, momentum, eps, pre ? bn_slots_pivot(slots, C) : (const float*)nullptr);
+                     reinterpret_cast<const double*>(slots), NS, gamma, beta, residual, y, mask, mean, invstd,
+                     running_mean, running_var, P, C, relu, momentum, eps, pre ? bn_slots_pivot(slots, C) : (const float*)nullptr);
   FAMI_CHECK_LAUNCH(nm);
   return FAMI_OK;
 }
 
 template <typename T>
-static int bn_bwd2_impl(const T* dy, const T* x, const T* y, const float* mean, const float* invstd, const float* gamma,
-                        const float* beta, T* dx, float* dgamma, float* dbeta, T* dres, long P, int C, int relu,
-                        int acc_dx, int acc_param, int acc_dres, void* slots, int pre, hipStream_t s, const char* nm) {
+static int bn_bwd2_impl(const T* dy, const T* x, const T* y, const unsigned char* mask, bool mask_abi, const float* mean,
+                        const float* invstd, const float* gamma, const float* beta, T* dx, float* dgamma, float* dbeta,
+                        T* dres, long P, int C, int relu, int acc_dx, int acc_param, int acc_dres, void* slots, int pre,
+                        hipStream_t s, const char* nm) {
   FAMI_REQUIRE(dy && x && mean && invstd && gamma && beta && dx && slots, nm, "null pointer");
   FAMI_REQUIRE(relu != 1 || y, nm, "relu = 1 needs y");
-  FAMI_REQUIRE(relu >= 0 && relu <= 2, nm, "relu must be 0, 1 (mask from y) or 2 (mask recomputed from x)");
+  if (mask_abi) {
+    FAMI_REQUIRE(relu >= 0 && relu <= 3, nm, "relu must be 0, 1 (mask from y), 2 (mask recomputed from x) or 3 (mask bytes)");
+    FAMI_REQUIRE(relu != 3 || mask, nm, "relu = 3 needs the mask bytes");
+  } else {
+    FAMI_REQUIRE(relu >= 0 && relu <= 2, nm, "relu must be 0, 1 (mask from y) or 2 (mask recomputed from x)");
+  }
   if (!bn_shape_ok(P, C)) {
     fami_set_error(nm, "C must be a multiple of 4, <= 1024");
     return FAMI_ESHAPE;
   }
   if (bn_small_ok(P, C) && !pre) {
-    FAMI_REQUIRE(relu != 2 || y, nm, "small tensors take the ReLU mask from y");
+    FAMI_REQUIRE(relu < 2 || y, nm, "small tensors take the ReLU mask from y");
     hipLaunchKernelGGL(bn_small_bwd_kernel<T>, dim3(C / 4), dim3(256), 0, s, dy, x, y, mean, invstd, gamma, dx, dgamma,
                        dbeta, dres, P, C, relu ? 1 : 0, acc_dx, acc_param, acc_dres);
     FAMI_CHECK_LAUNCH(nm);
@@ -1015,13 +1051,13 @@
   const int G = bn_grid2(P, C, (int)sizeof(T)), NS = bn_slots(C);
   const int rows = 256 / (C >> 2);
   if (!pre) {
-    hipLaunchKernelGGL(bn_bwd_partial2_kernel<T>, dim3(G), dim3(256), (size_t)rows * 2 * C * sizeof(float), s, dy, x, y, mean,
-                       invstd, gamma, beta, reinterpret_cast<double*>(slots), NS, P, C, relu);
+    hipLaunchKernelGGL(bn_bwd_partial2_kernel<T>, dim3(G), dim3(256), (size_t)rows * 2 * C * sizeof(float), s, dy, x, y, mask,
+                       mean, invstd, gamma, beta, reinterpret_cast<double*>(slots), NS, P, C, relu);
     FAMI_CHECK_LAUNCH(nm);
   }
   hipLaunchKernelGGL(bn_bwd_apply2_kernel<T>, dim3(bn_apply_grid(P, C)), dim3(256), (size_t)2 * C * sizeof(float), s, dy, x,
-                     y, mean, invstd, gamma, beta, reinterpret_cast<const double*>(slots), NS, dx, dgamma, dbeta, dres, P,
-                     C, relu, acc_dx, acc_param, acc_dres);
+                     y, mask, mean, invstd, gamma, beta, reinterpret_cast<const double*>(slots), NS, dx, dgamma, dbeta, dres,
+                     P, C, relu, acc_dx, acc_param, acc_dres);
   FAMI_CHECK_LAUNCH(nm);
   return FAMI_OK;
 }
@@ -1119,14 +1155,23 @@
   }                                                                                                                    \
   int fami_bn_apply_##sfx(const T* x, const float* mean, const float* invstd, const float* gamma, const float* beta,   \
                           const T* residual, T* y, long P, int C, int relu, hipStream_t s) {                           \
-    return bn_apply_impl<T>(x, mean, invstd, gamma, beta, residual, y, P, C, relu, s, "fami_bn_apply_" #sfx);          \
+    return bn_apply_impl<T>(x, mean, invstd, gamma, beta, residual, y, nullptr, P, C, relu, s, "fami_bn_apply_" #sfx); \
   }                                                                                                                    \
                      \
   int fami_bn_bwd_##sfx(const T* dy, const T* x, const T* y, const float* mean, const float* invstd,                   \
                         const float* gamma, T* dx, float* dgamma, float* dbeta, T* dres, long P, int C, int relu,      \
                         int acc_dx, int acc_param, int acc_dres, float* ws, hipStream_t s) {                           \
-    return bn_bwd_impl<T>(dy, x, y, mean, invstd, gamma, dx, dgamma, dbeta, dres, P, C, relu, acc_dx, acc_param,       \
-                          acc_dres, ws, s, "fami_bn_bwd_" #sfx);                                                       \
+    return bn_bwd_impl<T>(dy, x, y, nullptr, mean, invstd, gamma, dx, dgamma, dbeta, dres, P, C, relu ? 1 : 0, acc_dx, \
+                          acc_param, acc_dres, ws, s, "fami_bn_bwd_" #sfx);                                            \
+  }                                                                                                                    \
+   \
+   \
+  int fami_bn_bwd_mask_##sfx(const T* dy, const T* x, const T* y, const unsigned char* mask, const float* mean,        \
+                             const float* invstd, const float* gamma, T* dx, float* dgamma, float* dbeta, T* dres,     \
+                             long P, int C, int relu, int acc_dx, int acc_param, int acc_dres, float* ws,              \
+                             hipStream_t s) {                                                                          \
+    return bn_bwd_impl<T>(dy, x, y, mask, mean, invstd, gamma, dx, dgamma, dbeta, dres, P, C, relu, acc_dx, acc_param, \
+                          acc_dres, ws, s, "fami_bn_bwd_mask_" #sfx);                                                  \
   }                                                                                                                    \
    \
    \
@@ -1140,8 +1185,18 @@
   int fami_bn_train_fwd_##sfx(const T* x, const T* residual, T* y, const float* gamma, const float* beta,              \
                               float* mean, float* invstd, float* running_mean, float* running_var, long P, int C,      \
                               int relu, float momentum, float eps, float* ws, hipStream_t s) {                         \
-    return bn_train_fwd_impl<T>(x, residual, y, gamma, beta, mean, invstd, running_mean, running_var, P, C, relu,      \
-                                momentum, eps, ws, s, "fami_bn_train_fwd_" #sfx);                                      \
+    return bn_train_fwd_impl<T>(x, residual, y, nullptr, gamma, beta, mean, invstd, running_mean, running_var, P, C,   \
+                                relu, momentum, eps, ws, s, "fami_bn_train_fwd_" #sfx);                                \
+  }                                                                                                                    \
+   \
+   \
+  int fami_bn_train_fwd_mask_##sfx(const T* x, const T* residual, T* y, unsigned char* mask, const float* gamma,       \
+                                   const float* beta, float* mean, float* invstd, float* running_mean,                 \
+                                   float* running_var, long P, int C, int relu, float momentum, float eps, float* ws,  \
+                                   hipStream_t s) {                                                                    \
+    FAMI_REQUIRE(!relu || mask, "fami_bn_train_fwd_mask_" #sfx, "relu needs the mask bytes");                          \
+    return bn_train_fwd_impl<T>(x, residual, y, mask, gamma, beta, mean, invstd, running_mean, running_var, P, C,      \
+                                relu, momentum, eps, ws, s, "fami_bn_train_fwd_mask_" #sfx);                           \
   }                                                                                                                    \
    \
    \
@@ -1149,15 +1204,31 @@
   int fami_bn_train_fwd2_##sfx(const T* x, const T* residual, T* y, const float* gamma, const float* beta,             \
                                float* mean, float* invstd, float* running_mean, float* running_var, long P, int C,     \
                                int relu, float momentum, float eps, void* slots, hipStream_t s) {                      \
-    return bn_train_fwd2_impl<T>(x, residual, y, gamma, beta, mean, invstd, running_mean, running_var, P, C, relu,     \
-                                 momentum, eps, slots, 0, s, "fami_bn_train_fwd2_" #sfx);                              \
+    return bn_train_fwd2_impl<T>(x, residual, y, nullptr, gamma, beta, mean, invstd, running_mean, running_var, P, C,  \
+                                 relu, momentum, eps, slots, 0, s, "fami_bn_train_fwd2_" #sfx);                        \
+  }                                                                                                                    \
+  int fami_bn_train_fwd2_mask_##sfx(const T* x, const T* residual, T* y, unsigned char* mask, const float* gamma,      \
+                                    const float* beta, float* mean, float* invstd, float* running_mean,                \
+                                    float* running_var, long P, int C, int relu, float momentum, float eps,            \
+                                    void* slots, hipStream_t s) {                                                      \
+    FAMI_REQUIRE(!relu || mask, "fami_bn_train_fwd2_mask_" #sfx, "relu needs the mask bytes");                         \
+    return bn_train_fwd2_impl<T>(x, residual, y, mask, gamma, beta, mean, invstd, running_mean, running_var, P, C,     \
+                                 relu, momentum, eps, slots, 0, s, "fami_bn_train_fwd2_mask_" #sfx);                   \
   }                                                                                                                    \
     \
   int fami_bn_apply_slots_##sfx(const T* x, const T* residual, T* y, const float* gamma, const float* beta,            \
                                 float* mean, float* invstd, float* running_mean, float* running_var, long P, int C,    \
                                 int relu, float momentum, float eps, void* slots, hipStream_t s) {                     \
-    return bn_train_fwd2_impl<T>(x, residual, y, gamma, beta, mean, invstd, running_mean, running_var, P, C, relu,     \
-                                 momentum, eps, slots, 1, s, "fami_bn_apply_slots_" #sfx);                             \
+    return bn_train_fwd2_impl<T>(x, residual, y, nullptr, gamma, beta, mean, invstd, running_mean, running_var, P, C,  \
+                                 relu, momentum, eps, slots, 1, s, "fami_bn_apply_slots_" #sfx);                       \
+  }                                                                                                                    \
+  int fami_bn_apply_slots_mask_##sfx(const T* x, const T* residual, T* y, unsigned char* mask, const float* gamma,     \
+                                     const float* beta, float* mean, float* invstd, float* running_mean,               \
+                                     float* running_var, long P, int C, int relu, float momentum, float eps,           \
+                                     void* slots, hipStream_t s) {                                                     \
+    FAMI_REQUIRE(!relu || mask, "fami_bn_apply_slots_mask_" #sfx, "relu needs the mask bytes");                        \
+    return bn_train_fwd2_impl<T>(x, residual, y, mask, gamma, beta, mean, invstd, running_mean, running_var, P, C,     \
+                                 relu, momentum, eps, slots, 1, s, "fami_bn_apply_slots_mask_" #sfx);                  \
   }                                                                                                                    \
   \
   \
@@ -1165,14 +1236,22 @@
                                     const float* gamma, const float* beta, T* dx, float* dgamma, float* dbeta,         \
                                     T* dres, long P, int C, int acc_dx, int acc_param, int acc_dres, void* slots,      \
                                     hipStream_t s) {                                                                   \
-    return bn_bwd2_impl<T>(dz, x, (const T*)nullptr, mean, invstd, gamma, beta, dx, dgamma, dbeta, dres, P, C, 0,      \
-                           acc_dx, acc_param, acc_dres, slots, 1, s, "fami_bn_bwd_apply_slots_" #sfx);                 \
+    return bn_bwd2_impl<T>(dz, x, (const T*)nullptr, nullptr, false, mean, invstd, gamma, beta, dx, dgamma, dbeta,     \
+                           dres, P, C, 0, acc_dx, acc_param, acc_dres, slots, 1, s, "fami_bn_bwd_apply_slots_" #sfx);  \
   }                                                                                                                    \
   int fami_bn_bwd2_##sfx(const T* dy, const T* x, const T* y, const float* mean, const float* invstd,                  \
                          const float* gamma, const float* beta, T* dx, float* dgamma, float* dbeta, T* dres, long P,   \
                          int C, int relu, int acc_dx, int acc_param, int acc_dres, void* slots, hipStream_t s) {       \
-    return bn_bwd2_impl<T>(dy, x, y, mean, invstd, gamma, beta, dx, dgamma, dbeta, dres, P, C, relu, acc_dx,           \
-                           acc_param, acc_dres, slots, 0, s, "fami_bn_bwd2_" #sfx);                                    \
+    return bn_bwd2_impl<T>(dy, x, y, nullptr, false, mean, invstd, gamma, beta, dx, dgamma, dbeta, dres, P, C, relu,   \
+                           acc_dx, acc_param, acc_dres, slots, 0, s, "fami_bn_bwd2_" #sfx);                            \
+  }                                                                                                                    \
+   \
+  int fami_bn_bwd2_mask_##sfx(const T* dy, const T* x, const T* y, const unsigned char* mask, const float* mean,       \
+                              const float* invstd, const float* gamma, const float* beta, T* dx, float* dgamma,        \
+                              float* dbeta, T* dres, long P, int C, int relu, int acc_dx, int acc_param, int acc_dres, \
+                              void* slots, hipStream_t s) {                                                            \
+    return bn_bwd2_impl<T>(dy, x, y, mask, true, mean, invstd, gamma, beta, dx, dgamma, dbeta, dres, P, C, relu,       \
+                           acc_dx, acc_param, acc_dres, slots, 0, s, "fami_bn_bwd2_mask_" #sfx);                       \
   }                                                                                                                    \
                                                                         \
   int fami_channel_sum_##sfx(const T* x, long P, int C, float* out, int accumulate, float* ws, hipStream_t s) {        \
diff --git a/fami-pose_amd/csrc/relu_mask.h b/fami-pose_amd/csrc/relu_mask.h
--- /dev/null
+++ b/fami-pose_amd/csrc/relu_mask.h
@@ -0,0 +1,20 @@
+#pragma once
+#include "common.h"
+
+template <typename T>
+__device__ __forceinline__ unsigned char relu_mask_byte(f32x4 v) {
+  if constexpr (sizeof(T) == 2) {
+    typedef T tx4 __attribute__((ext_vector_type(4)));
+    v = __builtin_convertvector(__builtin_convertvector(v, tx4), f32x4);
+  }
+  unsigned m = 0u;
+#pragma unroll
+  for (int t = 0; t < 4; ++t) m |= (v[t] > 0.f ? 1u : 0u) << t;
+  return (unsigned char)m;
+}
+
+__device__ __forceinline__ f32x4 relu_mask_apply(f32x4 g, unsigned m) {
+#pragma unroll
+  for (int t = 0; t < 4; ++t) g[t] = ((m >> t) & 1u) ? g[t] : 0.f;
+  return g;
+}
diff --git a/fami-pose_amd/engine.py b/fami-pose_amd/engine.py
--- a/fami-pose_amd/engine.py
+++ b/fami-pose_amd/engine.py
@@ -136,6 +136,7 @@
         self._sliced = []
         self._keep = []
         self.bn2 = not self.deterministic
+        self.relu_mask = options.flag('FAMI_RELU_MASK', '0' if self.half else '1')
         fz = options.get('FAMI_FUSE_BN', 'auto')
         self.fuse_bn_fwd = self.bn2 and fz in ('1', 'fwd', 'auto', 'autoall', 'fwd3')
         self.fuse_bn_fwd3 = fz == 'fwd3' or (fz == 'auto' and self.half)
@@ -862,6 +863,8 @@
         mean, invstd = self.empty(C), self.empty(C)
         y = self.like(x.data)
         pending = None
+        mk = None
+        mka = ()
         training = self.bn_batch_stats(bn)
         if training:
             deferred = self.defer_bn is not None and bn.running_mean is not None
@@ -869,6 +872,9 @@
                 self._lane_guard(('running statistics', id(bn)))
             mom = 0.1 if bn.momentum is None else bn.momentum
             bn2 = self.bn2
+            if relu and residual is not None and self.relu_mask and not (pre is not None and (self._abl_skip & 1)):
+                mk = self.empty(P * C // 4, dtype=torch.uint8)
+            mka = () if mk is None else (_p(mk),)
             if pre is not None and (self._abl_skip & 1):
                 y = x.data
                 self.call('fami_bn_finalize_slots_f32', _p(pre), P, C, _p(mean), _p(invstd), _p(None if deferred else bn.running_mean),
@@ -879,14 +885,14 @@
                            'mom': float(mom), 'eps': float(bn.eps), 'done': False}
                 self._pending.append(pending)
             elif pre is not None:
-                self.acall('fami_bn_apply_slots', _p(x.data), _p(None if residual is None else residual.data), _p(y),
-                           _p(bn.weight.data), _p(bn.bias.data), _p(mean), _p(invstd),
+                self.acall('fami_bn_apply_slots' + ('' if mk is None else '_mask'), _p(x.data),
+                           _p(None if residual is None else residual.data), _p(y), *mka, _p(bn.weight.data), _p(bn.bias.data), _p(mean), _p(invstd),
                            _p(None if deferred else bn.running_mean), _p(None if deferred else bn.running_var), P, C,
                            int(relu), float(mom), float(bn.eps), _p(pre))
             else:
                 ws = self.zeros_bytes(self.Q.fami_bn_slots_bytes(C)) if bn2 else self.ws(self.Q.fami_bn_workspace(C))
-                self.acall('fami_bn_train_fwd2' if bn2 else 'fami_bn_train_fwd', _p(x.data),
-                           _p(None if residual is None else residual.data), _p(y),
+                self.acall(('fami_bn_train_fwd2' if bn2 else 'fami_bn_train_fwd') + ('' if mk is None else '_mask'), _p(x.data),
+                           _p(None if residual is None else residual.data), _p(y), *mka,
                            _p(bn.weight.data), _p(bn.bias.data), _p(mean), _p(invstd),
                            _p(None if deferred else bn.running_mean), _p(None if deferred else bn.running_var), P, C,
                            int(relu), float(mom), float(bn.eps), _p(ws))
@@ -939,14 +945,15 @@
                                _p(bn.weight.data), _p(bn.bias.data), _p(gx), _p(gg), _p(gb), _p(gr), P, C, accx, accp,
                                accr, _p(rec['pre_bwd']))
                 elif self.bn2:
-                    self.acall('fami_bn_bwd2', _p(out.grad), _p(x.data), _p(y), _p(mean), _p(invstd),
-                               _p(bn.weight.data), _p(bn.bias.data), _p(gx), _p(gg), _p(gb), _p(gr), P, C, rmode, accx,
-                               accp, accr, _p(self.zeros_bytes(self.Q.fami_bn_slots_bytes(C))))
+                    self.acall('fami_bn_bwd2' + ('' if mk is None else '_mask'), _p(out.grad), _p(x.data), _p(y), *mka,
+                               _p(mean), _p(invstd), _p(bn.weight.data), _p(bn.bias.data), _p(gx), _p(gg), _p(gb), _p(gr),
+                               P, C, rmode if mk is None else 3, accx, accp, accr,
+                               _p(self.zeros_bytes(self.Q.fami_bn_slots_bytes(C))))
                 else:
                     ws = self.ws(self.Q.fami_bn_workspace(C))
-                    self.acall('fami_bn_bwd', _p(out.grad), _p(x.data), _p(y), _p(mean), _p(invstd),
-                               _p(bn.weight.data), _p(gx), _p(gg), _p(gb), _p(gr), P, C, int(relu), accx, accp, accr,
-                               _p(ws))
+                    self.acall('fami_bn_bwd' + ('' if mk is None else '_mask'), _p(out.grad), _p(x.data), _p(y), *mka,
+                               _p(mean), _p(invstd), _p(bn.weight.data), _p(gx), _p(gg), _p(gb), _p(gr), P, C,
+                               int(relu) if mk is None else 3, accx, accp, accr, _p(ws))
             self.record_bwd(bwd, [bn.weight, bn.bias], (x, residual))
         return out
 
@@ -965,7 +972,7 @@
 
     def fuse_term(self, x, bn, shift, pre=None):
         C = x.shape[-1]
-        h = {'x': x, 'bn': bn, 'shift': shift, 'stats': None, 'out': None}
+        h = {'x': x, 'bn': bn, 'shift': shift, 'stats': None, 'out': None, 'mask': None}
         if bn is not None:
             Pk = x.data.numel() // C
             mean, invstd = self.empty(C), self.empty(C)
@@ -993,11 +1000,16 @@
                 if out is None or out.grad is None:
                     return
                 dy, y = out.grad, out.data
+                mk = h['mask']
+                mka = () if mk is None else (_p(mk),)
                 N, H, W, _ = out.shape
                 if bn is None:
                     if x.requires_grad:
                         g, acc = self.gbuf(x)
-                        self.acall('fami_relu_bwd', _p(dy), _p(y), _p(g), y.numel(), acc)
+                        if mk is None:
+                            self.acall('fami_relu_bwd', _p(dy), _p(y), _p(g), y.numel(), acc)
+                        else:
+                            self.acall('fami_relu_bwd_mask', _p(dy), _p(mk), _p(g), y.numel(), acc)
                     return
                 Pk = x.data.numel() // C
                 gx, accx = self.gbuf(x) if x.requires_grad else (self.like(x.data), 0)
@@ -1020,16 +1032,20 @@
                     return
                 two = self.bn2 and self.bn_fusable(Pk, C)
                 ws = self.zeros_bytes(self.Q.fami_bn_slots_bytes(C)) if two else self.ws(self.Q.fami_bn_workspace(C))
+                sfx, rm = ('', 1) if mk is None else ('_mask', 3)
                 if shift == 0:
                     if two:
-                        self.acall('fami_bn_bwd2', _p(dy), _p(x.data), _p(y), _p(st[0]), _p(st[1]), _p(bn.weight.data),
-                                   _p(bn.bias.data), _p(gx), _p(gg), _p(gb), None, Pk, C, 1, accx, accp, 0, _p(ws))
+                        self.acall('fami_bn_bwd2' + sfx, _p(dy), _p(x.data), _p(y), *mka, _p(st[0]), _p(st[1]), _p(bn.weight.data),
+                                   _p(bn.bias.data), _p(gx), _p(gg), _p(gb), None, Pk, C, rm, accx, accp, 0, _p(ws))
                     else:
-                        self.acall('fami_bn_bwd', _p(dy), _p(x.data), _p(y), _p(st[0]), _p(st[1]),
-                                   _p(bn.weight.data), _p(gx), _p(gg), _p(gb), None, Pk, C, 1, accx, accp, 0, _p(ws))
+                        self.acall('fami_bn_bwd' + sfx, _p(dy), _p(x.data), _p(y), *mka, _p(st[0]), _p(st[1]),
+                                   _p(bn.weight.data), _p(gx), _p(gg), _p(gb), None, Pk, C, rm, accx, accp, 0, _p(ws))
                 else:
                     low = self.like(x.data)
-                    self.acall('fami_pool_relu_bwd', _p(dy), _p(y), _p(low), N, H >> shift, W >> shift, C, shift, 1)
+                    if mk is None:
+                        self.acall('fami_pool_relu_bwd', _p(dy), _p(y), _p(low), N, H >> shift, W >> shift, C, shift, 1)
+                    else:
+                        self.acall('fami_pool_relu_bwd_mask', _p(dy), _p(mk), _p(low), N, H >> shift, W >> shift, C, shift, 1)
                     if two:
                         self.acall('fami_bn_bwd2', _p(low), _p(x.data), None, _p(st[0]), _p(st[1]), _p(bn.weight.data),
                                    _p(bn.bias.data), _p(gx), _p(gg), _p(gb), None, Pk, C, 0, accx, accp, 0, _p(ws))
@@ -1052,11 +1068,17 @@
         bet_a = PA(*[None if h['bn'] is None else _p(h['bn'].bias.data) for h in handles])
         sh_a = (ctypes.c_int * k)(*[h['shift'] for h in handles])
         y = self.act(N, H, W, C)
-        self.acall('fami_fuse_sum', k, xs, mean_a, inv_a, gam_a, bet_a, sh_a, _p(y), N, H, W, C, 1)
         rg = self.record and any(h['x'].requires_grad or (h['bn'] is not None and self.rq(h['bn'].weight)) for h in handles)
+        mk = None
+        if rg and self.relu_mask and all(h['bn'] is None or self.bn_batch_stats(h['bn']) for h in handles):
+            mk = self.empty(N * H * W * C // 4, dtype=torch.uint8)
+            self.acall('fami_fuse_sum_mask', k, xs, mean_a, inv_a, gam_a, bet_a, sh_a, _p(y), _p(mk), N, H, W, C, 1)
+        else:
+            self.acall('fami_fuse_sum', k, xs, mean_a, inv_a, gam_a, bet_a, sh_a, _p(y), N, H, W, C, 1)
         out = T(y, rg)
         for h in handles:
             h['out'] = out
+            h['mask'] = mk
         return out
 
     def batch_slice(self, x, n0, n1, terminal=False):
diff --git a/fami-pose_amd/options.py b/fami-pose_amd/options.py
--- a/fami-pose_amd/options.py
+++ b/fami-pose_amd/options.py
@@ -7,6 +7,7 @@
     'FAMI_BN_IN': ('1', 'conv1 -> bn1 -> ReLU -> conv2 (16-bit storage): bn1\'s apply pass inside conv2\'s launch where the weight-resident 48-channel kernel takes conv2 (fami_conv2d_fwd_bnin_*)'),
     'FAMI_XBN': (None, 'BatchNorm + ReLU applied by the consumer convolution; default on in f32 storage, off in the 16-bit modes'),
     'FAMI_MERGE_PREDICTORS': ('1', 'offset + mask predictor of a DCN layer as one 48 -> 324 convolution (needs the Trainer arena)'),
+    'FAMI_RELU_MASK': (None, 'BatchNorm + residual + ReLU and the fuse sums store their ReLU mask as one byte per 4-channel vector and the backwards read it instead of y (fami_*_mask_*); 0: the mask comes from the stored y; default on in f32 storage, off in the 16-bit modes'),
     'FAMI_DETERMINISTIC': ('0', 'run-to-run reproducible kernels (fixed-point DCN input gradient, three-launch BatchNorm)'),
     'FAMI_DDP_PLAN': ('overlap', 'data-parallel launch plan: overlap (graph segments + all-reduce between them) | serial'),
     'FAMI_DDP_GRAPH': ('1', '0: eager launches with the all-reduce fired from the backward hooks'),
diff --git a/include/fami.h b/include/fami.h
--- a/include/fami.h
+++ b/include/fami.h
@@ -508,6 +508,73 @@
                            fami_f16_t* gom, int B, int H, int W, int C, int Co, int G, int kh, int kw, int stride, int pad,
                            int dil, int acc_om, int acc_x, void* ws, fami_stream_t stream);
 
+int fami_bn_train_fwd_mask_f32(const float* x, const float* residual, float* y, unsigned char* mask, const float* gamma,
+        const float* beta, float* mean, float* invstd, float* running_mean, float* running_var, long P, int C, int relu,
+        float momentum, float eps, float* ws, fami_stream_t stream);
+int fami_bn_train_fwd2_mask_f32(const float* x, const float* residual, float* y, unsigned char* mask, const float* gamma,
+        const float* beta, float* mean, float* invstd, float* running_mean, float* running_var, long P, int C, int relu,
+        float momentum, float eps, void* slots, fami_stream_t stream);
+int fami_bn_apply_slots_mask_f32(const float* x, const float* residual, float* y, unsigned char* mask, const float* gamma,
+        const float* beta, float* mean, float* invstd, float* running_mean, float* running_var, long P, int C, int relu,
+        float momentum, float eps, void* slots, fami_stream_t stream);
+int fami_bn_bwd_mask_f32(const float* dy, const float* x, const float* y, const unsigned char* mask, const float* mean,
+        const float* invstd, const float* gamma, float* dx, float* dgamma, float* dbeta, float* dres, long P, int C, int relu,
+        int acc_dx, int acc_param, int acc_dres, float* ws, fami_stream_t stream);
+int fami_bn_bwd2_mask_f32(const float* dy, const float* x, const float* y, const unsigned char* mask, const float* mean,
+        const float* invstd, const float* gamma, const float* beta, float* dx, float* dgamma, float* dbeta, float* dres, long P,
+        int C, int relu, int acc_dx, int acc_param, int acc_dres, void* slots, fami_stream_t stream);
+int fami_fuse_sum_mask_f32(int nterms, const float* const* x, const float* const* mean, const float* const* invstd,
+        const float* const* gamma, const float* const* beta, const int* shift, float* y, unsigned char* mask, int N, int H,
+        int W, int C, int relu, fami_stream_t stream);
+int fami_relu_bwd_mask_f32(const float* dy, const unsigned char* mask, float* dx, long n, int accumulate,
+        fami_stream_t stream);
+int fami_pool_relu_bwd_mask_f32(const float* dy, const unsigned char* mask, float* out, int N, int Hl, int Wl, int C,
+        int shift, int relu, fami_stream_t stream);
+int fami_bn_train_fwd_mask_bf16(const fami_bf16_t* x, const fami_bf16_t* residual, fami_bf16_t* y, unsigned char* mask, const float* gamma,
+        const float* beta, float* mean, float* invstd, float* running_mean, float* running_var, long P, int C, int relu,
+        float momentum, float eps, float* ws, fami_stream_t stream);
+int fami_bn_train_fwd2_mask_bf16(const fami_bf16_t* x, const fami_bf16_t* residual, fami_bf16_t* y, unsigned char* mask, const float* gamma,
+        const float* beta, float* mean, float* invstd, float* running_mean, float* running_var, long P, int C, int relu,
+        float momentum, float eps, void* slots, fami_stream_t stream);
+int fami_bn_apply_slots_mask_bf16(const fami_bf16_t* x, const fami_bf16_t* residual, fami_bf16_t* y, unsigned char* mask, const float* gamma,
+        const float* beta, float* mean, float* invstd, float* running_mean, float* running_var, long P, int C, int relu,
+        float momentum, float eps, void* slots, fami_stream_t stream);
+int fami_bn_bwd_mask_bf16(const fami_bf16_t* dy, const fami_bf16_t* x, const fami_bf16_t* y, const unsigned char* mask, const float* mean,
+        const float* invstd, const float* gamma, fami_bf16_t* dx, float* dgamma, float* dbeta, fami_bf16_t* dres, long P, int C, int relu,
+        int acc_dx, int acc_param, int acc_dres, float* ws, fami_stream_t stream);
+int fami_bn_bwd2_mask_bf16(const fami_bf16_t* dy, const fami_bf16_t* x, const fami_bf16_t* y, const unsigned char* mask, const float* mean,
+        const float* invstd, const float* gamma, const float* beta, fami_bf16_t* dx, float* dgamma, float* dbeta, fami_bf16_t* dres, long P,
+        int C, int relu, int acc_dx, int acc_param, int acc_dres, void* slots, fami_stream_t stream);
+int fami_fuse_sum_mask_bf16(int nterms, const fami_bf16_t* const* x, const float* const* mean, const float* const* invstd,
+        const float* const* gamma, const float* const* beta, const int* shift, fami_bf16_t* y, unsigned char* mask, int N, int H,
+        int W, int C, int relu, fami_stream_t stream);
+int fami_relu_bwd_mask_bf16(const fami_bf16_t* dy, const unsigned char* mask, fami_bf16_t* dx, long n, int accumulate,
+        fami_stream_t stream);
+int fami_pool_relu_bwd_mask_bf16(const fami_bf16_t* dy, const unsigned char* mask, fami_bf16_t* out, int N, int Hl, int Wl, int C,
+        int shift, int relu, fami_stream_t stream);
+int fami_bn_train_fwd_mask_f16(const fami_f16_t* x, const fami_f16_t* residual, fami_f16_t* y, unsigned char* mask, const float* gamma,
+        const float* beta, float* mean, float* invstd, float* running_mean, float* running_var, long P, int C, int relu,
+        float momentum, float eps, float* ws, fami_stream_t stream);
+int fami_bn_train_fwd2_mask_f16(const fami_f16_t* x, const fami_f16_t* residual, fami_f16_t* y, unsigned char* mask, const float* gamma,
+        const float* beta, float* mean, float* invstd, float* running_mean, float* running_var, long P, int C, int relu,
+        float momentum, float eps, void* slots, fami_stream_t stream);
+int fami_bn_apply_slots_mask_f16(const fami_f16_t* x, const fami_f16_t* residual, fami_f16_t* y, unsigned char* mask, const float* gamma,
+        const float* beta, float* mean, float* invstd, float* running_mean, float* running_var, long P, int C, int relu,
+        float momentum, float eps, void* slots, fami_stream_t stream);
+int fami_bn_bwd_mask_f16(const fami_f16_t* dy, const fami_f16_t* x, const fami_f16_t* y, const unsigned char* mask, const float* mean,
+        const float* invstd, const float* gamma, fami_f16_t* dx, float* dgamma, float* dbeta, fami_f16_t* dres, long P, int C, int relu,
+        int acc_dx, int acc_param, int acc_dres, float* ws, fami_stream_t stream);
+int fami_bn_bwd2_mask_f16(const fami_f16_t* dy, const fami_f16_t* x, const fami_f16_t* y, const unsigned char* mask, const float* mean,
+        const float* invstd, const float* gamma, const float* beta, fami_f16_t* dx, float* dgamma, float* dbeta, fami_f16_t* dres, long P,
+        int C, int relu, int acc_dx, int acc_param, int acc_dres, void* slots, fami_stream_t stream);
+int fami_fuse_sum_mask_f16(int nterms, const fami_f16_t* const* x, const float* const* mean, const float* const* invstd,
+        const float* const* gamma, const float* const* beta, const int* shift, fami_f16_t* y, unsigned char* mask, int N, int H,
+        int W, int C, int relu, fami_stream_t stream);
+int fami_relu_bwd_mask_f16(const fami_f16_t* dy, const unsigned char* mask, fami_f16_t* dx, long n, int accumulate,
+        fami_stream_t stream);
+int fami_pool_relu_bwd_mask_f16(const fami_f16_t* dy, const unsigned char* mask, fami_f16_t* out, int N, int Hl, int Wl, int C,
+        int shift, int relu, fami_stream_t stream);
+
 #ifdef __cplusplus
 }
 #endif
```

Result: no change. 92.03 (median of 6 runs) (+0.7%).
